# maximyudayev/Realtime-ST-GCN

Hardware: AMD Instinct MI355X
Metric: skeleton-frames/sec/GPU (fwd+bwd), 10-layer ST-GCN N=64 T=300 V=25 (higher is better)
Workload: dtype bf16; 1 GPU; config 2: as_is st-gcn (fcn_in + 9 StgcnLayer, BatchNorm, Kt=9), fwd + loss + bwd + Adam; global_batch=64, seq_len=300, joints=25, parallelism=single, bn_stats=per-replica, launch=eager

## Files before the change

### include/stgcn_amd.h

```cpp
#ifndef STGCN_AMD_H
#define STGCN_AMD_H

#ifdef __cplusplus
extern "C" {
#endif

#define STGCN_ABI_VERSION 7

typedef struct {
  const void* in;
  void* out;
  const void* w;
  const float* bias;
  const float* pro_a;
  const float* pro_b;
  const float* pro_stats;
  float* stats;
  int N, T_in, T_out, V, Cin, Cout, Cin_pad, Cout_pad;
  int Kt, stride, pad, trans, pro, bias_mode, accumulate;
  int in_ld, out_ld;
  const void* w_frag;
} stgcn_conv_desc;

int stgcn_conv_rows(const stgcn_conv_desc* d, int dtype, void* stream);
// ... 2 lines not shown
int stgcn_pack_weight(const float* src, long s0, long s1, long s2, int Kt, int Cout, int Cin, void* dst, int Cout_pad,
                      int Cin_pad, int dtype, void* stream);
int stgcn_pack_weight_frag(const float* src, long s0, long s1, long s2, int Kt, int Cout, int Cin, void* dst,
                           void* dst_frag, int Cout_pad, int Cin_pad, int dtype, void* stream);
int stgcn_pack_weight_s2frag(const float* src, long s0, long s1, long s2, int Cout, int Cin, void* dst_frag, int trans,
                             int dtype, void* stream);
int stgcn_conv_rows_col_tile(int cout);
long stgcn_conv_rows_row_blocks(long M, int cout);

typedef struct {
  const void* in;
  const void* dy;
  float* dw;
  const float* pro_a;
  const float* pro_b;
  const float* pro_stats;
  int N, T_in, T_out, V, Cin, Cout, Kt, stride, pad, pro;
  int in_ld, dy_ld;
  long rows_per_block;
  void* work;
  long work_bytes;
  int out_mode;
  int pad_;
} stgcn_wgrad_desc;

int stgcn_conv_wgrad(const stgcn_wgrad_desc* d, int dtype, void* stream);
long stgcn_conv_wgrad_workspace(const stgcn_wgrad_desc* d, int dtype);

typedef struct {
  const void* x;
  void* out;
  const float* A;
  int N, T, V, P, Cin, per_sample, accumulate;
  int x_ld, out_ld;
} stgcn_amix_desc;

int stgcn_amix_fwd(const stgcn_amix_desc* d, int dtype, void* stream);
int stgcn_amix_trans(const stgcn_amix_desc* d, int dtype, void* stream);
long stgcn_amix_dA_workspace(const stgcn_amix_desc* d);
int stgcn_amix_dA(const stgcn_amix_desc* d, const void* dw, float* dA, void* work, int dtype, void* stream);
int stgcn_gcn_bias_bwd(const float* A, const float* b, const float* S, int P, int V, int C, float* dA, float* db,
                       void* stream);
int stgcn_gcn_bias(const float* A, const float* b, float* out, int N, int P, int V, int C, int per_sample,
                   void* stream);

typedef struct {
  const void* in;
  void* out;
  const void* w;
  const int* nbr;
  const int* deg;
  const float* bias;
  float* stats;
  int NT, V, J, Cin, Cout, Cin_pad, Cout_pad, in_ld, out_ld, accumulate;
  const void* res;
  const void* res_bits;
  int res_ld;
} stgcn_gconv_desc;

int stgcn_gconv(const stgcn_gconv_desc* d, int dtype, void* stream);

long stgcn_gconv_row_blocks(int NT, int V);
int stgcn_gconv_weights(const float* A, const float* W, const int* nbr, const int* deg, int P, int V, int J, int Cout,
                        int Cin, int trans, void* out, int rows_pad, int cols_pad, int dtype, void* stream);
int stgcn_gconv_weights_bias(const float* A, const float* W, const float* b, const int* nbr, const int* deg, int P,
                             int V, int J, int Cout, int Cin, void* out, int rows_pad, int cols_pad, float* bias2d,
                             int dtype, void* stream);
typedef struct {
  const void* x;
  const void* dy;
  const int* nbr;
  const int* deg;
  float* dweff;
  int NT, V, J, Cin, Cout, x_ld, dy_ld;
  void* work;
  long work_bytes;
  float* rowsum;
  int phase;
  int pad_;
} stgcn_gconv_wgrad_desc;

int stgcn_gconv_wgrad(const stgcn_gconv_wgrad_desc* d, int dtype, void* stream);
long stgcn_gconv_wgrad_workspace(const stgcn_gconv_wgrad_desc* d, int dtype);
long stgcn_gconv_wgrad_finish_workspace(int P, int V, int J, int Cout, int Cin);
int stgcn_gconv_wgrad_finish_bias(const float* dweff, const float* A, const float* W, const int* nbr, const int* deg,
                                  int P, int V, int J, int Cout, int Cin, const float* bconv, const float* S, float* dW,
                                  float* dA, float* db, void* work, void* stream);
int stgcn_gconv_wgrad_finish(const float* dweff, const float* A, const float* W, const int* nbr, const int* deg, int P,
                             int V, int J, int Cout, int Cin, float* dW, float* dA, void* work, void* stream);

long stgcn_bn_stat_blocks(long M);
int stgcn_bn_stats_partial(const void* x, int ld, long M, int C, void* part_f4, int dtype, void* stream);
int stgcn_bn_finalize(const void* part_f4, int nblocks, int ld_part, int C, const float* gamma, const float* beta,
                      float eps, void* mean_rstd_f2, float* scale, float* shift, void* stream);
int stgcn_bn_merge(const void* part_f4, int nblocks, int ld_part, int C, void* merged_f4, void* stream);
typedef struct {
  const void* dy;
  const void* mref;
  const void* x1;
  const void* x2;
  const float* msc;
  const float* msh;
  const float* mean_rstd1;
  const float* mean_rstd2;
  const float* gamma1;
  const float* gamma2;
  float* sums;
  void* out1;
  void* out2;
  float* osum;
  float* work;
  long M;
  int C, mask, lddy, ldm, ldx1, ldx2, ldo1, ldo2, acc2;
} stgcn_bn_bwd_desc;

long stgcn_bn_bwd_fused_workspace(long M, int C, int dtype);
int stgcn_bn_bwd_fused_reduce(const stgcn_bn_bwd_desc* d, int dtype, void* stream);
int stgcn_bn_bwd_fused_apply(const stgcn_bn_bwd_desc* d, int dtype, void* stream);
int stgcn_bn_apply(const void* u, int ldu, const float* sc, const float* sh, int res_mode, const void* r, int ldr,
                   const float* rsc, const float* rsh, int relu, void* y, int ldy, long M, int C, int dtype,
                   void* stream);
int stgcn_bn_apply_bits(const void* u, int ldu, const float* sc, const float* sh, int res_mode, const void* r, int ldr,
                        const float* rsc, const float* rsh, int relu, void* y, int ldy, long M, int C, void* bits,
                        void* stream);
int stgcn_bn_bwd_reduce(const void* dy, int lddy, int mask, const void* mref, int ldm, const float* msc,
                        const float* msh, const void* x, int ldx, const void* mean_rstd_f2, long M, int C,
                        void* part_f2, void* sums_f2, int dtype, void* stream);
int stgcn_bn_bwd_apply(const void* dy, int lddy, int mask, const void* mref, int ldm, const float* msc,
                       const float* msh, const void* x, int ldx, const void* mean_rstd_f2, const float* gamma,
                       const void* sums_f2, long M, int C, void* dx, int lddx, int accumulate, int dtype,
                       void* stream);
int stgcn_rowgroup_sum(const void* x, int ld, long M, int C, int G, long period, float* S, float* work, int dtype,
                       void* stream);
long stgcn_rowgroup_sum_workspace(long M, int C, int G, long period);

int stgcn_ln_stats(const void* x, int ld, long frames, int V, int C, float eps, void* stats_f2, int dtype,
                   void* stream);
int stgcn_ln_apply(const void* u, int ldu, const void* st_f2, const float* g, const float* b, int res_mode,
                   const void* r, int ldr, const void* rst_f2, const float* rg, const float* rb, int relu, void* y,
                   int ldy, long M, int V, int C, int dtype, void* stream);
int stgcn_ln_bwd(const void* dy, int lddy, int mask, const void* mref, int ldm, const void* x, int ldx,
                 const void* st_f2, const float* g, const float* b, long frames, int V, int C, void* dx, int lddx,
                 int accumulate, float* dgb, void* work, long work_bytes, int dtype, void* stream);
long stgcn_ln_bwd_workspace(long frames, int V, int C, int dtype);

int stgcn_cast_colsum(const float* x, int ldx, long M, int C, void* out_bf16, int ldo, float* colsum, float* work,
                      void* stream);
long stgcn_cast_colsum_workspace(long M, int C);

int stgcn_pool_rows(const void* x, int ld, int N, int R, int C, void* out, int ldo, int dtype, void* stream);
int stgcn_unpool_rows(const void* dp, int ldp, int R, int C, long M, void* dx, int ldx, int dtype, void* stream);

int stgcn_box_sum(const void* x, int ldx, void* y, int ldy, int N, int T, int V, int C, int K, int S, int trans,
                  int accumulate, int dtype, void* stream);
int stgcn_rt_online_step(const void* z_f32, float* fifo, float* acc, int* idx, int C, int V, int fifo_size, int S,
                         float* out, void* stream);

int stgcn_attn_proj(const void* x, int ldx, long M, int Cin, const float* w, const float* bias, int Nout, float* out,
                    int ldo, void* stream);
long stgcn_attn_scores_workspace(int N, int T, int V, int P);
int stgcn_attn_scores(const void* theta, const void* phi, int ld, int N, int T, int V, int P, int ce, float* C,
                      void* work, int dtype, void* stream);
int stgcn_attn_bwd(const void* theta, const void* phi, int ld, int N, int T, int V, int P, int ce, const float* C,
                   const float* dC, float* dS, void* dtheta, void* dphi, int dtype, void* stream);

int stgcn_abi_version(void);
// ... 290 lines not shown
  const float* ln_b;
  const float* w_in;
  const float* b_in;
  const float* w_out;
  const float* b_out;
  float* xb;
  float* z;
  float* r;
  float* a;
  float* out;
  stgcn_rt_streams_layer layers[STGCN_RT_MAX_LAYERS];
} stgcn_rt_streams_clip_desc;
int stgcn_rt_streams_clip(const stgcn_rt_streams_clip_desc* d, void* stream);

typedef struct {
  int R, V, F, dil, dtype, pad_;
  const float* x;
  const void* wp;
  const float* b1;
  const float* b2;
  float* y;
  void* h;
  const float* dy;
  void* g;
  float* dx;
  float* part;
  float* grads;
} stgcn_ms_layer;
long stgcn_ms_pack_elems(int F);
int stgcn_ms_pack_layer(const float* w1, const float* w2, int F, int kernel, void* dst, int dtype, void* stream);
int stgcn_ms_wgrad_blocks(int R);
int stgcn_ms_layer_fwd(const stgcn_ms_layer* d, void* stream);
int stgcn_ms_layer_bwd(const stgcn_ms_layer* d, void* stream);

typedef struct {
  int rows, pool, I, O, mode, pad_;
  const float* in;
  const float* w;
  const float* b;
  float* out;
  float* p;
  const float* d;
  float* din;
  float* part;
  float* grads;
} stgcn_ms_lin;
int stgcn_ms_lin_blocks(int rows);
int stgcn_ms_in_fwd(const stgcn_ms_lin* d, void* stream);
int stgcn_ms_in_bwd(const stgcn_ms_lin* d, void* stream);
int stgcn_ms_out_fwd(const stgcn_ms_lin* d, void* stream);
int stgcn_ms_out_bwd(const stgcn_ms_lin* d, void* stream);
int stgcn_ms_prob_fwd(const float* x, int rows, int C, int mode, float* y, void* stream);
int stgcn_ms_prob_bwd(const float* y, const float* dy, int rows, int C, int mode, float* dx, void* stream);

int stgcn_window_stat_blocks(int nw, int W);
int stgcn_window_stats(const float* x, int Cin, int Lp, int V, int W, int n0, int nw, int mode, float eps, float* out,
                       void* stream);
int stgcn_window_expand(const float* x, int Cin, int Lp, int V, int W, int n0, int nw, int mode, const float* g,
                        const float* b, const float* fst, const float* w, const float* bias, int Cout, void* out,
                        int ldo, int dtype, void* stream);
long stgcn_window_grad_workspace(int nw, int W, int V, int Cin, int Cout);
int stgcn_window_grad(const void* dy, int ldd, int dtype, const float* x, int Cin, int Lp, int V, int W, int n0, int nw,
                      int mode, const float* st, const float* gamma, const float* beta, const float* w, int Cout,
                      void* work, float* dgamma, float* dbeta, float* dw, float* db, void* stream);

typedef struct {
  int kind, dtype, trans, Kt, Co, Ci, cp, kp;
  long s0, s1, s2, threads;
  const float* src;
  void* dst;
  void* dst_frag;
  const float* A;
  const float* M;
  const int* nbr;
  const int* deg;
  int P, V, J, R_pad, C_pad, pad_;
  const float* bconv;
  float* bias2d;
} stgcn_prep_job;
int stgcn_prep_check(stgcn_prep_job* jobs, int njobs);
int stgcn_prep_run(const stgcn_prep_job* jobs_dev, const long* block_start_dev, int njobs, long nblocks,
                   void* stream);

#define STGCN_ADAM_MAXT 256
typedef struct {
  float* p;
  float* m;
  float* v;
  long n, b0;
  int vec, pad_;
} stgcn_adam_entry;
long stgcn_adam_blocks(long n);
int stgcn_adam_step(const stgcn_adam_entry* table_dev, int ntensors, long nblocks, const float* const* grads,
                    float* steps, double lr, double beta1, double beta2, double eps, double weight_decay,
                    void* stream);

#ifdef __cplusplus
}
#endif
#endif
```

### realtime-st-gcn_amd/__init__.py

```python
from . import _lib, data, loss, metrics, native, optim, parallel, routing, segment, syncbn
from .syncbn import convert_sync_batchnorm, revert_sync_batchnorm
from .graph import Graph, PKU_MMD
from .modules import BatchNorm1d, ConvTemporalGraphical, LayerNorm, StgcnLayer, set_compute_dtype
from .stgcn import Model as Stgcn

MODELS = {
    "st-gcn": Stgcn,
}

try:
    from .rtstgcn import Model as RtStgcn
    MODELS["rt-st-gcn"] = RtStgcn
except ImportError:
    pass
try:
    from .aagcn import Model as AaGcn
    MODELS["aa-gcn"] = AaGcn
except ImportError:
    pass
try:
    from .costgcn import Model as CoStgcn
    MODELS["co-st-gcn"] = CoStgcn
except ImportError:
    pass
try:
    from .mstcn import Model as MsTcn
    from .msgcn import Model as MsGcn
    MODELS["ms-tcn"] = MsTcn
    MODELS["ms-gcn"] = MsGcn
except ImportError:
    pass
```

### realtime-st-gcn_amd/_lib.py

```python
from __future__ import annotations

import ctypes
import os

import torch

_HERE = os.path.dirname(os.path.abspath(__file__))
LIB_PATH = os.environ.get("STGCN_LIB") or os.path.join(_HERE, "lib", "libstgcn_amd.so")

ABI_VERSION = 7

_ERR = {1: "bad shape/arguments", 2: "unsupported dtype", 3: "HIP launch error"}

c_void_p = ctypes.c_void_p
c_int = ctypes.c_int
c_long = ctypes.c_long
c_float = ctypes.c_float


class AdamEntry(ctypes.Structure):
    _fields_ = [("p", c_void_p), ("m", c_void_p), ("v", c_void_p), ("n", c_long), ("b0", c_long), ("vec", c_int),
                ("pad_", c_int)]


class ConvDesc(ctypes.Structure):
    _fields_ = [("in_", c_void_p), ("out", c_void_p), ("w", c_void_p), ("bias", c_void_p), ("pro_a", c_void_p),
                ("pro_b", c_void_p), ("pro_stats", c_void_p), ("stats", c_void_p)] + \
               [(n, c_int) for n in ("N", "T_in", "T_out", "V", "Cin", "Cout", "Cin_pad", "Cout_pad", "Kt", "stride",
                                     "pad", "trans", "pro", "bias_mode", "accumulate", "in_ld", "out_ld")] + \
               [("w_frag", c_void_p)]


class WgradDesc(ctypes.Structure):
    _fields_ = [("in_", c_void_p), ("dy", c_void_p), ("dw", c_void_p), ("pro_a", c_void_p), ("pro_b", c_void_p),
                ("pro_stats", c_void_p)] + \
               [(n, c_int) for n in ("N", "T_in", "T_out", "V", "Cin", "Cout", "Kt", "stride", "pad", "pro",
                                     "in_ld", "dy_ld")] + [("rows_per_block", c_long), ("work", c_void_p),
                                                           ("work_bytes", c_long), ("out_mode", c_int), ("pad_", c_int)]


class AmixDesc(ctypes.Structure):
    _fields_ = [("x", c_void_p), ("out", c_void_p), ("A", c_void_p)] + \
               [(n, c_int) for n in ("N", "T", "V", "P", "Cin", "per_sample", "accumulate", "x_ld", "out_ld")]


class GconvDesc(ctypes.Structure):
    _fields_ = [("in_", c_void_p), ("out", c_void_p), ("w", c_void_p), ("nbr", c_void_p), ("deg", c_void_p),
                ("bias", c_void_p), ("stats", c_void_p)] + \
               [(n, c_int) for n in ("NT", "V", "J", "Cin", "Cout", "Cin_pad", "Cout_pad", "in_ld", "out_ld",
                                     "accumulate")] + [("res", c_void_p), ("res_bits", c_void_p), ("res_ld", c_int)]


class GconvWgradDesc(ctypes.Structure):
    _fields_ = [("x", c_void_p), ("dy", c_void_p), ("nbr", c_void_p), ("deg", c_void_p), ("dweff", c_void_p)] + \
               [(n, c_int) for n in ("NT", "V", "J", "Cin", "Cout", "x_ld", "dy_ld")] + \
               [("work", c_void_p), ("work_bytes", c_long), ("rowsum", c_void_p), ("phase", c_int), ("pad_", c_int)]


class LayerFusedDesc(ctypes.Structure):
    _fields_ = [(n, c_void_p) for n in ("x", "z", "wg_frag", "A", "gbias", "wt_frag", "tbias")] + \
               [(n, c_int) for n in ("N", "T", "V", "P", "x_ld", "z_ld")] + \
               [(n, c_void_p) for n in ("ln1_g", "ln1_b", "ln2_g", "ln2_b")] + [("residual", c_int), ("pad_", c_int)] + \
               [(n, c_void_p) for n in ("g_out", "u_out", "st1_out", "st2_out")] + [("g_ld", c_int), ("u_ld", c_int)] + \
               [("h_out", c_void_p), ("h_ld", c_int), ("pad2_", c_int)]


class BnBwdDesc(ctypes.Structure):
    _fields_ = [(n, c_void_p) for n in ("dy", "mref", "x1", "x2", "msc", "msh", "mean_rstd1", "mean_rstd2",
                                        "gamma1", "gamma2", "sums", "out1", "out2", "osum", "work")] + \
               [("M", c_long)] + [(n, c_int) for n in ("C", "mask", "lddy", "ldm", "ldx1", "ldx2", "ldo1", "ldo2",
                                                       "acc2")]


class PrepJob(ctypes.Structure):
    _fields_ = [(n, c_int) for n in ("kind", "dtype", "trans", "Kt", "Co", "Ci", "cp", "kp")] + \
               [(n, c_long) for n in ("s0", "s1", "s2", "threads")] + \
               [(n, c_void_p) for n in ("src", "dst", "dst_frag", "A", "M", "nbr", "deg")] + \
               [(n, c_int) for n in ("P", "V", "J", "R_pad", "C_pad", "pad_")] + \
               [(n, c_void_p) for n in ("bconv", "bias2d")]


RT_MAX_LAYERS = 12


class RtLayer(ctypes.Structure):
    _fields_ = [(n, c_int) for n in ("Cin", "Cout", "P", "fifo_size", "S", "res_mode")] + \
               [(n, c_void_p) for n in ("A", "w", "bias2d", "wr", "ln_w", "ln_b", "lnr_w", "lnr_b", "fifo", "acc",
                                        "idx", "a_buf", "r_buf")]


class RtFrameDesc(ctypes.Structure):
    _fields_ = [(n, c_int) for n in ("V", "L", "C0", "K", "blocks")] + \
               [(n, c_void_p) for n in ("x", "ln_w", "ln_b", "w_in", "b_in", "w_out", "b_out", "out", "sync",
                                        "status")] + \
               [("layers", RtLayer * RT_MAX_LAYERS)]


class RtStreamsLayer(ctypes.Structure):
    _fields_ = [(n, c_int) for n in ("Cin", "Cout", "P", "fifo_size", "S", "res_mode")] + \
               [(n, c_void_p) for n in ("A", "wp", "bias2d", "wrp", "ln_w", "ln_b", "lnr_w", "lnr_b", "fifo", "acc",
                                        "idx")]


class RtStreamsDesc(ctypes.Structure):
    _fields_ = [(n, c_int) for n in ("V", "L", "C0", "K", "B", "dtype")] + \
               [(n, c_void_p) for n in ("x", "active", "ln_w", "ln_b", "w_in", "b_in", "w_out", "b_out", "out")] + \
               [("layers", RtStreamsLayer * RT_MAX_LAYERS)]


class CoLayer(ctypes.Structure):
    _fields_ = [(n, c_int) for n in ("V", "Cin", "Cout", "P", "Kt", "S", "res_mode", "dtype", "splits", "pad_")] + \
               [(n, c_void_p) for n in ("x", "A", "w", "bias2d", "wr", "br", "ln1_w", "ln1_b", "ln2_w", "ln2_b",
                                        "lnr_w", "lnr_b", "wt", "bt", "ring", "res_ring", "idx", "z_buf", "r_buf",
                                        "partial", "y")]


class CoStreamsLayer(ctypes.Structure):
    _fields_ = [(n, c_int) for n in ("Cin", "Cout", "P", "Kt", "S", "res_mode", "splits", "pad_")] + \
               [(n, c_void_p) for n in ("A", "wp", "bias2d", "wrp", "br", "ln1_w", "ln1_b", "ln2_w", "ln2_b", "lnr_w",
                                        "lnr_b", "wt", "bt", "ring", "res_ring", "idx", "z_buf", "r_buf", "partial",
                                        "y")]


class CoStreamsDesc(ctypes.Structure):
    _fields_ = [(n, c_int) for n in ("B", "V", "L", "C0", "K", "dtype")] + \
               [(n, c_void_p) for n in ("x", "active", "ln_w", "ln_b", "w_in", "b_in", "w_out", "b_out", "h0", "order",
                                        "out")] + \
               [("layers", CoStreamsLayer * RT_MAX_LAYERS)]


CO_CLIP_MAX_T = 256


class CoClipLayer(ctypes.Structure):
    _fields_ = [(n, c_int) for n in ("Cin", "Cout", "P", "Kt", "S", "res_mode", "splits", "pad_")] + \
               [(n, c_void_p) for n in ("A", "wp", "bias2d", "wrp", "br", "ln1_w", "ln1_b", "ln2_w", "ln2_b", "lnr_w",
                                        "lnr_b", "wt", "bt", "ring", "res_ring", "idx", "z_buf", "r_buf", "hist",
                                        "resq", "partial", "y")]


class CoClipDesc(ctypes.Structure):
    _fields_ = [(n, c_int) for n in ("T", "V", "L", "C0", "K", "dtype")] + [("x_stride", c_long)] + \
               [(n, c_void_p) for n in ("x", "ln_w", "ln_b", "w_in", "b_in", "w_out", "b_out", "h0", "out")] + \
               [("layers", CoClipLayer * RT_MAX_LAYERS)]


class CoStreamsClipLayer(ctypes.Structure):
    _fields_ = list(CoClipLayer._fields_)


class CoStreamsClipDesc(ctypes.Structure):
    _fields_ = [(n, c_int) for n in ("B", "T", "t0", "V", "L", "C0", "K", "dtype")] + \
               [(n, c_long) for n in ("x_stride", "x_bstride", "out_bstride")] + \
               [(n, c_void_p) for n in ("x", "active", "lengths", "ln_w", "ln_b", "w_in", "b_in", "w_out", "b_out",
                                        "h0", "out")] + \
               [("layers", CoStreamsClipLayer * RT_MAX_LAYERS)]


RT_CLIP_MAX_T = 256


class RtStreamsClipDesc(ctypes.Structure):
    _fields_ = [(n, c_int) for n in ("B", "T", "t0", "V", "L", "C0", "K", "dtype")] + \
               [(n, c_long) for n in ("x_stride", "x_bstride", "out_bstride", "fstride")] + \
               [(n, c_void_p) for n in ("x", "active", "lengths", "ln_w", "ln_b", "w_in", "b_in", "w_out", "b_out",
                                        "xb", "z", "r", "a", "out")] + \
               [("layers", RtStreamsLayer * RT_MAX_LAYERS)]


class MsLayer(ctypes.Structure):
    _fields_ = [(n, c_int) for n in ("R", "V", "F", "dil", "dtype", "pad_")] + \
               [(n, c_void_p) for n in ("x", "wp", "b1", "b2", "y", "h", "dy", "g", "dx", "part", "grads")]


class MsLin(ctypes.Structure):
    _fields_ = [(n, c_int) for n in ("rows", "pool", "I", "O", "mode", "pad_")] + \
               [(n, c_void_p) for n in ("in_", "w", "b", "out", "p", "d", "din", "part", "grads")]


_SIGS = {
    "stgcn_abi_version": (c_int, []),
    "stgcn_conv_rows": (c_int, [ctypes.POINTER(ConvDesc), c_int, c_void_p]),
    "stgcn_conv_rows_col_tile": (c_int, [c_int]),
    "stgcn_conv_rows_row_blocks": (c_long, [c_long, c_int]),
    "stgcn_conv_wgrad": (c_int, [ctypes.POINTER(WgradDesc), c_int, c_void_p]),
    "stgcn_conv_wgrad_workspace": (c_long, [ctypes.POINTER(WgradDesc), c_int]),
    "stgcn_gconv": (c_int, [ctypes.POINTER(GconvDesc), c_int, c_void_p]),
    "stgcn_bn_bwd_fused_workspace": (c_long, [c_long, c_int, c_int]),
    "stgcn_bn_bwd_fused_reduce": (c_int, [ctypes.POINTER(BnBwdDesc), c_int, c_void_p]),
    "stgcn_bn_bwd_fused_apply": (c_int, [ctypes.POINTER(BnBwdDesc), c_int, c_void_p]),
    "stgcn_gconv_row_blocks": (c_long, [c_int, c_int]),
    "stgcn_gconv_weights_bias": (c_int, [c_void_p] * 5 + [c_int] * 5 + [c_void_p, c_int, c_int, c_void_p, c_int,
                                                                       c_void_p]),
    "stgcn_gconv_weights": (c_int, [c_void_p, c_void_p, c_void_p, c_void_p] + [c_int] * 6 + [c_void_p, c_int, c_int,
                                                                                           c_int, c_void_p]),
    "stgcn_gconv_wgrad": (c_int, [ctypes.POINTER(GconvWgradDesc), c_int, c_void_p]),
    "stgcn_gconv_wgrad_workspace": (c_long, [ctypes.POINTER(GconvWgradDesc), c_int]),
    "stgcn_gconv_wgrad_finish_workspace": (ctypes.c_long, [c_int] * 5),
    "stgcn_gconv_wgrad_finish": (c_int, [c_void_p] * 5 + [c_int] * 5 + [c_void_p, c_void_p, c_void_p, c_void_p]),
    "stgcn_gconv_wgrad_finish_bias": (c_int, [c_void_p] * 5 + [c_int] * 5 + [c_void_p] * 7),
    "stgcn_amix_fwd": (c_int, [ctypes.POINTER(AmixDesc), c_int, c_void_p]),
    "stgcn_amix_trans": (c_int, [ctypes.POINTER(AmixDesc), c_int, c_void_p]),
    "stgcn_gcn_bias_bwd": (c_int, [c_void_p, c_void_p, c_void_p, c_int, c_int, c_int, c_void_p, c_void_p, c_void_p]),
    "stgcn_pack_weight": (c_int, [c_void_p, ctypes.c_long, ctypes.c_long, ctypes.c_long, c_int, c_int, c_int,
                                  c_void_p, c_int, c_int, c_int, c_void_p]),
    "stgcn_tconv_frame": (c_int, [ctypes.POINTER(ConvDesc), c_void_p]),
    "stgcn_tconv_frame_row_blocks": (ctypes.c_long, [c_int, c_int]),
    "stgcn_pack_weight_s2frag": (c_int, [c_void_p, ctypes.c_long, ctypes.c_long, ctypes.c_long, c_int, c_int,
                                         c_void_p, c_int, c_int, c_void_p]),
    "stgcn_pack_weight_frag": (c_int, [c_void_p, ctypes.c_long, ctypes.c_long, ctypes.c_long, c_int, c_int, c_int,
                                       c_void_p, c_void_p, c_int, c_int, c_int, c_void_p]),
    "stgcn_amix_dA_workspace": (ctypes.c_long, [ctypes.POINTER(AmixDesc)]),
    "stgcn_amix_dA": (c_int, [ctypes.POINTER(AmixDesc), c_void_p, c_void_p, c_void_p, c_int, c_void_p]),
    "stgcn_gcn_bias": (c_int, [c_void_p, c_void_p, c_void_p, c_int, c_int, c_int, c_int, c_int, c_void_p]),
    "stgcn_bn_stat_blocks": (c_long, [c_long]),
    "stgcn_bn_stats_partial": (c_int, [c_void_p, c_int, c_long, c_int, c_void_p, c_int, c_void_p]),
    "stgcn_bn_finalize": (c_int, [c_void_p, c_int, c_int, c_int, c_void_p, c_void_p, c_float, c_void_p, c_void_p,
                                  c_void_p, c_void_p]),
    "stgcn_bn_merge": (c_int, [c_void_p, c_int, c_int, c_int, c_void_p, c_void_p]),
    "stgcn_bn_apply": (c_int, [c_void_p, c_int, c_void_p, c_void_p, c_int, c_void_p, c_int, c_void_p, c_void_p,
                               c_int, c_void_p, c_int, c_long, c_int, c_int, c_void_p]),
    "stgcn_bn_apply_bits": (c_int, [c_void_p, c_int, c_void_p, c_void_p, c_int, c_void_p, c_int, c_void_p, c_void_p,
                                    c_int, c_void_p, c_int, c_long, c_int, c_void_p, c_void_p]),
    "stgcn_bn_bwd_reduce": (c_int, [c_void_p, c_int, c_int, c_void_p, c_int, c_void_p, c_void_p, c_void_p, c_int,
                                    c_void_p, c_long, c_int, c_void_p, c_void_p, c_int, c_void_p]),
    "stgcn_bn_bwd_apply": (c_int, [c_void_p, c_int, c_int, c_void_p, c_int, c_void_p, c_void_p, c_void_p, c_int,
                                   c_void_p, c_void_p, c_void_p, c_long, c_int, c_void_p, c_int, c_int, c_int,
                                   c_void_p]),
    "stgcn_rowgroup_sum": (c_int, [c_void_p, c_int, c_long, c_int, c_int, c_long, c_void_p, c_void_p, c_int,
                                   c_void_p]),
    "stgcn_rowgroup_sum_workspace": (c_long, [c_long, c_int, c_int, c_long]),
    "stgcn_ln_stats": (c_int, [c_void_p, c_int, c_long, c_int, c_int, c_float, c_void_p, c_int, c_void_p]),
    "stgcn_ln_apply": (c_int, [c_void_p, c_int, c_void_p, c_void_p, c_void_p, c_int, c_void_p, c_int, c_void_p,
                               c_void_p, c_void_p, c_int, c_void_p, c_int, c_long, c_int, c_int, c_int, c_void_p]),
    "stgcn_ln_bwd": (c_int, [c_void_p, c_int, c_int, c_void_p, c_int, c_void_p, c_int, c_void_p, c_void_p, c_void_p,
                             c_long, c_int, c_int, c_void_p, c_int, c_int, c_void_p, c_void_p, c_long, c_int,
                             c_void_p]),
    "stgcn_ln_bwd_workspace": (c_long, [c_long, c_int, c_int, c_int]),
    "stgcn_cast_colsum": (c_int, [c_void_p, c_int, c_long, c_int, c_void_p, c_int, c_void_p, c_void_p, c_void_p]),
    "stgcn_cast_colsum_workspace": (c_long, [c_long, c_int]),
    "stgcn_pool_rows": (c_int, [c_void_p, c_int, c_int, c_int, c_int, c_void_p, c_int, c_int, c_void_p]),
    "stgcn_unpool_rows": (c_int, [c_void_p, c_int, c_int, c_int, c_long, c_void_p, c_int, c_int, c_void_p]),
    "stgcn_box_sum": (c_int, [c_void_p, c_int, c_void_p, c_int, c_int, c_int, c_int, c_int, c_int, c_int, c_int,
                              c_int, c_int, c_void_p]),
    "stgcn_rt_online_step": (c_int, [c_void_p, c_void_p, c_void_p, c_void_p, c_int, c_int, c_int, c_int, c_void_p,
                                     c_void_p]),
    "stgcn_attn_scores_workspace": (ctypes.c_long, [c_int, c_int, c_int, c_int]),
    "stgcn_attn_scores": (c_int, [c_void_p, c_void_p, c_int, c_int, c_int, c_int, c_int, c_int, c_void_p, c_void_p,
                                  c_int, c_void_p]),
    "stgcn_attn_bwd": (c_int, [c_void_p, c_void_p, c_int, c_int, c_int, c_int, c_int, c_int, c_void_p, c_void_p,
                               c_void_p, c_void_p, c_void_p, c_int, c_void_p]),
    "stgcn_layer_fused_fwd": (c_int, [ctypes.POINTER(LayerFusedDesc), c_void_p]),
    "stgcn_rt_frame_in": (c_int, [c_void_p, c_int, c_void_p, c_void_p, c_void_p, c_void_p, c_int, c_void_p, c_void_p]),
    "stgcn_rt_frame_gcn": (c_int, [c_void_p, c_int, c_int, c_int, c_int] + [c_void_p] * 10),
    "stgcn_rt_frame_norm": (c_int, [c_void_p, c_void_p, c_void_p, c_int, c_void_p, c_void_p, c_void_p, c_int, c_int,
                                    c_void_p, c_int, c_int, c_void_p, c_void_p]),
    "stgcn_rt_frame_out": (c_int, [c_void_p, c_int, c_int, c_void_p, c_void_p, c_int, c_void_p, c_void_p]),
    "stgcn_rt_frame": (c_int, [ctypes.POINTER(RtFrameDesc), c_void_p]),
    "stgcn_rt_streams_pack_elems": (c_long, [c_int, c_int]),
    "stgcn_rt_streams_pack_weight": (c_int, [c_void_p, c_int, c_int, c_int, c_void_p, c_void_p]),
    "stgcn_rt_streams_pack_weight_as": (c_int, [c_void_p, c_int, c_int, c_int, c_void_p, c_int, c_void_p]),
    "stgcn_rt_streams": (c_int, [ctypes.POINTER(RtStreamsDesc), c_void_p]),
    "stgcn_co_pack_elems": (c_long, [c_int, c_int, c_int]),
    "stgcn_co_pack_weight": (c_int, [c_void_p, c_int, c_int, c_int, c_void_p, c_int, c_void_p]),
    "stgcn_co_splits": (c_int, [ctypes.POINTER(CoLayer), c_void_p]),
    "stgcn_co_workspace": (c_long, [ctypes.POINTER(CoLayer), c_void_p]),
    "stgcn_co_gcn": (c_int, [ctypes.POINTER(CoLayer), c_void_p]),
    "stgcn_co_push": (c_int, [ctypes.POINTER(CoLayer), c_void_p]),
    "stgcn_co_taps": (c_int, [ctypes.POINTER(CoLayer), c_void_p]),
    "stgcn_co_finish": (c_int, [ctypes.POINTER(CoLayer), c_void_p]),
    "stgcn_co_streams_splits": (c_int, [ctypes.POINTER(CoStreamsDesc), c_int]),
    "stgcn_co_streams_workspace": (c_long, [ctypes.POINTER(CoStreamsDesc), c_int]),
    "stgcn_co_streams": (c_int, [ctypes.POINTER(CoStreamsDesc), c_void_p]),
    "stgcn_co_clip_splits": (c_int, [ctypes.POINTER(CoClipDesc), c_int]),
    "stgcn_co_clip_workspace": (c_long, [ctypes.POINTER(CoClipDesc), c_int]),
    "stgcn_co_clip": (c_int, [ctypes.POINTER(CoClipDesc), c_void_p]),
    "stgcn_co_streams_clip_splits": (c_int, [ctypes.POINTER(CoStreamsClipDesc), c_int]),
    "stgcn_co_streams_clip_workspace": (c_long, [ctypes.POINTER(CoStreamsClipDesc), c_int]),
    "stgcn_co_streams_clip": (c_int, [ctypes.POINTER(CoStreamsClipDesc), c_void_p]),
    "stgcn_rt_streams_clip": (c_int, [ctypes.POINTER(RtStreamsClipDesc), c_void_p]),
    "stgcn_ms_pack_elems": (c_long, [c_int]),
    "stgcn_ms_pack_layer": (c_int, [c_void_p, c_void_p, c_int, c_int, c_void_p, c_int, c_void_p]),
    "stgcn_ms_wgrad_blocks": (c_int, [c_int]),
    "stgcn_ms_layer_fwd": (c_int, [ctypes.POINTER(MsLayer), c_void_p]),
    "stgcn_ms_layer_bwd": (c_int, [ctypes.POINTER(MsLayer), c_void_p]),
    "stgcn_ms_lin_blocks": (c_int, [c_int]),
    "stgcn_ms_in_fwd": (c_int, [ctypes.POINTER(MsLin), c_void_p]),
    "stgcn_ms_in_bwd": (c_int, [ctypes.POINTER(MsLin), c_void_p]),
    "stgcn_ms_out_fwd": (c_int, [ctypes.POINTER(MsLin), c_void_p]),
    "stgcn_ms_out_bwd": (c_int, [ctypes.POINTER(MsLin), c_void_p]),
    "stgcn_ms_prob_fwd": (c_int, [c_void_p, c_int, c_int, c_int, c_void_p, c_void_p]),
    "stgcn_ms_prob_bwd": (c_int, [c_void_p, c_void_p, c_int, c_int, c_int, c_void_p, c_void_p]),
    "stgcn_window_stat_blocks": (c_int, [c_int, c_int]),
    "stgcn_window_stats": (c_int, [c_void_p] + [c_int] * 7 + [c_float, c_void_p, c_void_p]),
    "stgcn_window_expand": (c_int, [c_void_p] + [c_int] * 7 + [c_void_p] * 5 + [c_int, c_void_p, c_int, c_int,
                                                                                c_void_p]),
    "stgcn_window_grad_workspace": (ctypes.c_long, [c_int] * 5),
    "stgcn_window_grad": (c_int, [c_void_p, c_int, c_int, c_void_p] + [c_int] * 7 + [c_void_p] * 4 + [c_int] +
                          [c_void_p] * 6),
    "stgcn_attn_proj": (c_int, [c_void_p, c_int, c_long, c_int, c_void_p, c_void_p, c_int, c_void_p, c_int, c_void_p]),
    "stgcn_segment_metrics_workspace": (ctypes.c_long, [c_int]),
    "stgcn_segment_metrics": (c_int, [c_void_p, c_void_p, c_int, c_int, c_void_p, c_int, c_void_p, c_void_p,
                                      c_void_p, c_void_p, c_void_p]),
    "stgcn_seg_loss_workspace": (ctypes.c_long, [c_int]),
    "stgcn_seg_loss": (c_int, [c_void_p, c_int, c_void_p, c_void_p, c_void_p, c_int, c_int, c_int, c_int, c_void_p,
                               c_float, c_void_p, c_void_p, c_void_p, c_void_p, c_void_p, c_void_p]),
    "stgcn_seg_loss_bwd": (c_int, [c_void_p, c_void_p, c_void_p, c_void_p, c_long, c_void_p, c_void_p]),
    "stgcn_prep_check": (c_int, [ctypes.POINTER(PrepJob), c_int]),
    "stgcn_prep_run": (c_int, [c_void_p, c_void_p, c_int, c_long, c_void_p]),
    "stgcn_adam_blocks": (ctypes.c_long, [c_long]),
    "stgcn_adam_step": (c_int, [c_void_p, c_int, c_long, c_void_p, c_void_p] + [ctypes.c_double] * 5 + [c_void_p]),
}

EXPORTS = tuple(_SIGS)

_lib = None


def load_library(path: str = LIB_PATH):
    global _lib
    if _lib is not None:
        return _lib
    if not os.path.exists(path):
        raise RuntimeError(f"stgcn_amd: native library not built: {path} (run __graft_entry__.build())")
    lib = ctypes.CDLL(path)
    for name, (res, args) in _SIGS.items():
        fn = getattr(lib, name)
        fn.restype = res
        fn.argtypes = args
    got = lib.stgcn_abi_version()
    if got != ABI_VERSION:
        raise RuntimeError(f"stgcn_amd: {path} implements C-ABI version {got}, these bindings need {ABI_VERSION} "
                           "(stale build: run __graft_entry__.build())")
    _lib = lib
    return lib


def lib():
    if _lib is None:
        load_library()
    return _lib


def check(rc: int, name: str):
    if rc != 0:
        raise RuntimeError(f"stgcn_amd.{name} failed with code {rc} ({_ERR.get(rc, 'unknown')})")


def require_device(t: torch.Tensor):
    if not t.is_cuda:
        raise RuntimeError("stgcn_amd ops run on the HIP device only (no CPU fallback); got a CPU tensor")


def stream() -> int:
    return torch._C._cuda_getCurrentRawStream(torch._C._cuda_getDevice())


def dtype_code(dt: torch.dtype) -> int:
    if dt == torch.float32:
        return 0
    if dt == torch.bfloat16:
        return 1
    raise RuntimeError(f"stgcn_amd: unsupported dtype {dt} (fp32 or bf16)")


def ptr(t):
    return None if t is None else t.data_ptr()
```

### realtime-st-gcn_amd/csrc/capi.cpp

```cpp
#include <hip/hip_runtime.h>

#include "../../include/stgcn_amd.h"
#include "launchers.h"

#define STGCN_OK 0
#define STGCN_EBADSHAPE 1
#define STGCN_EDTYPE 2

#define CHECK_DTYPE(dt) \
  if ((dt) != 0 && (dt) != 1) return STGCN_EDTYPE
#define STREAM(s) reinterpret_cast<hipStream_t>(s)

extern "C" {

int stgcn_abi_version(void) { return STGCN_ABI_VERSION; }

int stgcn_conv_rows(const stgcn_conv_desc* d, int dtype, void* stream) {
  CHECK_DTYPE(dtype);
  if (!d || !d->in || !d->out || !d->w || d->N <= 0 || d->V <= 0 || d->T_in <= 0 || d->T_out <= 0 || d->Kt <= 0 ||
      d->stride <= 0 || d->Cin <= 0 || d->Cout <= 0 || d->in_ld < d->Cin || d->out_ld < d->Cout ||
      d->Cin_pad < d->Cin || d->Cout_pad < d->Cout)
    return STGCN_EBADSHAPE;
  if ((d->pro == 1 && (!d->pro_a || !d->pro_b)) || (d->pro == 2 && (!d->pro_a || !d->pro_b || !d->pro_stats)))
    return STGCN_EBADSHAPE;
// ... 20 lines not shown
  if (!src || !dst || !dst_frag || Kt <= 0 || Co <= 0 || Ci <= 0 || Cout_pad < Co || Cin_pad < Ci) return STGCN_EBADSHAPE;
  return pack_weight_launch(src, s0, s1, s2, Kt, Co, Ci, dst, Cout_pad, Cin_pad, dtype, STREAM(stream), dst_frag);
}
long stgcn_conv_rows_row_blocks(long M, int cout) { return conv_rows_num_row_blocks(M, cout); }

long stgcn_conv_wgrad_workspace(const stgcn_wgrad_desc* d, int dtype) {
  if (!d || (dtype != 0 && dtype != 1)) return 0;
  const long wr = wgrad_ring_workspace(*d, dtype);
  if (wr > 0) return wr;
  const long w = wgrad_wide_workspace(*d, dtype);
  if (w > 0) return w;
  const long w1 = wgrad1x1_workspace(*d, dtype);
  return w1 > 0 ? w1 : wgrad_tile_workspace(*d, dtype);
}

int stgcn_conv_wgrad(const stgcn_wgrad_desc* d, int dtype, void* stream) {
  CHECK_DTYPE(dtype);
  if (!d || !d->in || !d->dy || !d->dw || d->N <= 0 || d->Kt <= 0 || d->stride <= 0) return STGCN_EBADSHAPE;
  if (d->pro && (!d->pro_a || !d->pro_b || (d->pro == 2 && !d->pro_stats))) return STGCN_EBADSHAPE;
  if (d->out_mode != 0 && d->out_mode != 1) return STGCN_EBADSHAPE;
  const int rr = wgrad_ring_launch(*d, dtype, STREAM(stream));
  if (rr >= 0) return rr;
  const int rw = wgrad_wide_launch(*d, dtype, STREAM(stream));
  if (rw >= 0) return rw;
  const int r1 = wgrad1x1_launch(*d, dtype, STREAM(stream));
  if (r1 >= 0) return r1;
  const int r = wgrad_tile_launch(*d, dtype, STREAM(stream));
  if (r >= 0) return r;
  if (d->out_mode) return STGCN_EBADSHAPE;
  return conv_wgrad_launch(*d, dtype, STREAM(stream));
}

long stgcn_bn_bwd_fused_workspace(long M, int C, int dtype) {
  if (M <= 0 || C <= 0 || (dtype != 0 && dtype != 1)) return 0;
  return bn_bwd_fused_work_floats(M, C, dtype);
}
int stgcn_bn_bwd_fused_reduce(const stgcn_bn_bwd_desc* d, int dtype, void* stream) {
  CHECK_DTYPE(dtype);
  if (!d || !d->dy || d->M <= 0 || d->C <= 0 || (d->mask && !d->mref) || (d->mask == 2 && (!d->msc || !d->msh)) ||
      (d->x1 && !d->mean_rstd1) || (d->x2 && !d->mean_rstd2) || (d->mask == 3 && (dtype != 1 || d->C % 8 || d->ldm < d->C / 8)))
    return STGCN_EBADSHAPE;
  return bn_bwd_fused_reduce_launch(*d, dtype, STREAM(stream));
}
int stgcn_bn_bwd_fused_apply(const stgcn_bn_bwd_desc* d, int dtype, void* stream) {
  CHECK_DTYPE(dtype);
  if (!d || !d->dy || d->M <= 0 || d->C <= 0 || (d->mask && !d->mref) || (d->mask == 2 && (!d->msc || !d->msh)) ||
      (d->x1 && !d->mean_rstd1) || (d->x2 && !d->mean_rstd2) || (d->mask == 3 && (dtype != 1 || d->C % 8 || d->ldm < d->C / 8)))
    return STGCN_EBADSHAPE;
  return bn_bwd_fused_apply_launch(*d, dtype, STREAM(stream));
}

int stgcn_gconv(const stgcn_gconv_desc* d, int dtype, void* stream) {
  CHECK_DTYPE(dtype);
  if (!d || !d->in || !d->out || !d->w || !d->nbr || !d->deg || d->NT <= 0 || d->V <= 0 || d->J <= 0 ||
      d->Cin <= 0 || d->Cout <= 0 || d->Cin_pad < d->Cin || d->Cout_pad < d->Cout || d->in_ld < d->Cin ||
      d->out_ld < d->Cout)
    return STGCN_EBADSHAPE;
  return gconv_launch(*d, dtype, STREAM(stream));
}
long stgcn_gconv_row_blocks(int NT, int V) { return gconv_row_blocks(NT, V); }
int stgcn_gconv_weights(const float* A, const float* W, const int* nbr, const int* deg, int P, int V, int J, int Cout,
                        int Cin, int trans, void* out, int rows_pad, int cols_pad, int dtype, void* stream) {
  CHECK_DTYPE(dtype);
  if (!A || !W || !nbr || !deg || !out || P <= 0 || V <= 0 || J <= 0 || Cout <= 0 || Cin <= 0 ||
      rows_pad < (trans ? Cin : Cout) || cols_pad < (trans ? Cout : Cin))
    return STGCN_EBADSHAPE;
  return gconv_weights_launch(A, W, nbr, deg, P, V, J, Cout, Cin, trans, out, rows_pad, cols_pad, dtype,
                              STREAM(stream));
}
int stgcn_gconv_weights_bias(const float* A, const float* W, const float* b, const int* nbr, const int* deg, int P,
                             int V, int J, int Cout, int Cin, void* out, int rows_pad, int cols_pad, float* bias2d,
                             int dtype, void* stream) {
  CHECK_DTYPE(dtype);
  if (!A || !W || !b || !nbr || !deg || !out || !bias2d || P <= 0 || V <= 0 || J <= 0 || Cout <= 0 || Cin <= 0 ||
      rows_pad < Cout || cols_pad < Cin || (cols_pad % 8) != 0)
    return STGCN_EBADSHAPE;
  return gconv_weights_launch(A, W, nbr, deg, P, V, J, Cout, Cin, 0, out, rows_pad, cols_pad, dtype, STREAM(stream),
                              b, bias2d);
}
long stgcn_gconv_wgrad_workspace(const stgcn_gconv_wgrad_desc* d, int dtype) {
  if (!d || (dtype != 0 && dtype != 1)) return 0;
  return gconv_wgrad_workspace(*d, dtype);
}
int stgcn_gconv_wgrad(const stgcn_gconv_wgrad_desc* d, int dtype, void* stream) {
  CHECK_DTYPE(dtype);
  if (!d || !d->x || !d->dy || !d->nbr || !d->deg || !d->dweff || d->NT <= 0 || d->V <= 0 || d->J <= 0 ||
      d->Cin <= 0 || d->Cout <= 0)
    return STGCN_EBADSHAPE;
  return gconv_wgrad_launch(*d, dtype, STREAM(stream));
}
int stgcn_gconv_wgrad_finish_bias(const float* dweff, const float* A, const float* W, const int* nbr, const int* deg,
                                  int P, int V, int J, int Cout, int Cin, const float* bconv, const float* S, float* dW,
                                  float* dA, float* db, void* work, void* stream) {
  if (!dweff || !A || !W || !nbr || !deg || !bconv || !S || !dW || !dA || !db || !work || P <= 0 || V <= 0 || J <= 0 ||
      Cout <= 0 || Cin <= 0)
    return STGCN_EBADSHAPE;
  return gconv_wgrad_finish_bias_launch(dweff, A, W, nbr, deg, P, V, J, Cout, Cin, bconv, S, dW, dA, db, work,
                                        STREAM(stream));
}
long stgcn_gconv_wgrad_finish_workspace(int P, int V, int J, int Cout, int Cin) {
  return gconv_wgrad_finish_workspace(P, V, J, Cout, Cin);
}
int stgcn_gconv_wgrad_finish(const float* dweff, const float* A, const float* W, const int* nbr, const int* deg, int P,
                             int V, int J, int Cout, int Cin, float* dW, float* dA, void* work, void* stream) {
  if (!dweff || !A || !W || !nbr || !deg || P <= 0 || V <= 0 || J <= 0 || Cout <= 0 || Cin <= 0)
    return STGCN_EBADSHAPE;
  return gconv_wgrad_finish_launch(dweff, A, W, nbr, deg, P, V, J, Cout, Cin, dW, dA, work, STREAM(stream));
}
int stgcn_tconv_frame(const stgcn_conv_desc* d, void* stream) {
  if (!d) return STGCN_EBADSHAPE;
  return tconv_frame_launch(*d, STREAM(stream));
}
long stgcn_tconv_frame_row_blocks(int N, int T) { return tconv_frame_row_blocks(N, T); }

int stgcn_amix_fwd(const stgcn_amix_desc* d, int dtype, void* stream) {
  CHECK_DTYPE(dtype);
  if (!d || !d->x || !d->out || !d->A) return STGCN_EBADSHAPE;
  return amix_fwd_launch(*d, dtype, STREAM(stream));
}
int stgcn_amix_trans(const stgcn_amix_desc* d, int dtype, void* stream) {
  CHECK_DTYPE(dtype);
  if (!d || !d->x || !d->out || !d->A) return STGCN_EBADSHAPE;
  return amix_trans_launch(*d, dtype, STREAM(stream));
}
long stgcn_amix_dA_workspace(const stgcn_amix_desc* d) { return d ? amix_dA_workspace(*d) : 0; }
int stgcn_amix_dA(const stgcn_amix_desc* d, const void* dw, float* dA, void* work, int dtype, void* stream) {
  CHECK_DTYPE(dtype);
  if (!d || !d->x || !dw || !dA) return STGCN_EBADSHAPE;
  return amix_dA_launch(*d, dw, dA, work, dtype, STREAM(stream));
}
int stgcn_gcn_bias_bwd(const float* A, const float* b, const float* S, int P, int V, int C, float* dA, float* db,
                       void* stream) {
  if (!A || !b || !S || !dA || !db || P <= 0 || V <= 0 || C <= 0) return STGCN_EBADSHAPE;
  return gcn_bias_bwd_launch(A, b, S, P, V, C, dA, db, STREAM(stream));
}
int stgcn_gcn_bias(const float* A, const float* b, float* out, int N, int P, int V, int C, int per_sample,
                   void* stream) {
  if (!A || !b || !out) return STGCN_EBADSHAPE;
  return gcn_bias_launch(A, b, out, N, P, V, C, per_sample, STREAM(stream));
}

long stgcn_bn_stat_blocks(long M) { return norm_stats_num_blocks(M); }
int stgcn_bn_stats_partial(const void* x, int ld, long M, int C, void* part, int dtype, void* stream) {
  CHECK_DTYPE(dtype);
  return bn_stats_partial_launch(x, ld, M, C, (float4*)part, dtype, STREAM(stream));
}
int stgcn_bn_finalize(const void* part, int nb, int ldp, int C, const float* gamma, const float* beta, float eps,
                      void* mean_rstd, float* scale, float* shift, void* stream) {
  return bn_finalize_launch((const float4*)part, nb, ldp, C, gamma, beta, eps, (float2*)mean_rstd, scale, shift,
                            STREAM(stream));
}
int stgcn_bn_merge(const void* part, int nb, int ldp, int C, void* merged, void* stream) {
  return bn_merge_launch((const float4*)part, nb, ldp, C, (float4*)merged, STREAM(stream));
}
int stgcn_bn_apply(const void* u, int ldu, const float* sc, const float* sh, int res_mode, const void* r, int ldr,
                   const float* rsc, const float* rsh, int relu, void* y, int ldy, long M, int C, int dtype,
                   void* stream) {
  CHECK_DTYPE(dtype);
  if (res_mode && !r) return STGCN_EBADSHAPE;
  return bn_apply_launch(u, ldu, sc, sh, res_mode, r, ldr, rsc, rsh, relu, y, ldy, M, C, dtype, STREAM(stream));
}
int stgcn_bn_apply_bits(const void* u, int ldu, const float* sc, const float* sh, int res_mode, const void* r, int ldr,
                        const float* rsc, const float* rsh, int relu, void* y, int ldy, long M, int C, void* bits,
                        void* stream) {
  if ((res_mode && !r) || !bits || C % 8) return STGCN_EBADSHAPE;
  return bn_apply_launch(u, ldu, sc, sh, res_mode, r, ldr, rsc, rsh, relu, y, ldy, M, C, 1, STREAM(stream),
// ... 267 lines not shown
```

### realtime-st-gcn_amd/csrc/gconv_finish.hip

```cpp
#include "common.h"
#include "launchers.h"

namespace {

__global__ void gconv_dw_kernel(const float* __restrict__ dweff, const float* __restrict__ A, const int* nbr,
                                const int* deg, int P, int V, int J, int Cout, int Cin, float* dW) {
  const long idx = (long)blockIdx.x * blockDim.x + threadIdx.x;
  const long E = (long)Cout * Cin;
  if (idx >= (long)P * E) return;
  const int p = (int)(idx / E);
  const long e = idx % E;
  float s = 0.f;
  for (int w = 0; w < V; ++w)
    for (int j = 0; j < deg[w]; ++j) s += A[((long)p * V + nbr[w * J + j]) * V + w] * dweff[(long)(w * J + j) * E + e];
  dW[idx] += s;
}

__global__ void gconv_dA_kernel(const float* __restrict__ dweff, const float* __restrict__ W, const int* nbr,
                                const int* deg, int P, int V, int J, int Cout, int Cin, float* dA) {
  const int pair = blockIdx.x, p = blockIdx.y;
  const int w = pair / J, j = pair % J;
  if (j >= deg[w]) return;
  const long E = (long)Cout * Cin;
  const float* d = dweff + (long)pair * E;
  const float* wp = W + (long)p * E;
  float s = 0.f;
  for (long e = threadIdx.x; e < E; e += blockDim.x) s += wp[e] * d[e];
  s = wave_sum(s);
  __shared__ float part[4];
  if ((threadIdx.x & 63) == 0) part[threadIdx.x >> 6] = s;
  __syncthreads();
  if (threadIdx.x == 0) {
    const float t = part[0] + part[1] + part[2] + part[3];
    dA[((long)p * V + nbr[w * J + j]) * V + w] += t;
  }
}

constexpr int PMAX = 4;
constexpr int DW_PAIRS = 32 * 8;
DEV void gconv_dw_all_body(const float* __restrict__ dweff, const float* __restrict__ A, const int* nbr,
                           const int* deg, int P, int V, int J, long E, float* dW, long bb, bool acc_out) {
  __shared__ int spair[DW_PAIRS];
  __shared__ float scoef[DW_PAIRS][PMAX];
  __shared__ int snp;
  if (threadIdx.x == 0) {
    int n = 0;
    for (int w = 0; w < V; ++w)
      for (int j = 0; j < deg[w]; ++j) spair[n++] = w * J + j;
    snp = n;
  }
  __syncthreads();
  const int np = snp;
  for (int i = threadIdx.x; i < np * PMAX; i += 256) {
    const int k = i / PMAX, p = i % PMAX;
    const int pr = spair[k], w = pr / J;
    scoef[k][p] = p < P ? A[((long)p * V + nbr[pr]) * V + w] : 0.f;
  }
  __syncthreads();
  const int g = threadIdx.x >> 6;
  const long e = (bb * 64 + (threadIdx.x & 63)) * 4;
  float4 acc[PMAX];
#pragma unroll
  for (int p = 0; p < PMAX; ++p) acc[p] = make_float4(0.f, 0.f, 0.f, 0.f);
  if (e < E) {
#pragma unroll 4
    for (int k = g; k < np; k += 4) {
      const float4 d = *reinterpret_cast<const float4*>(dweff + (long)spair[k] * E + e);
#pragma unroll
      for (int p = 0; p < PMAX; ++p) {
        const float c = scoef[k][p];
        acc[p].x += c * d.x; acc[p].y += c * d.y; acc[p].z += c * d.z; acc[p].w += c * d.w;
      }
    }
  }
  __shared__ float4 part[4][PMAX][64];
#pragma unroll
  for (int p = 0; p < PMAX; ++p) part[g][p][threadIdx.x & 63] = acc[p];
  __syncthreads();
  if (threadIdx.x < 64 && e < E) {
    const int l = threadIdx.x;
#pragma unroll
    for (int p = 0; p < PMAX; ++p)
      if (p < P) {
        const float4 a0 = part[0][p][l], a1 = part[1][p][l], a2 = part[2][p][l], a3 = part[3][p][l];
        float4 t = make_float4(((a0.x + a1.x) + a2.x) + a3.x, ((a0.y + a1.y) + a2.y) + a3.y,
                               ((a0.z + a1.z) + a2.z) + a3.z, ((a0.w + a1.w) + a2.w) + a3.w);
        float4* o = reinterpret_cast<float4*>(dW + (long)p * E + e);
        if (acc_out) {
          const float4 q = *o;
          t.x += q.x; t.y += q.y; t.z += q.z; t.w += q.w;
        }
        *o = t;
      }
  }
}
__global__ __launch_bounds__(256) void gconv_dw_all_kernel(const float* __restrict__ dweff, const float* __restrict__ A,
                                                           const int* nbr, const int* deg, int P, int V, int J, long E,
                                                           float* dW) {
  gconv_dw_all_body(dweff, A, nbr, deg, P, V, J, E, dW, blockIdx.x, true);
}

constexpr int DA_CHUNK = 2048;
DEV void gconv_dA_part_body(const float* __restrict__ dweff, const float* __restrict__ W, const int* deg, int P, int J,
                           long E, float* part, int pair, int c, int nch) {
  if (pair % J >= deg[pair / J]) return;
  const float* d = dweff + (long)pair * E;
  float acc[PMAX] = {0.f, 0.f, 0.f, 0.f};
  const long e1 = min(E, (long)(c + 1) * DA_CHUNK);
  for (long e = (long)c * DA_CHUNK + threadIdx.x * 4; e < e1; e += 1024) {
    const float4 dv = *reinterpret_cast<const float4*>(d + e);
#pragma unroll
    for (int p = 0; p < PMAX; ++p)
      if (p < P) {
        const float4 w = *reinterpret_cast<const float4*>(W + (long)p * E + e);
        acc[p] += ((w.x * dv.x + w.y * dv.y) + w.z * dv.z) + w.w * dv.w;
      }
  }
  __shared__ float red[4][PMAX];
#pragma unroll
  for (int p = 0; p < PMAX; ++p) {
    const float t = wave_sum(acc[p]);
    if ((threadIdx.x & 63) == 0) red[threadIdx.x >> 6][p] = t;
  }
  __syncthreads();
  if (threadIdx.x < P)
    part[((long)pair * nch + c) * PMAX + threadIdx.x] =
        ((red[0][threadIdx.x] + red[1][threadIdx.x]) + red[2][threadIdx.x]) + red[3][threadIdx.x];
}
__global__ __launch_bounds__(256) void gconv_dA_part_kernel(const float* __restrict__ dweff, const float* __restrict__ W,
                                                            const int* deg, int P, int J, long E, float* part) {
  gconv_dA_part_body(dweff, W, deg, P, J, E, part, blockIdx.x, blockIdx.y, gridDim.y);
}

__global__ __launch_bounds__(256) void gconv_finish1_kernel(const float* __restrict__ dweff, const float* __restrict__ A,
                                                            const float* __restrict__ W, const int* nbr, const int* deg,
                                                            int P, int V, int J, long E, float* dW, int nb_dw, int nch,
                                                            float* part) {
  const int b = blockIdx.x;
  if (b < nb_dw) {
    gconv_dw_all_body(dweff, A, nbr, deg, P, V, J, E, dW, b, false);
  } else {
    const int b2 = b - nb_dw;
    gconv_dA_part_body(dweff, W, deg, P, J, E, part, b2 / nch, b2 % nch, nch);
  }
}

constexpr int FV_MAX = 32;
__global__ __launch_bounds__(256) void gconv_finish2_kernel(const float* __restrict__ part, const float* __restrict__ A,
                                                            const float* __restrict__ b, const float* __restrict__ S,
                                                            const int* nbr, const int* deg, int P, int V, int J, int C,
                                                            int nch, float* dA, float* db) {
  const int bx = blockIdx.x;
  if (bx < P * V) {
    const int p = bx / V, w = bx % V;
    float t = 0.f;
    for (int c = threadIdx.x; c < C; c += 256) t += b[p * C + c] * S[w * C + c];
    t = wave_sum(t);
    __shared__ float red[4];
    __shared__ float sup[FV_MAX];
    if ((threadIdx.x & 63) == 0) red[threadIdx.x >> 6] = t;
    if (threadIdx.x < V) sup[threadIdx.x] = 0.f;
    __syncthreads();
    const float tot = ((red[0] + red[1]) + red[2]) + red[3];
    if (threadIdx.x < deg[w]) {
      const int j = threadIdx.x, pair = w * J + j;
      float s = 0.f;
      for (int c = 0; c < nch; ++c) s += part[((long)pair * nch + c) * PMAX + p];
      sup[nbr[pair]] = s;
    }
    __syncthreads();
    for (int v = threadIdx.x; v < V; v += 256) dA[(p * V + v) * V + w] = sup[v] + tot;
    return;
  }
  __shared__ float cs[PMAX * FV_MAX];
  for (int i = threadIdx.x; i < P * V; i += 256) {
    const int p = i / V, w = i % V;
    float t = 0.f;
    for (int v = 0; v < V; ++v) t += A[(p * V + v) * V + w];
    cs[i] = t;
  }
  __syncthreads();
  const int i = (bx - P * V) * 256 + threadIdx.x;
  if (i >= P * C) return;
  const int p = i / C, c = i % C;
  float t = 0.f;
  for (int w = 0; w < V; ++w) t += cs[p * V + w] * S[w * C + c];
  db[i] = t;
}

__global__ void gconv_dA_reduce_kernel(const float* __restrict__ part, const int* nbr, const int* deg, int P, int V,
                                       int J, int nch, float* dA) {
  const int i = blockIdx.x * blockDim.x + threadIdx.x;
  if (i >= V * J * P) return;
  const int pair = i / P, p = i % P, w = pair / J, j = pair % J;
  if (j >= deg[w]) return;
  float s = 0.f;
  for (int c = 0; c < nch; ++c) s += part[((long)pair * nch + c) * PMAX + p];
  dA[((long)p * V + nbr[w * J + j]) * V + w] += s;
}

}

long gconv_wgrad_finish_workspace(int P, int V, int J, int Cout, int Cin) {
  const long E = (long)Cout * Cin;
  return P > PMAX ? 0 : (long)V * J * ((E + DA_CHUNK - 1) / DA_CHUNK) * PMAX * (long)sizeof(float);
}

bool gconv_finish_bias_ok(int P, int V, int J) { return P <= PMAX && V <= FV_MAX && V * J <= DW_PAIRS; }

int gconv_wgrad_finish_bias_launch(const float* dweff, const float* A, const float* W, const int* nbr, const int* deg,
                                   int P, int V, int J, int Cout, int Cin, const float* bconv, const float* S, float* dW,
                                   float* dA, float* db, void* work, hipStream_t s) {
  if (!gconv_finish_bias_ok(P, V, J) || !work || ((long)Cout * Cin) % 4) return STGCN_EBADSHAPE;
  const long E = (long)Cout * Cin;
  const int nch = (int)((E + DA_CHUNK - 1) / DA_CHUNK);
  const int nb_dw = (int)((E + 255) / 256);
  float* part = reinterpret_cast<float*>(work);
  hipLaunchKernelGGL(gconv_finish1_kernel, dim3((unsigned)(nb_dw + V * J * nch)), dim3(256), 0, s, dweff, A, W, nbr,
                     deg, P, V, J, E, dW, nb_dw, nch, part);
  hipLaunchKernelGGL(gconv_finish2_kernel, dim3((unsigned)(P * V + (P * Cout + 255) / 256)), dim3(256), 0, s,
                     (const float*)part, A, bconv, S, nbr, deg, P, V, J, Cout, nch, dA, db);
  return hipGetLastError() == hipSuccess ? STGCN_OK : STGCN_EHIP;
}

int gconv_wgrad_finish_launch(const float* dweff, const float* A, const float* W, const int* nbr, const int* deg,
                              int P, int V, int J, int Cout, int Cin, float* dW, float* dA, void* work, hipStream_t s) {
  const long E = (long)Cout * Cin;
  if (P > PMAX || (dA && !work) || V * J > DW_PAIRS || E % 4) {
    const long n = (long)P * E;
    if (dW)
      hipLaunchKernelGGL(gconv_dw_kernel, dim3((unsigned)((n + 255) / 256)), dim3(256), 0, s, dweff, A, nbr, deg, P,
                         V, J, Cout, Cin, dW);
    if (dA)
      hipLaunchKernelGGL(gconv_dA_kernel, dim3((unsigned)(V * J), (unsigned)P), dim3(256), 0, s, dweff, W, nbr, deg,
                         P, V, J, Cout, Cin, dA);
  } else {
    if (dW)
      hipLaunchKernelGGL(gconv_dw_all_kernel, dim3((unsigned)((E + 255) / 256)), dim3(256), 0, s, dweff, A, nbr, deg,
                         P, V, J, E, dW);
    if (dA) {
      const int nch = (int)((E + DA_CHUNK - 1) / DA_CHUNK);
      float* part = reinterpret_cast<float*>(work);
      hipLaunchKernelGGL(gconv_dA_part_kernel, dim3((unsigned)(V * J), (unsigned)nch), dim3(256), 0, s, dweff, W,
                         deg, P, J, E, part);
      hipLaunchKernelGGL(gconv_dA_reduce_kernel, dim3((unsigned)((V * J * P + 255) / 256)), dim3(256), 0, s, part,
                         nbr, deg, P, V, J, nch, dA);
    }
  }
  return hipGetLastError() == hipSuccess ? STGCN_OK : STGCN_EHIP;
}
```

### realtime-st-gcn_amd/csrc/gconv_wgrad.hip

```cpp
#include "common.h"
#include "launchers.h"
#include "lds_ops.h"
#include "../../include/stgcn_amd.h"

namespace {

constexpr int WKM = 128;
constexpr int WPR = 64;

struct WGG {
  int ntile, tpb, R, nco, nci;
  float* slab;
  float* rowpart;
  int zero_unused;
  float* part;
  unsigned* cnt;
};
constexpr int W3_SPLIT_DEG = 4;

__global__ __launch_bounds__(256, 2) void gconv_wgrad_kernel(const stgcn_gconv_wgrad_desc a, const WGG g) {
  constexpr int PANEL = WKM * WPR;
  constexpr int STAGE = 4 * PANEL;
  extern __shared__ __attribute__((aligned(16))) char smem[];
  const int tid = threadIdx.x, lane = tid & 63, wave = tid >> 6;
  const int V = a.V;
  const int ngrp = g.nco * g.nci;
  const int pair = blockIdx.x / (ngrp * g.R);
  const int rem = blockIdx.x % (ngrp * g.R);
  const int rr = rem / ngrp, grp = rem % ngrp;
  const int w = pair / a.J, j = pair % a.J;
  if (j >= a.deg[w]) return;
  const int src = a.nbr[pair];
  const int co0 = (grp % g.nco) * 64, ci0 = (grp / g.nco) * 64;
  const int t0 = rr * g.tpb, t1 = min(g.ntile, t0 + g.tpb);

  const bf16* __restrict__ dy = reinterpret_cast<const bf16*>(a.dy);
  const bf16* __restrict__ x = reinterpret_cast<const bf16*>(a.x);
  const int uc = tid & 7;
  const int co = co0 + uc * 8, ci = ci0 + uc * 8;
  uint4 ry[4], rx[4];
  auto load = [&](int t) {
#pragma unroll
    for (int u = 0; u < 4; ++u) {
      const int row = (tid >> 3) + u * 32;
      const int i = t * WKM + row;
      ry[u] = make_uint4(0, 0, 0, 0);
      rx[u] = make_uint4(0, 0, 0, 0);
      if (i < a.NT) {
        if (co < a.Cout) ry[u] = *reinterpret_cast<const uint4*>(dy + ((long)i * V + w) * a.dy_ld + co);
        if (ci < a.Cin) rx[u] = *reinterpret_cast<const uint4*>(x + ((long)i * V + src) * a.x_ld + ci);
      }
    }
  };
  auto store = [&](int buf) {
    char* base = smem + buf * STAGE;
#pragma unroll
    for (int u = 0; u < 4; ++u) {
      const int row = (tid >> 3) + u * 32;
      const int off = (uc >> 2) * PANEL + row * WPR + (uc & 3) * 16;
      *reinterpret_cast<uint4*>(base + off) = ry[u];
      *reinterpret_cast<uint4*>(base + 2 * PANEL + off) = rx[u];
    }
  };

  f32x16 acc[2][2];
#pragma unroll
  for (int a2 = 0; a2 < 2; ++a2)
#pragma unroll
    for (int b2 = 0; b2 < 2; ++b2)
#pragma unroll
      for (int r = 0; r < 16; ++r) acc[a2][b2][r] = 0.f;

  int cur = 0;
  if (t0 < t1) {
    load(t0);
    store(0);
  }
  __syncthreads();
  for (int t = t0; t < t1; ++t) {
    const bool more = t + 1 < t1;
    if (more) load(t + 1);
    const char* base = smem + cur * STAGE;
#pragma unroll
    for (int kk = 0; kk < WKM / 16 / 4; ++kk) {
      const int ks = wave + 4 * kk;
// ... 569 lines not shown

__global__ __launch_bounds__(256, 1) void gconv_wgrad3w_kernel(const stgcn_gconv_wgrad_desc a, const WGG g) {
  extern __shared__ __attribute__((aligned(16))) char smem[];
  const int ngrp = g.nco * g.nci;
  const int bid = blockIdx.x;
  const int e = bid / (ngrp * g.R), rem = bid % (ngrp * g.R);
  const int rr = rem / ngrp, grp = rem % ngrp;
  int* sdeg = reinterpret_cast<int*>(smem);
  int* order = sdeg + 64;
  int* ent = order + 64;
  const int tid = threadIdx.x;
  if (tid < a.V) sdeg[tid] = a.deg[tid];
  __syncthreads();
  if (tid < a.V) {
    const int d = sdeg[tid];
    int r = 0;
    for (int u = 0; u < a.V; ++u) r += (sdeg[u] > d) | ((sdeg[u] == d) & (u < tid));
    order[r] = tid;
  }
  __syncthreads();
  if (tid == 0) {
    int E = 0;
    for (int r = 0; r < a.V; ++r) {
      const int w = order[r], d = sdeg[w];
      if (d > W3W_JE) {
        const int h = (d + 1) / 2;
        ent[1 + 3 * E] = w, ent[2 + 3 * E] = 0, ent[3 + 3 * E] = h, ++E;
        ent[1 + 3 * E] = w, ent[2 + 3 * E] = h, ent[3 + 3 * E] = d - h, ++E;
      } else {
        ent[1 + 3 * E] = w, ent[2 + 3 * E] = 0, ent[3 + 3 * E] = d, ++E;
      }
    }
    ent[0] = E;
  }
  __syncthreads();
  const int E = ent[0];
  const int wj = e < E ? ent[1 + 3 * e] : 0, j0 = e < E ? ent[2 + 3 * e] : 0, n = e < E ? ent[3 + 3 * e] : 0;
  const int dtot = e < E ? sdeg[wj] : 0;
  __syncthreads();
  if (e >= E) return;
  const int t0 = rr * g.tpb, t1 = min(g.ntile, t0 + g.tpb);
  switch (n) {
    case 1: wgrad3w_body<1>(a, g, smem, wj, e, j0, dtot, rr, grp, t0, t1); break;
    case 2: wgrad3w_body<2>(a, g, smem, wj, e, j0, dtot, rr, grp, t0, t1); break;
    case 3: wgrad3w_body<3>(a, g, smem, wj, e, j0, dtot, rr, grp, t0, t1); break;
    default:
      if (rr != 0) break;
      const int co0 = (grp % g.nco) * 128, ci0 = (grp / g.nco) * 128;
      if (g.rowpart != nullptr && grp / g.nco == 0 && tid < 128) {
        const bf16* dy = reinterpret_cast<const bf16*>(a.dy);
        float s = 0.f;
        for (int i = 0; i < a.NT; ++i) s += (float)dy[((long)i * a.V + wj) * a.dy_ld + co0 + tid];
        g.rowpart[(long)wj * a.Cout + co0 + tid] = s;
      }
      for (int i = tid; i < a.J * 128 * 128; i += blockDim.x) {
        const int j = i >> 14, co = (i >> 7) & 127, ci = i & 127;
        g.slab[(((long)wj * a.J + j) * a.Cout + co0 + co) * a.Cin + ci0 + ci] = 0.f;
      }
      break;
  }
}

__global__ void gconv_wgrad_f32_kernel(const stgcn_gconv_wgrad_desc a) {
  const long idx = (long)blockIdx.x * blockDim.x + threadIdx.x;
  const long total = (long)a.V * a.J * a.Cout * a.Cin;
  if (idx >= total) return;
  const int ci = (int)(idx % a.Cin);
  const int co = (int)((idx / a.Cin) % a.Cout);
  const int pair = (int)(idx / ((long)a.Cin * a.Cout));
  const int w = pair / a.J, j = pair % a.J;
  if (j >= a.deg[w]) {
    a.dweff[idx] = 0.f;
    return;
  }
  const int src = a.nbr[pair];
  const float* dy = reinterpret_cast<const float*>(a.dy);
  const float* x = reinterpret_cast<const float*>(a.x);
  float s = 0.f;
  for (int i = 0; i < a.NT; ++i)
    s += dy[((long)i * a.V + w) * a.dy_ld + co] * x[((long)i * a.V + src) * a.x_ld + ci];
  a.dweff[idx] = s;
}

__global__ void rowpart_sum_kernel(const float* __restrict__ part, int R, long E, float* __restrict__ out) {
  const long e = (long)blockIdx.x * blockDim.x + threadIdx.x;
  if (e >= E) return;
  float s = 0.f;
  for (int r = 0; r < R; ++r) s += part[(long)r * E + e];
  out[e] = s;
}

__global__ void gslab_rowpart_kernel(const float* __restrict__ slab, int R, long E, long EC, const int* deg, int J,
                                     float* __restrict__ dweff, int nb1, const float* __restrict__ rpart, long ER,
                                     float* __restrict__ rowsum) {
  if ((int)blockIdx.x < nb1) {
    const long e = (long)blockIdx.x * blockDim.x + threadIdx.x;
    if (e >= E) return;
    const int pair = (int)(e / EC);
    float s = 0.f;
    if (pair % J < deg[pair / J])
      for (int r = 0; r < R; ++r) s += slab[(long)r * E + e];
    dweff[e] = s;
    return;
  }
  const long e = (long)(blockIdx.x - nb1) * blockDim.x + threadIdx.x;
  if (e >= ER) return;
  float s = 0.f;
  for (int r = 0; r < R; ++r) s += rpart[(long)r * ER + e];
  rowsum[e] = s;
}

__global__ void gslab_reduce_kernel(const float* __restrict__ slab, int R, long E, long EC, const int* deg, int J,
                                    float* __restrict__ out) {
  const long e = (long)blockIdx.x * blockDim.x + threadIdx.x;
  if (e >= E) return;
  const int pair = (int)(e / EC);
  float s = 0.f;
  if (pair % J < deg[pair / J])
    for (int r = 0; r < R; ++r) s += slab[(long)r * E + e];
  out[e] = s;
}

enum WgradKernel {
  WG_F32,
  WG_PAIR,
  WG_REG,
  WG_RING,
  WG_WIDE,
};
struct WgradPlan {
  WgradKernel kernel;
  WGG g;
  bool direct;
  bool split;
  long slab_floats;
  long rowpart_floats;
  long part_floats;
  long cnt_bytes;
  long slab_off, rowpart_off, part_off, cnt_off, total;
  long grid;
  int block;
  size_t lds;
};

void set_row_parts(WGG& g, long want) {
  long R = want;
  if (R > g.ntile) R = g.ntile;
  if (R < 1) R = 1;
  g.tpb = (int)((g.ntile + R - 1) / R);
  g.R = (g.ntile + g.tpb - 1) / g.tpb;
}

constexpr long W3_WIDE_TARGET = 256;
constexpr long W3_NARROW_TARGET = 1024;
constexpr long W2_TARGET = 512;
constexpr long W3W_TARGET = 256;

WgradPlan plan_wgrad(const stgcn_gconv_wgrad_desc& a, int dtype) {
  WgradPlan p{};
  WGG& g = p.g;
  const long E = (long)a.V * a.J * a.Cout * a.Cin;
  p.block = 256;
  if (dtype != 1) {
    p.kernel = WG_F32;
    p.direct = true;
    p.grid = (E + 255) / 256;
    return p;
  }
  const bool grouped = a.J <= J2 && a.Cin % 64 == 0 && a.Cout % 64 == 0;
  const bool wide = grouped && a.Cin % 128 == 0 && a.Cout % 128 == 0 && a.V <= 64 && a.J <= 2 * W3W_JE &&
                    W3W_TARGET / ((long)a.V * (a.Cout / 128) * (a.Cin / 128)) <= 2;
  if (wide) {
    p.kernel = WG_WIDE;
    g.ntile = (a.NT + 31) / 32;
    g.nco = a.Cout / 128;
    g.nci = a.Cin / 128;
    const long groups = (long)a.V * g.nco * g.nci;
    set_row_parts(g, W3W_TARGET / groups);
    p.direct = true;
    if (g.R > 1) {
      p.part_floats = 2 * groups * g.R * ((long)W3W_JE * W3W_PSZ_J + 128);
      p.cnt_bytes = (2 * groups * 4 + 15) / 16 * 16;
    }
    p.grid = 2 * groups * g.R;
    p.lds = W3W_LDS;
  } else if (grouped) {
    const bool ring = !(a.Cin == 64 && a.Cout == 128);
    p.kernel = ring ? WG_RING : WG_REG;
    g.ntile = (a.NT + W2M - 1) / W2M;
    g.nco = a.Cout / W2_COB;
    g.nci = a.Cin / 64;
    const long groups = (long)a.V * g.nco * g.nci;
    const long target = !ring ? W2_TARGET : groups <= 32 ? W3_NARROW_TARGET : groups < 200 ? 512 : W3_WIDE_TARGET;
    set_row_parts(g, (target + groups - 1) / groups);
    p.direct = p.split = ring && g.R == 1;
    if (p.split) {
      p.part_floats = groups * 2 * ((long)a.J * 4096 + 64);
      p.cnt_bytes = (groups * 4 + 15) / 16 * 16;
    } else {
      p.slab_floats = (long)g.R * E;
      p.rowpart_floats = a.rowsum ? (long)g.R * a.V * a.Cout : 0;
    }
    p.grid = groups * g.R * (p.split ? 2 : 1);
    p.lds = ring ? W3_LDS : W2_LDS;
  } else {
    p.kernel = WG_PAIR;
    g.ntile = (a.NT + WKM - 1) / WKM;
    g.nco = (a.Cout + 63) / 64;
    g.nci = (a.Cin + 63) / 64;
    const long groups = (long)a.V * a.J * g.nco * g.nci;
    set_row_parts(g, (1024 + groups - 1) / groups);
    p.slab_floats = (long)g.R * E;
    p.grid = groups * g.R;
    p.lds = 2 * 4 * WKM * WPR;
  }
  p.rowpart_off = p.slab_off + p.slab_floats * (long)sizeof(float);
  p.part_off = p.rowpart_off + p.rowpart_floats * (long)sizeof(float);
  p.cnt_off = p.part_off + p.part_floats * (long)sizeof(float);
  p.total = p.cnt_off + p.cnt_bytes;
  return p;
}

}

long gconv_wgrad_workspace(const stgcn_gconv_wgrad_desc& a, int dtype) { return plan_wgrad(a, dtype).total; }

int gconv_wgrad_launch(const stgcn_gconv_wgrad_desc& a, int dtype, hipStream_t s) {
  const long E = (long)a.V * a.J * a.Cout * a.Cin;
  if (a.phase < 0 || a.phase > 2) return STGCN_EBADSHAPE;
  if (dtype == 1 && (a.Cin % 8 || a.Cout % 8 || a.x_ld % 8 || a.dy_ld % 8)) return STGCN_EBADSHAPE;
  const WgradPlan p = plan_wgrad(a, dtype);
  if (p.kernel == WG_F32) {
    if (a.phase == 2) return STGCN_OK;
    hipLaunchKernelGGL(gconv_wgrad_f32_kernel, dim3((unsigned)p.grid), dim3(p.block), 0, s, a);
    return hipGetLastError() == hipSuccess ? STGCN_OK : STGCN_EHIP;
  }
  if (p.kernel == WG_WIDE && a.phase == 2) return STGCN_OK;
  if (p.kernel == WG_PAIR && a.rowsum) return STGCN_EBADSHAPE;
  if (p.total && (!a.work || a.work_bytes < p.total)) return STGCN_EBADSHAPE;
  char* const work = reinterpret_cast<char*>(a.work);
  WGG g = p.g;
  if (p.direct) {
    g.slab = a.dweff;
    g.rowpart = a.rowsum;
    g.zero_unused = 1;
  } else {
    g.slab = reinterpret_cast<float*>(work + p.slab_off);
    g.rowpart = p.rowpart_floats ? reinterpret_cast<float*>(work + p.rowpart_off) : nullptr;
  }
  if (p.part_floats) {
    g.part = reinterpret_cast<float*>(work + p.part_off);
    g.cnt = reinterpret_cast<unsigned*>(work + p.cnt_off);
    if (a.phase != 2 && hipMemsetAsync(g.cnt, 0, (size_t)p.cnt_bytes, s) != hipSuccess) return STGCN_EHIP;
  }
  void (*const k)(const stgcn_gconv_wgrad_desc, const WGG) = p.kernel == WG_WIDE   ? gconv_wgrad3w_kernel
                                                             : p.kernel == WG_RING ? gconv_wgrad3_kernel
                                                             : p.kernel == WG_REG  ? gconv_wgrad2_kernel
                                                                                   : gconv_wgrad_kernel;
  if (stgcn_lds_attr((const void*)k, 160 * 1024, s)) return STGCN_EHIP;
  if (a.phase != 2) hipLaunchKernelGGL(k, dim3((unsigned)p.grid), dim3(p.block), p.lds, s, a, g);
  if (p.direct || a.phase == 1) return hipGetLastError() == hipSuccess ? STGCN_OK : STGCN_EHIP;
  if (p.rowpart_floats) {
    const long ER = (long)a.V * a.Cout;
    const int nb1 = (int)((E + 255) / 256);
    hipLaunchKernelGGL(gslab_rowpart_kernel, dim3((unsigned)(nb1 + (ER + 255) / 256)), dim3(256), 0, s,
                       (const float*)g.slab, g.R, E, (long)a.Cout * a.Cin, a.deg, a.J, a.dweff, nb1,
                       (const float*)g.rowpart, ER, a.rowsum);
  } else {
    hipLaunchKernelGGL(gslab_reduce_kernel, dim3((unsigned)((E + 255) / 256)), dim3(256), 0, s, (const float*)g.slab,
                       g.R, E, (long)a.Cout * a.Cin, a.deg, a.J, a.dweff);
  }
  return hipGetLastError() == hipSuccess ? STGCN_OK : STGCN_EHIP;
}
```

### realtime-st-gcn_amd/csrc/launchers.h

```cpp
#pragma once
#include <hip/hip_runtime.h>

#include "../../include/stgcn_amd.h"

int conv_rows_launch(const stgcn_conv_desc& a, int dtype, hipStream_t s);
int conv_rows_bn_tile(int cout);
int pack_weight_launch(const float* src, long s0, long s1, long s2, int Kt, int Co, int Ci, void* dst, int cp, int kp,
                       int dtype, hipStream_t s, void* dst_frag);
long conv_rows_num_row_blocks(long M, int cout);
int pack_s2frag_launch(const float* src, long s0, long s1, long s2, int Co, int Ci, void* dst, int trans,
                       hipStream_t s);
int tconv_frame_launch(const stgcn_conv_desc& a, hipStream_t s);
long tconv_frame_row_blocks(int N, int T);
int conv_wgrad_launch(stgcn_wgrad_desc a, int dtype, hipStream_t s);
long wgrad_tile_workspace(const stgcn_wgrad_desc& a, int dtype);
int wgrad_tile_launch(const stgcn_wgrad_desc& a, int dtype, hipStream_t s);
long wgrad_wide_workspace(const stgcn_wgrad_desc& a, int dtype);
int wgrad_wide_launch(const stgcn_wgrad_desc& a, int dtype, hipStream_t s);
long wgrad_ring_workspace(const stgcn_wgrad_desc& a, int dtype);
int wgrad_ring_launch(const stgcn_wgrad_desc& a, int dtype, hipStream_t s);
long wgrad1x1_workspace(const stgcn_wgrad_desc& a, int dtype);
int wgrad1x1_launch(const stgcn_wgrad_desc& a, int dtype, hipStream_t s);
long gconv_row_blocks(int NT, int V);
int gconv_launch(const stgcn_gconv_desc& a, int dtype, hipStream_t s);
int gconv_weights_launch(const float* A, const float* W, const int* nbr, const int* deg, int P, int V, int J, int Cout,
                         int Cin, int trans, void* out, int R_pad, int C_pad, int dtype, hipStream_t s,
                         const float* bconv = nullptr, float* bias2d = nullptr);
long gconv_wgrad_workspace(const stgcn_gconv_wgrad_desc& a, int dtype);
int gconv_wgrad_launch(const stgcn_gconv_wgrad_desc& a, int dtype, hipStream_t s);
int gconv_wgrad_finish_launch(const float* dweff, const float* A, const float* W, const int* nbr, const int* deg,
                              int P, int V, int J, int Cout, int Cin, float* dW, float* dA, void* work, hipStream_t s);
long gconv_wgrad_finish_workspace(int P, int V, int J, int Cout, int Cin);
int gconv_wgrad_finish_bias_launch(const float* dweff, const float* A, const float* W, const int* nbr, const int* deg,
                                   int P, int V, int J, int Cout, int Cin, const float* bconv, const float* S, float* dW,
                                   float* dA, float* db, void* work, hipStream_t s);
int amix_fwd_launch(const stgcn_amix_desc& a, int dtype, hipStream_t s);
int amix_trans_launch(const stgcn_amix_desc& a, int dtype, hipStream_t s);
int amix_dA_launch(const stgcn_amix_desc& a, const void* dw, float* dA, void* work, int dtype, hipStream_t s);
long amix_dA_workspace(const stgcn_amix_desc& a);
int gcn_bias_bwd_launch(const float* A, const float* b, const float* S, int P, int V, int C, float* dA, float* db,
                        hipStream_t s);
int gcn_bias_launch(const float* A, const float* b, float* out, int N, int P, int V, int C, int per_sample,
                    hipStream_t s);
long bn_bwd_fused_work_floats(long M, int C, int dtype);
int bn_bwd_fused_reduce_launch(const stgcn_bn_bwd_desc& a, int dtype, hipStream_t s);
int bn_bwd_fused_apply_launch(const stgcn_bn_bwd_desc& a, int dtype, hipStream_t s);
long norm_stats_num_blocks(long M);
int bn_stats_partial_launch(const void* x, int ld, long M, int C, float4* part, int dtype, hipStream_t s);
int bn_finalize_launch(const float4* part, int nb, int ldp, int C, const float* gamma, const float* beta, float eps,
                       float2* mean_rstd, float* scale, float* shift, hipStream_t s);
int bn_merge_launch(const float4* part, int nb, int ldp, int C, float4* merged, hipStream_t s);
int bn_apply_launch(const void* u, int ldu, const float* sc, const float* sh, int res_mode, const void* r, int ldr,
                    const float* rsc, const float* rsh, int relu, void* y, int ldy, long M, int C, int dtype,
                    hipStream_t s, unsigned char* bits = nullptr);
int bn_bwd_reduce_launch(const void* dy, int lddy, int mask, const void* mref, int ldm, const float* msc,
                         const float* msh, const void* x, int ldx, const float2* mean_rstd, long M, int C,
                         float2* part, float2* out, int dtype, hipStream_t s);
int bn_bwd_apply_launch(const void* dy, int lddy, int mask, const void* mref, int ldm, const float* msc,
                        const float* msh, const void* x, int ldx, const float2* mean_rstd, const float* gamma,
                        const float2* sums, long M, int C, void* dx, int lddx, int accumulate, int dtype,
                        hipStream_t s);
int rowgroup_sum_launch(const void* x, int ld, long M, int C, int G, long period, float* S, float* work, int dtype,
                        hipStream_t s);
long rowgroup_sum_workspace(long M, int C, int G, long period);
long cast_colsum_workspace(long M, int C);
int cast_colsum_launch(const float* x, int ldx, long M, int C, void* out16, int ldo, float* colsum, float* work,
                       hipStream_t s);
int pool_rows_launch(const void* x, int ld, int N, int R, int C, void* out, int ldo, int dtype, hipStream_t s);
int unpool_rows_launch(const void* dp, int ldp, int R, int C, long M, void* dx, int ldx, int dtype, hipStream_t s);
int ln_stats_launch(const void* x, int ld, long F, int V, int C, float eps, float2* stats, int dtype, hipStream_t s);
int ln_apply_launch(const void* u, int ldu, const float2* st, const float* g, const float* b, int res_mode,
                    const void* r, int ldr, const float2* rst, const float* rg, const float* rb, int relu, void* y,
                    int ldy, long M, int V, int C, int dtype, hipStream_t s);
long ln_bwd_workspace(long F, int V, int C, int dtype);
int ln_bwd_launch(const void* dy, int lddy, int mask, const void* mref, int ldm, const void* x, int ldx,
                  const float2* st, const float* g, const float* b, long F, int V, int C, void* dx, int lddx,
                  int accumulate, float* dgb, void* work, long work_bytes, int dtype, hipStream_t s);
int box_sum_launch(const void* x, int ldx, void* y, int ldy, int N, int T_, int V, int C, int K, int S, int trans,
                   int accumulate, int dtype, hipStream_t s);
int rt_online_launch(const float* z, float* fifo, float* acc, int* idx, int C, int V, int fifo_size, int S,
                     float* out, hipStream_t s);
int attn_scores_launch(const void* th, const void* ph, int ld, int N, int T_, int V, int P, int ce, float* S,
                       void* work, int dtype, hipStream_t s);
long attn_scores_workspace(int N, int T_, int V, int P);
int attn_proj_launch(const void* x, int ldx, long M, int Cin, const float* W, const float* bias, int Nout, float* out,
                     int ldo, hipStream_t s);
int attn_bwd_launch(const void* th, const void* ph, int ld, int N, int T_, int V, int P, int ce, const float* C,
                    const float* dC, float* dS, void* dth, void* dph, int dtype, hipStream_t s);
int layer_fused_launch(const stgcn_layer_fused_desc& a, hipStream_t s);
int rt_in_launch(const float* x, int V, const float* g, const float* b, const float* W, const float* bias, int C0,
                 float* out, hipStream_t s);
int rt_gcn_launch(const float* x, int V, int Cin, int Cout, int P, const float* A, const float* W, const float* bias2d,
                  float* fifo, float* acc, const int* idx, const float* Wr, float* a_out, float* r_out,
                  hipStream_t s);
int rt_norm_launch(const float* a, const float* g, const float* b, int res_mode, const float* res, const float* gr,
                   const float* br, int V, int C, int* idx, int fifo_size, int S, float* y, hipStream_t s);
int rt_out_launch(const float* x, int V, int C, const float* W, const float* bias, int K, float* out, hipStream_t s);
int rt_frame_launch(const stgcn_rt_frame_desc& d, hipStream_t s);
int rt_streams_launch(const stgcn_rt_streams_desc& d, hipStream_t s);
int co_check(const stgcn_co_layer& d, bool shapes_only);
int co_num_splits(const stgcn_co_layer& d, hipStream_t s);
long co_pack_elems(int Cout, int C, int Kt);
int co_pack_launch(const float* w, int Cout, int C, int Kt, void* dst, int dtype, hipStream_t s);
long co_pack_rows_elems(int rows, int C);
int co_pack_rows_launch(const float* w, int groups, int rows, int C, void* dst, int dtype, hipStream_t s);
int co_gcn_launch(const stgcn_co_layer& d, hipStream_t s);
int co_push_launch(const stgcn_co_layer& d, hipStream_t s);
int co_taps_launch(const stgcn_co_layer& d, hipStream_t s);
int co_finish_launch(const stgcn_co_layer& d, hipStream_t s);
int co_streams_check(const stgcn_co_streams_desc& d, bool shapes_only);
int co_streams_num_splits(const stgcn_co_streams_desc& d, int layer);
int co_streams_launch(const stgcn_co_streams_desc& d, hipStream_t s);
// ... 36 lines not shown
```

### realtime-st-gcn_amd/layer_fn.py

```python
from __future__ import annotations

from types import SimpleNamespace
from typing import NamedTuple

import torch

from . import native as K
from .routing import ROUTING
from .syncbn import active_sync

BN, LN = "BatchNorm", "LayerNorm"


class LayerCfg(NamedTuple):
    kt: int
    stride: int
    residual: bool
    norm: str
    dtype: torch.dtype
    sup: object = None
    dense_dA: bool = False
    infer: bool = False
    cache: dict = None
    packs: object = None
    sync: object = None


class RtLayerCfg(NamedTuple):
    Kt: int
    S: int
    residual: bool
    norm: str
    dtype: torch.dtype
    sync: object = None


def _save_named(ctx, **tensors):
    ctx.saved_names = tuple(tensors)
    ctx.save_for_backward(*tensors.values())


def _saved(ctx):
    return SimpleNamespace(**dict(zip(ctx.saved_names, ctx.saved_tensors)))


def _f32(p):
    return p.detach().float().contiguous()


def _flat_ln(p):
    return p.detach().reshape(-1).float().contiguous()


def _wg_rows(wg, P, Cout, Cin):
    return wg.detach().float().view(P, Cout, Cin).permute(1, 0, 2).reshape(1, Cout, P * Cin)


def _wg_rows_T(wg, P, Cout, Cin):
    return wg.detach().float().view(P, Cout, Cin).permute(0, 2, 1).reshape(1, P * Cin, Cout)


def gcn_forward(x, A32, wg, bg, dtype, stats=None):
    N, Cin, T, V = x.shape
    P = A32.shape[-3]
    Cout = wg.shape[0] // P
    XA = K.amix_fwd(x, A32)
    wgp, cp, kp = K.pack_weight(_wg_rows(wg, P, Cout, Cin), dtype)
    bias2d = K.gcn_bias(A32, _f32(bg), N, Cout)
    g = K.conv_rows(XA, wgp, P * Cin, Cout, cp, kp, T, T, bias=bias2d, bias_mode=3 if A32.dim() == 4 else 2,
                    stats=stats)
    return XA, g, cp


def gcn_stats_buffer(M, Cout, dev):
    cp = -(-Cout // K.col_tile(Cout)) * K.col_tile(Cout)
    return torch.zeros((K.row_blocks(M, Cout), cp, 4), dtype=torch.float32, device=dev), cp


def _gcn_dgrad_rows(dg, wg, P, Cin, Cout, T, dtype):
    wgTp, cq, kq = K.pack_weight(_wg_rows_T(wg, P, Cout, Cin), dtype)
    return K.conv_rows(dg, wgTp, Cout, P * Cin, cq, kq, T, T)


def gcn_backward(x, A32, XA, wg, bg, dg, dx, accumulate, dtype, z_S=None):
    N, Cin, T, V = x.shape
    P = A32.shape[-3]
    Cout = wg.shape[0] // P
    DW = _gcn_dgrad_rows(dg, wg, P, Cin, Cout, T, dtype)
    K.amix_trans(DW, A32, Cin, dx, accumulate=accumulate)
    dA = K.amix_dA(x, DW, A32)
    dwg = K.conv_wgrad(XA, dg, P * Cin, Cout, T, T, Kt=1)
    dwg = dwg.view(Cout, P, Cin).permute(1, 0, 2).reshape(P * Cout, Cin, 1, 1)
    dA, dbg = _bias_through_A(dA, A32, bg, dg, z_S=z_S)
    return dA, dwg, dbg


def _bias_through_A(dA, A32, bg, dg, S=None, z_S=None):
    N, Cout, T, V = dg.shape
    M = N * T * V
    if A32.dim() == 4:
        Sn = K.rowgroup_sum(dg, M, Cout, V, per_sample=True, out=z_S)
        dA = dA + torch.einsum("pc,nwc->npw", bg.detach().float().view(-1, Cout), Sn).unsqueeze(2)
        colsum = A32.sum(dim=2)
        return dA, torch.einsum("npw,nwc->pc", colsum, Sn).reshape(-1)
    if S is None:
        S = K.rowgroup_sum(dg, M, Cout, V, out=z_S)
    if not dA.is_contiguous():
        dA = dA.contiguous()
# ... 1 lines not shown


def _packs(cache, wg, wt, P, Cin, Cout, dtype):
    key = (wg.data_ptr(), wg._version, wt.data_ptr(), wt._version, dtype)
    if cache is not None and cache.get("key") == key:
        return cache["val"]
    wimg, cpg, kwg = K.pack_gcn_weight(_wg_rows(wg, P, Cout, Cin)[0], dtype)
    wt3 = wt.detach().float().squeeze(-1).permute(2, 0, 1)
    wtp, _, _ = K.pack_weight(wt3, dtype, stride=1)
    val = (wimg, cpg, kwg, wtp)
    if cache is not None:
        cache["key"], cache["val"] = key, val
    return val


class LayerPacks:
    __slots__ = ("gw", "gwT", "wt", "wtT", "wr", "wrT")

    def __init__(self):
        self.gw = self.gwT = self.wt = self.wtT = self.wr = self.wrT = None


def plan_layer_packs(plan, layer, A, M, dtype):
    sup = layer._gsup
    P, V = A.shape[0], A.shape[-1]
    conv = layer.tcn[2]
    Cout, Cin = conv.out_channels, layer.gcn.conv.in_channels
    kt, stride = layer.kernel_size[0], layer.stride
    if sup is None or A.dim() != 3 or sup.dense(P):
        return None
    pk = LayerPacks()
    wg2 = layer.gcn.conv.weight.detach().reshape(P * Cout, Cin)
    pk.gw = K.gconv_weights(A, wg2, sup, Cout, Cin, False, dtype, bias=layer.gcn.conv.bias.detach(), plan=plan, M=M)
    pk.gwT = K.gconv_weights(A, wg2, sup, Cout, Cin, True, dtype, plan=plan, M=M)
    wt = conv.weight.detach().squeeze(-1)
    pk.wt = K.pack_weight(wt.permute(2, 0, 1), dtype, stride=stride, plan=plan)
    pk.wtT = K.pack_weight(wt.permute(2, 1, 0), dtype, stride=stride, trans=True, plan=plan)
    if layer.is_residual_conv:
        wr = layer.residual[0].weight.detach().view(Cout, Cin)
        pk.wr = K.pack_weight(wr.unsqueeze(0), dtype, plan=plan)
        pk.wrT = K.pack_weight(wr.t().unsqueeze(0), dtype, plan=plan)
    return pk


def fused_layer_forward(x, A32, wg, bg, n1w, n1b, wt, bt, n2w, n2b, residual, dtype, tag=None, cache=None,
                        train=False, packs=None):
    N, Cin, T, V = x.shape
    P = A32.shape[0]
    Cout = wt.shape[0]
    if packs is not None and packs.wt is not None and packs.gw is not None:
        bias2d = packs.gw[1]
        wimg, cpg, kwg = K.pack_gcn_weight(_wg_rows(wg, P, Cout, Cin)[0], dtype)
        wtp = packs.wt[0]
    else:
        bias2d = K.gcn_bias(A32, _f32(bg), N, Cout)
        wimg, cpg, kwg, wtp = _packs(cache, wg, wt, P, Cin, Cout, dtype)
    lkey = tuple((t.data_ptr(), t._version) for t in (n1w, n1b, n2w, n2b))
    if cache is not None and cache.get("ln_key") == lkey:
        ln = cache["ln_val"]
    else:
        ln = tuple(torch.stack([p.detach().float().reshape(Cout, V).t() for p in (n1w, n1b, n2w, n2b)]).unbind(0))
        if cache is not None:
            cache["ln_key"], cache["ln_val"] = lkey, ln
    return K.layer_fused(x, A32, wimg, bias2d, wtp, _f32(bt), ln, tag=tag, residual=residual, train=train)


def _stats_arena(cache, dev, dtype, shapes, route):
    if cache is None:
        return K.zeros_arena(dev, *shapes)
    key = ("bn_stats", str(dev), dtype, tuple(map(tuple, shapes)), route)
    st = cache.get(key)
    if st is None:
        old = [k for k in list(cache) if isinstance(k, tuple) and k[:1] == ("bn_stats",)]
        for k in old[:-6]:
            del cache[k]
        st = cache[key] = K.zeros_arena(dev, *shapes)
    return st


@K.on_tensor_device
class StgcnLayerFunction(torch.autograd.Function):

    @staticmethod
    def forward(ctx, x, A, wg, bg, n1w, n1b, wt, bt, n2w, n2b, wr, br, nrw, nrb, cfg):
        kt, stride, residual, norm, dtype, sup, packs = (cfg.kt, cfg.stride, cfg.residual, cfg.norm, cfg.dtype,
                                                         cfg.sup, cfg.packs)
        dev = x.device
        x = K.to_rows(x, dtype)
        N, Cin, T, V = x.shape
        P = A.shape[-3]
        Cout = wt.shape[0]
        pad = (kt - 1) // 2
        T_out = (T + 2 * pad - kt) // stride + 1
        M1, M2 = N * T * V, N * T_out * V
        A32 = _f32(A)
        res_conv = residual and not (Cin == Cout and stride == 1)
        cache = cfg.cache.setdefault(("dev", str(dev)), {}) if cfg.cache is not None else None
        bn_finalize = cfg.sync.finalize if cfg.sync is not None else K.bn_finalize

        gather = sup is not None and A32.dim() == 3 and not sup.dense(P)
        if (gather and cfg.infer and ROUTING.fused_inference and norm == LN
                and K.layer_fused_ok(sup, P, Cin, Cout, V, kt, stride, dtype)):
            return fused_layer_forward(x, A32, wg, bg, n1w, n1b, wt, bt, n2w, n2b, residual, dtype, cache=cache)
        if (gather and norm == LN and ROUTING.fused_ln_train and not cfg.infer
                and K.layer_fused_ok(sup, P, Cin, Cout, V, kt, stride, dtype)):
            y, g, u, ls1, ls2, h = fused_layer_forward(x, A32, wg, bg, n1w, n1b, wt, bt, n2w, n2b, residual, dtype,
                                                       cache=cache, train=True, packs=packs)
            ctx.cfg = cfg
            ctx.sup = sup
            ctx.dims = (N, Cin, Cout, T, T_out, V, P, pad, False)
            _save_named(ctx, x=x, A32=A32, XA=None, g=g, u=u, y=y, wg=wg, bg=bg, wt=wt, n1w=n1w, n1b=n1b, n2w=n2w,
                        n2b=n2b, ls1=ls1, ls2=ls2, h=h)
            ctx.in_dtype = A.dtype
            return y
        st1 = st2 = str_ = None
        if norm == BN:
            cpo = -(-Cout // K.col_tile(Cout)) * K.col_tile(Cout)
            rb1 = K.gconv_row_blocks(N * T, V) if gather else K.row_blocks(M1, Cout)
            rb2 = K.row_blocks(M2, Cout)
            st_shapes = [(rb1, cpo, 4), (rb2, cpo, 4)] + ([(K.row_blocks(M2, Cout), cpo, 4)] if res_conv else [])
            st_all = _stats_arena(cache, dev, x.dtype, st_shapes, gather)
            st1, st2 = st_all[0], st_all[1]
            str_ = st_all[2] if res_conv else None
        r = None
        if res_conv:
            wrp, cpr, kpr = packs.wr if packs is not None else K.pack_weight(_f32(wr).view(1, Cout, Cin), dtype)
            r = K.conv_rows(x, wrp, Cin, Cout, cpr, kpr, T, T_out, Kt=1, stride=stride, pad=0, bias=_f32(br),
                            stats=str_)
            if norm == BN:
                strr, scr, shr = bn_finalize(str_, str_.shape[0], cpr, Cout, _f32(nrw), _f32(nrb))
            else:
                strr = K.ln_stats(r, N * T_out, V, Cout)

        if gather:
            if packs is not None and packs.gw is not None:
                wgp, bias2d = packs.gw
            else:
                wgp, bias2d = K.gconv_weights(A32, _f32(wg).reshape(P * Cout, Cin), sup, Cout, Cin, False, dtype,
                                              bias=_f32(bg))
            cpg = wgp.shape[2]
            if norm == BN:
                assert cpg == cpo
            g = K.gconv(x, wgp, sup, Cin, Cout, bias=bias2d, stats=st1)
            XA = None
        else:
            XA, g, cpg = gcn_forward(x, A32, wg, bg, dtype, stats=st1)
        if norm == BN:
            mr1, sc1, sh1 = bn_finalize(st1, st1.shape[0], cpg, Cout, _f32(n1w), _f32(n1b))
            pro1 = dict(pro=1, pro_a=sc1, pro_b=sh1)
        else:
            ls1 = K.ln_stats(g, N * T, V, Cout)
            h = K.ln_apply(g, ls1, _flat_ln(n1w), _flat_ln(n1b), M1, V, Cout, relu=True)
            pro1 = {}

        wtp, cpt, kpt = packs.wt if packs is not None else \
            K.pack_weight(wt.detach().float().squeeze(-1).permute(2, 0, 1), dtype, stride=stride)
        u = K.conv_rows(g if norm == BN else h, wtp, Cout, Cout, cpt, kpt, T, T_out, Kt=kt, stride=stride,
                        pad=pad, bias=_f32(bt), stats=st2, tag=f"tcn_fwd_c{Cout}" if stride == 1 else None, **pro1)

        if norm == BN:
            mr2, sc2, sh2 = bn_finalize(st2, st2.shape[0], cpt, Cout, _f32(n2w), _f32(n2b))
            ybits = torch.empty((M2, Cout // 8), dtype=torch.uint8, device=dev) \
                if (ROUTING.bn_mask_bits and dtype == torch.bfloat16 and K.bn_fused_ok(Cout, dtype) and Cout % 8 == 0) \
                else None
            if res_conv:
                y = K.bn_apply(u, sc2, sh2, M2, Cout, res_mode=2, r=r, rsc=scr, rsh=shr, bits=ybits)
            else:
                y = K.bn_apply(u, sc2, sh2, M2, Cout, res_mode=1 if residual else 0, r=x if residual else None,
                               bits=ybits)
        else:
            ls2 = K.ln_stats(u, N * T_out, V, Cout)
            g2, b2 = _flat_ln(n2w), _flat_ln(n2b)
            if res_conv:
                y = K.ln_apply(u, ls2, g2, b2, M2, V, Cout, res_mode=2, r=r, rst=strr, rg=_flat_ln(nrw),
                               rb=_flat_ln(nrb))
            else:
                y = K.ln_apply(u, ls2, g2, b2, M2, V, Cout, res_mode=1 if residual else 0,
                               r=x if residual else None)

        ctx.cfg = cfg
        ctx.sup = sup if gather else None
        ctx.dims = (N, Cin, Cout, T, T_out, V, P, pad, res_conv)
        saved = dict(x=x, A32=A32, XA=XA, g=g, u=u, y=y, wg=wg, bg=bg, wt=wt, n1w=n1w, n1b=n1b, n2w=n2w, n2b=n2b)
        if norm == BN:
            saved.update(mr1=mr1, sc1=sc1, sh1=sh1, mr2=mr2, ybits=ybits)
        else:
            saved.update(ls1=ls1, ls2=ls2, h=h)
        if res_conv:
            saved.update(r=r, wr=wr, nrw=nrw, nrb=nrb, strr=strr)
        _save_named(ctx, **saved)
        ctx.in_dtype = A.dtype
        return y

    @staticmethod
    def backward(ctx, dy):
        cfg, s = ctx.cfg, _saved(ctx)
        kt, stride, residual, norm, dtype, packs, sync = (cfg.kt, cfg.stride, cfg.residual, cfg.norm, cfg.dtype,
                                                          cfg.packs, cfg.sync)
        N, Cin, Cout, T, T_out, V, P, pad, res_conv = ctx.dims
        x, A32, g, u, y, wg, bg, wt = s.x, s.A32, s.g, s.u, s.y, s.wg, s.bg, s.wt
        st1, st2 = (s.mr1, s.mr2) if norm == BN else (s.ls1, s.ls2)
        ybits = s.ybits if norm == BN else None
        dev = x.device
        dy = K.to_rows(dy, dtype)
        M1, M2 = N * T * V, N * T_out * V
        grads = {}
        zl = {}

        def zero_targets():
            if not zl:
                zl["t"] = K.zeros_arena(dev, (P * Cout, Cin), (P, V, V),
                                        (N, V, Cout) if A32.dim() == 4 else (V, Cout))
            return zl["t"]

        du = K.cl_empty(N, Cout, T_out, V, dtype, dev)
        dx = K.cl_empty(N, Cin, T, V, dtype, dev)
        dx_written = False
        fused = norm == BN and K.bn_fused_ok(Cout, dtype)
        res_in_gconv = fused and residual and not res_conv and ybits is not None and ctx.sup is not None
        if fused:
            kw = dict(mask=1, mref=y, x1=u, mr1=st2, g1=_f32(s.n2w), out1=du, bias_sums=True)
            if ybits is not None:
                kw.update(mask=3, mref=ybits)
            if res_conv:
                dr = K.cl_empty(N, Cout, T_out, V, dtype, dev)
                kw.update(x2=s.r, mr2=s.strr, g2=_f32(s.nrw), out2=dr)
            elif residual and not res_in_gconv:
                kw.update(out2=dx)
                dx_written = True
            sums2, osum2 = K.bn_bwd_fused(dy, M2, Cout, sync=sync, **kw)
            grads["n2w"], grads["n2b"] = sums2[1], sums2[0]
            grads["bt"] = osum2[0]
            if res_conv:
                grads["nrw"], grads["nrb"] = sums2[2], sums2[0].clone()
                grads["br"] = osum2[1]
        else:
            grads["n2w"], grads["n2b"] = _norm_backward(norm, dy, u, st2, s.n2w, s.n2b, du, sync, mask=1, mref=y)

        if res_conv:
            if not fused:
                dr = K.cl_empty(N, Cout, T_out, V, dtype, dev)
                grads["nrw"], grads["nrb"] = _norm_backward(norm, dy, s.r, s.strr, s.nrw, s.nrb, dr, sync,
                                                            mask=1, mref=y)
                grads["br"] = K.bn_bwd_reduce(dr, M2, Cout)[:, 0].clone()
            wrTp, cq, kq = packs.wrT if packs is not None else \
                K.pack_weight(_f32(s.wr).view(Cout, Cin).t().unsqueeze(0), dtype)
            grads["wr"] = K.conv_wgrad_w(x, dr, Cin, Cout, T, T_out, Kt=1, stride=stride, pad=0).view(Cout, Cin, 1, 1)
            K.conv_rows(dr, wrTp, Cout, Cin, cq, kq, T_out, T, Kt=1, stride=stride, pad=0, trans=True, out=dx)
            dx_written = True
        elif residual and not fused:
            K.bn_bwd_apply(dy, M2, Cin, dx, mask=1, mref=y)
            dx_written = True

        wtTp, cq, kq = packs.wtT if packs is not None else \
            K.pack_weight(wt.detach().float().squeeze(-1).permute(2, 1, 0), dtype, stride=stride, trans=True)
        if norm == BN:
            pro1, hin = dict(pro=1, pro_a=s.sc1, pro_b=s.sh1), g
        else:
            pro1 = {}
            hin = s.h if s.h is not None else \
                K.ln_apply(g, st1, _flat_ln(s.n1w), _flat_ln(s.n1b), M1, V, Cout, relu=True)
        grads["wt"] = K.conv_wgrad_w(hin, du, Cout, Cout, T, T_out, Kt=kt, stride=stride, pad=pad,
                                     **pro1).unsqueeze(-1)
        if K.tconv_frame_ok(Cout, kt, stride, V, dtype) and getattr(wtTp, "frag_stride", None) == 1:
            dh = K.tconv_frame(du, wtTp, cq, kq, trans=True)
        else:
            dh = K.conv_rows(du, wtTp, Cout, Cout, cq, kq, T_out, T, Kt=kt, stride=stride, pad=pad, trans=True)
        if not fused:
            grads["bt"] = K.bn_bwd_reduce(du, M2, Cout)[:, 0].clone()

        dg = K.cl_empty(N, Cout, T, V, dtype, dev)
        if fused:
            s1, _ = K.bn_bwd_fused(dh, M1, Cout, mask=2, mref=g, msc=s.sc1, msh=s.sh1, x1=g, mr1=st1,
                                   g1=_f32(s.n1w), out1=dg, sync=sync)
            grads["n1w"], grads["n1b"] = s1[1], s1[0]
        else:
            m1 = dict(mask=2, mref=g, msc=s.sc1, msh=s.sh1) if norm == BN else dict(mask=2)
            grads["n1w"], grads["n1b"] = _norm_backward(norm, dh, g, st1, s.n1w, s.n1b, dg, sync, **m1)

        if ctx.sup is not None:
            sup = ctx.sup
            wg2 = _f32(wg).reshape(P * Cout, Cin)
            dA, grads["wg"], grads["bg"] = _gconv_wgrad_dweff(x, dg, A32, wg2, bg, sup,
                                                              cfg.dense_dA and ctx.needs_input_grad[1], zero_targets,
                                                              dtype)
            wgT = packs.gwT if packs is not None and packs.gwT is not None else \
                K.gconv_weights(A32, wg2, sup, Cout, Cin, True, dtype)
            K.gconv(dg, wgT, sup, Cout, Cin, trans=True, out=dx, accumulate=dx_written,
                    res=(dy, ybits) if res_in_gconv else None)
        else:
            dA, grads["wg"], grads["bg"] = gcn_backward(x, A32, s.XA, wg, bg, dg, dx, dx_written, dtype,
                                                        z_S=zero_targets()[2])

        def gr(name, like):
            v = grads.get(name)
            if v is None or like is None or not like.requires_grad:
                return None
            return v.to(like.dtype).view(like.shape)

        wr_, nrw_, nrb_ = (s.wr, s.nrw, s.nrb) if res_conv else (None, None, None)
        return (dx, dA.to(ctx.in_dtype), gr("wg", wg), gr("bg", bg), gr("n1w", s.n1w), gr("n1b", s.n1b), gr("wt", wt),
                grads["bt"], gr("n2w", s.n2w), gr("n2b", s.n2b), gr("wr", wr_),
                grads.get("br"), gr("nrw", nrw_), gr("nrb", nrb_), None)


def _norm_backward(norm, dy, x, st, gamma, beta, out, sync=None, **mask):
    N, C, T, V = x.shape
    M = N * T * V
    if norm == BN:
        sums = K.bn_bwd_reduce(dy, M, C, x=x, mean_rstd=st, **mask)
        dgamma, dbeta = sums[:, 1].clone(), sums[:, 0].clone()
        if sync is not None:
            sync.all_reduce_sums(sums, M)
        K.bn_bwd_apply(dy, M, C, out, x=x, mean_rstd=st, gamma=_f32(gamma), sums=sums, **mask)
        return dgamma, dbeta
    dgb = torch.zeros((2, C * V), dtype=torch.float32, device=x.device)
    K.ln_bwd(dy, x, st, _flat_ln(gamma), _flat_ln(beta), N * T, V, C, out, dgb=dgb, **mask)
    return dgb[0].view(gamma.shape), dgb[1].view(beta.shape)


def _gconv_wgrad_dweff(x, dg, A32, wg2, bg, sup, dense_dA, zero_targets, dtype):
    N, Cin, T, V = x.shape
    P, Cout = A32.shape[-3], dg.shape[1]
    fuse_s = A32.dim() == 3 and K.gconv_wgrad_rowsum_ok(sup, Cin, Cout, dtype)
    S_rows = torch.empty((V, Cout), dtype=torch.float32, device=x.device) if fuse_s else None
    dweff = K.gconv_wgrad(x, dg, sup, Cin, Cout, rowsum=S_rows)
    if fuse_s and not dense_dA and K.gconv_finish_bias_ok(A32, sup):
        dwg2, dA, dbg = K.gconv_finish_bias(dweff, A32, wg2, sup, Cout, Cin, _f32(bg), S_rows)
        return dA, dwg2, dbg
    z_dwg, z_dA, z_S = zero_targets()
    dwg2, dA = K.gconv_finish(dweff, A32, wg2, sup, Cout, Cin, dW=z_dwg, dA=z_dA)
    if dense_dA:
        dA = K.amix_dA(x, _gcn_dgrad_rows(dg, wg2, P, Cin, Cout, T, dtype), A32)
    dA, dbg = _bias_through_A(dA, A32, bg, dg, S=S_rows, z_S=z_S)
    return dA, dwg2, dbg


@K.on_tensor_device
class GcnFunction(torch.autograd.Function):

    @staticmethod
    def forward(ctx, x, A, wg, bg, dtype):
        x = K.to_rows(x, dtype)
        A32 = _f32(A)
        XA, g, _ = gcn_forward(x, A32, wg, bg, dtype)
        ctx.save_for_backward(x, A32, XA, wg, bg)
        ctx.meta = (dtype, A.dtype)
        return g

    @staticmethod
    def backward(ctx, dg):
        x, A32, XA, wg, bg = ctx.saved_tensors
        dtype, adt = ctx.meta
        dx = K.cl_empty(*x.shape, dtype, x.device)
        dA, dwg, dbg = gcn_backward(x, A32, XA, wg, bg, K.to_rows(dg, dtype), dx, False, dtype)
        return dx, dA.to(adt), dwg.to(wg.dtype), dbg.to(bg.dtype), None


def plan_conv1x1_packs(plan, w, dtype):
    Cout, Ci = w.shape[0], w.shape[1]
    w2 = w.detach().view(Cout, Ci)
    return K.pack_weight(w2.unsqueeze(0), dtype, plan=plan), K.pack_weight(w2.t().unsqueeze(0), dtype, plan=plan)


@K.on_tensor_device
class Conv1x1Function(torch.autograd.Function):

    @staticmethod
    def forward(ctx, x, w, b, dtype, packs=None):
        x = K.to_rows(x, dtype)
        N, Cin, T, V = x.shape
        Cout, Ci = w.shape[0], w.shape[1]
        wp, cp, kp = packs[0] if packs is not None else \
            K.pack_weight(w.detach().float().view(Cout, Ci).unsqueeze(0), dtype)
        y = K.conv_rows(x, wp, Cin, Cout, cp, kp, T, T, bias=_f32(b))
        ctx.save_for_backward(x, w)
        ctx.dtype = dtype
        ctx.packT = packs[1] if packs is not None else None
        return y

    @staticmethod
    def backward(ctx, dy):
        x, w = ctx.saved_tensors
        dtype = ctx.dtype
        N, Cin, T, V = x.shape
        Cout, Ci = w.shape[0], w.shape[1]
        dy = K.to_rows(dy, dtype)
        wT, cq, kq = ctx.packT if ctx.packT is not None else \
            K.pack_weight(w.detach().float().view(Cout, Ci).t().unsqueeze(0), dtype)
        dx = K.conv_rows(dy, wT, Cout, Cin, cq, kq, T, T, trans=True)
        dw = K.conv_wgrad_w(x, dy, Cin, Cout, T, T).view(Cout, Cin, 1, 1)
        if Ci < Cin:
            dw = dw[:, :Ci]
        db = K.bn_bwd_reduce(dy, N * T * V, Cout)[:, 0]
        return dx, dw.to(w.dtype), db.to(w.dtype), None, None


@K.on_tensor_device
class InputBatchNormFunction(torch.autograd.Function):

    @staticmethod
    def forward(ctx, x, w, b, dtype, sync=None):
        x = K.to_rows(x, dtype)
        N, C, T, V = x.shape
        if K.rows_ld(x) != C:
            x = x.contiguous(memory_format=torch.channels_last)
        F_, CV = N * T, V * C
        part, nb, _ = K.bn_stats_partial(x, F_, CV, ld=CV)
        mr, sc, sh = (sync.finalize if sync is not None else K.bn_finalize)(part, nb, CV, CV, w.detach().float(),
                                                                            b.detach().float())
        y = K.cl_empty(N, C, T, V, dtype, x.device)
        K.bn_apply(x, sc, sh, F_, CV, relu=False, out=y, ldu=CV, ldy=CV)
        ctx.save_for_backward(x, w, mr)
        ctx.dtype = dtype
        ctx.sync = sync
        return y

    @staticmethod
# ... 289 lines not shown
```

### realtime-st-gcn_amd/modules.py

```python
from __future__ import annotations

import torch
import torch.nn as nn

from . import layer_fn as F_
from . import native as K
from .syncbn import active_sync

_DTYPES = {"fp32": torch.float32, "bf16": torch.bfloat16, torch.float32: torch.float32,
           torch.bfloat16: torch.bfloat16}


def resolve_dtype(d):
    return _DTYPES[d]


class LayerNorm(nn.Module):

    def __init__(self, normalized_shape, eps=1e-05, elementwise_affine=True, bias=True, device=None, dtype=None):
        super().__init__()
        self.weight = nn.Parameter(torch.ones(normalized_shape, device=device, dtype=dtype))
        self.bias = nn.Parameter(torch.zeros(normalized_shape, device=device, dtype=dtype))
        self.eps = eps
        self.compute_dtype = torch.float32
# ... 13 lines not shown
        return F_.InputBatchNormFunction.apply(x, self.norm.weight, self.norm.bias, self.compute_dtype,
                                               active_sync(self))


def make_norm(normalization, channels, num_joints):
    if normalization == "LayerNorm":
        return LayerNorm([channels, 1, num_joints])
    return nn.BatchNorm2d(channels, track_running_stats=False)


class ConvTemporalGraphical(nn.Module):

    def __init__(self, in_channels, out_channels, kernel_size, partitions, t_kernel_size=1, t_stride=1,
                 t_padding=0, t_dilation=1, bias=True):
        super().__init__()
        if (t_kernel_size, t_stride, t_padding, t_dilation) != (1, 1, 0, 1) or not bias:
            raise NotImplementedError("stgcn_amd: ConvTemporalGraphical supports the reference's only use "
                                      "(t_kernel_size=1, stride 1, no padding/dilation, bias=True)")
        self.out_channels = out_channels
        self.partitions = partitions
        self.kernel_size = kernel_size
        self.conv = nn.Conv2d(in_channels, out_channels * partitions, kernel_size=(t_kernel_size, 1))
        self.compute_dtype = torch.float32

    def forward(self, x, A):
        return F_.GcnFunction.apply(x, A, self.conv.weight, self.conv.bias, self.compute_dtype)


class StgcnLayer(nn.Module):

    def __init__(self, in_channels, out_channels, kernel_size, partitions, num_joints, stride=1, dropout=0,
                 residual=True, normalization="LayerNorm"):
        super().__init__()
        assert len(kernel_size) == 2
        assert kernel_size[0] % 2 == 1
        padding = ((kernel_size[0] - 1) // 2, 0)
        self.kernel_size = kernel_size
        self.stride = stride
        self.dropout = dropout
        self.normalization = normalization
        self.is_residual = residual
        self.is_residual_conv = residual and not ((in_channels == out_channels) and (stride == 1))
        self.gcn = ConvTemporalGraphical(in_channels, out_channels, kernel_size[1], partitions)
        self.tcn = nn.Sequential(
            make_norm(normalization, out_channels, num_joints),
            nn.ReLU(inplace=True),
            nn.Conv2d(out_channels, out_channels, (kernel_size[0], 1), stride=(stride, 1), padding=padding),
            make_norm(normalization, out_channels, num_joints),
            nn.Dropout(dropout, inplace=True))
        if self.is_residual_conv:
            self.residual = nn.Sequential(
                nn.Conv2d(in_channels, out_channels, kernel_size=1, stride=(stride, 1)),
                make_norm(normalization, out_channels, num_joints))
        else:
            self.residual = nn.Identity()
        self.compute_dtype = torch.float32
        self._gsup = None
        self._graph_bound = False
        self._fused_cache = {}

    def _drop_packs(self):
        self._fused_cache.clear()

    def train(self, mode: bool = True):
        self._drop_packs()
        return super().train(mode)

    def _load_from_state_dict(self, *args, **kwargs):
        self._drop_packs()
        return super()._load_from_state_dict(*args, **kwargs)

    def bind_graph(self, A, masked=True):
        s = self._gsup
        if A.dim() == 3 and (s is None or s.V != A.shape[-1] or s.mask.device != A.device):
            self._gsup = K.GraphSupport(A)
        self._graph_bound = self._graph_bound or masked

    def graph_support(self, A):
        if A.dim() != 3:
            return None
        self.bind_graph(A, masked=False)
        return self._gsup

    def forward(self, x, A, packs=None):
        if self.dropout and self.training:
            raise NotImplementedError("stgcn_amd: dropout > 0 in training is not implemented (every reference "
                                      "config uses dropout 0)")
        if not self.is_residual and x.shape[1] != self.tcn[2].out_channels:
            raise RuntimeError("StgcnLayer(residual=False) requires in_channels == out_channels")
        n1, conv, n2 = self.tcn[0], self.tcn[2], self.tcn[3]
        if self.is_residual_conv:
            rc, rn = self.residual[0], self.residual[1]
            wr, br, nrw, nrb = rc.weight, rc.bias, rn.weight, rn.bias
        else:
            wr = br = nrw = nrb = None
        infer = not torch.is_grad_enabled() or not (
            x.requires_grad or A.requires_grad or any(p.requires_grad for p in self.parameters()))
        cfg = F_.LayerCfg(kt=self.kernel_size[0], stride=self.stride, residual=self.is_residual,
                          norm=self.normalization, dtype=self.compute_dtype, sup=self.graph_support(A),
                          dense_dA=not self._graph_bound, infer=infer, cache=self._fused_cache,
                          packs=None if infer else packs, sync=active_sync(self))
        return F_.StgcnLayerFunction.apply(x, A, self.gcn.conv.weight, self.gcn.conv.bias, n1.weight, n1.bias,
                                           conv.weight, conv.bias, n2.weight, n2.bias, wr, br, nrw, nrb, cfg)


def set_compute_dtype(module: nn.Module, dtype):
    dt = resolve_dtype(dtype)
    for m in module.modules():
        if hasattr(m, "compute_dtype"):
            m.compute_dtype = dt
    return module
```

### realtime-st-gcn_amd/native.py

```python
from __future__ import annotations

import ctypes

import torch

from . import _lib as L


class device_of:
    __slots__ = ("idx", "prev")

    def __init__(self, t):
        self.idx = t.device.index if getattr(t, "is_cuda", False) else None
        self.prev = None

    def __enter__(self):
        if self.idx is not None:
            cur = torch._C._cuda_getDevice()
            if cur != self.idx:
                torch._C._cuda_setDevice(self.idx)
                self.prev = cur
        return self

    def __exit__(self, *exc):
# ... 424 lines not shown
    key = (K, w2.device)
    perm = _PERM16.get(key)
    if perm is None:
        h = torch.arange(16) // 8
        j = torch.arange(16) % 8
        within = 8 * (j // 4) + 4 * h + j % 4
        perm = (torch.arange(K) // 16 * 16 + within.repeat(K // 16)).to(w2.device)
        _PERM16[key] = perm
    return pack_frag1(w2.float().index_select(1, perm), dtype)


def gcn_bias_plan(A, b, Cout, plan, M=None):
    A = _dense(A)
    P, V = A.shape[0], A.shape[-1]
    b2 = torch.empty((V, Cout), dtype=torch.float32, device=A.device)
    bc = b.detach()
    plan.add(kind=3, dtype=1, src=bc.view(1, -1), dst=b2, Co=Cout, Ci=1, A=A, M=None if M is None else _dense(M), P=P, V=V,
             bconv=bc, bias2d=b2)
    return b2


def layer_fused_ok(sup, P, Cin, Cout, V, kt, stride, dtype) -> bool:
    return (dtype == torch.bfloat16 and sup is not None and P <= 3 and 16 < V <= 25
            and Cin == 64 and Cout == 64 and kt == 9 and stride == 1)


def layer_fused(x, A, wimg, gbias, wt_packed, tbias, ln, tag=None, residual=False, train=False):
    N, C, T, V = x.shape
    if getattr(wt_packed, "frag_stride", None) != 1:
        raise RuntimeError("stgcn_amd: layer_fused needs the stride-1 fragment image of the temporal weight")
    z = cl_empty(N, C, T, V, x.dtype, x.device)
    A = _dense(A)
    d = L.LayerFusedDesc()
    d.x, d.z, d.wg_frag, d.A = x.data_ptr(), z.data_ptr(), wimg.data_ptr(), A.data_ptr()
    d.gbias, d.wt_frag, d.tbias = L.ptr(gbias), wt_packed.frag_ptr, L.ptr(tbias)
    d.N, d.T, d.V, d.P, d.x_ld, d.z_ld = N, T, V, A.shape[0], rows_ld(x), rows_ld(z)
    ln = [_f32c(t) for t in ln]
    if any(t.numel() != V * C for t in ln):
        raise RuntimeError("stgcn_amd: layer_fused LayerNorm parameters must be [V][64]")
    d.ln1_g, d.ln1_b, d.ln2_g, d.ln2_b = (t.data_ptr() for t in ln)
    d.residual = int(bool(residual))
    d._keep = ln
    if train:
        g = cl_empty(N, C, T, V, x.dtype, x.device)
        u = cl_empty(N, C, T, V, x.dtype, x.device)
        st = torch.empty((2, N * T, 2), dtype=torch.float32, device=x.device)
        d.g_out, d.u_out, d.st1_out, d.st2_out = g.data_ptr(), u.data_ptr(), st[0].data_ptr(), st[1].data_ptr()
        d.g_ld, d.u_ld = rows_ld(g), rows_ld(u)
        hh = cl_empty(N, C, T, V, x.dtype, x.device)
        d.h_out, d.h_ld = hh.data_ptr(), rows_ld(hh)
    _launch("layer_fused", L.lib().stgcn_layer_fused_fwd, d, L.stream(), tag=tag)
    if train:
        return z, g, u, st[0], st[1], hh
    return z


def gconv(x, wpk, sup, Cin, Cout, trans=False, bias=None, stats=None, out=None, accumulate=False, tag=None,
          res=None):
    N, _, T, V = x.shape
    if out is None:
        out = cl_empty(N, Cout, T, V, x.dtype, x.device)
    nbr, deg = (sup.rnbr, sup.rdeg) if trans else (sup.nbr, sup.deg)
    d = L.GconvDesc()
    d.in_, d.out, d.w = x.data_ptr(), out.data_ptr(), wpk.data_ptr()
    d.nbr, d.deg, d.bias, d.stats = nbr.data_ptr(), deg.data_ptr(), L.ptr(bias), L.ptr(stats)
    d.NT, d.V, d.J, d.Cin, d.Cout = N * T, V, sup.J, Cin, Cout
    d.Cin_pad, d.Cout_pad = wpk.shape[3], wpk.shape[2]
    d.in_ld, d.out_ld, d.accumulate = rows_ld(x), rows_ld(out), int(accumulate)
    if res is not None:
        rr, rbits = res
        if accumulate or rbits.dtype != torch.uint8:
            raise RuntimeError("stgcn_amd: gconv's masked residual needs accumulate=False and uint8 sign bits")
        d.res, d.res_bits, d.res_ld = rr.data_ptr(), rbits.data_ptr(), rows_ld(rr)
    _launch("gconv", L.lib().stgcn_gconv, d, L.dtype_code(x.dtype), L.stream(), kinfo=lambda: (
        "gconv_dgrad" if trans else "gconv_fwd", f"{Cin}->{Cout}" if not trans else f"{Cout}->{Cin}",
        2.0 * N * T * sup.nnz * Cin * Cout, x.element_size() * N * T * V * (Cin + Cout * (2 if accumulate else 1))))
    return out


def gconv_wgrad_rowsum_ok(sup, Cin, Cout, dtype) -> bool:
    return dtype == torch.bfloat16 and Cin % 64 == 0 and Cout % 64 == 0 and sup.J <= 5


def gconv_wgrad(x, dy, sup, Cin, Cout, rowsum=None):
    N, _, T, V = x.shape
    dweff = torch.empty((V, sup.J, Cout, Cin), dtype=torch.float32, device=x.device)
    d = L.GconvWgradDesc()
    d.rowsum = L.ptr(rowsum)
    d.x, d.dy, d.nbr, d.deg, d.dweff = x.data_ptr(), dy.data_ptr(), sup.nbr.data_ptr(), sup.deg.data_ptr(), \
        dweff.data_ptr()
    d.NT, d.V, d.J, d.Cin, d.Cout, d.x_ld, d.dy_ld = N * T, V, sup.J, Cin, Cout, rows_ld(x), rows_ld(dy)
    code = L.dtype_code(x.dtype)
    nbytes = L.lib().stgcn_gconv_wgrad_workspace(d, code)
    if nbytes > 0:
        work = torch.empty(nbytes // 4, dtype=torch.float32, device=x.device)
        d.work, d.work_bytes = work.data_ptr(), nbytes
    fn = L.lib().stgcn_gconv_wgrad

    def launches():
        hook = EVENT_HOOK
        if hook and gconv_wgrad3_shape(sup, Cin, Cout, x.dtype):
            d.phase = 1
            hook("gconv_wgrad3", "start", {"flop": 2.0 * N * T * sup.nnz * Cin * Cout,
                                           "bytes": x.element_size() * N * T * V * (Cin + Cout),
                                           "shape": f"{Cin}->{Cout}"})
            L.check(fn(d, code, L.stream()), "gconv_wgrad")
            hook("gconv_wgrad3", "end", None)
            d.phase = 2
        return fn(d, code, L.stream())

    _launch("gconv_wgrad", launches, kinfo=lambda: (
        "gconv_wgrad", f"{Cin}->{Cout}", 2.0 * N * T * sup.nnz * Cin * Cout,
        x.element_size() * N * T * V * (Cin + Cout)))
    return dweff


def gconv_wgrad3_shape(sup, Cin, Cout, dtype) -> bool:
    return dtype == torch.bfloat16 and Cin % 64 == 0 and Cout % 64 == 0 and sup.J <= 5 and not (Cin == 64 and Cout == 128)


def gconv_finish(dweff, A, W, sup, Cout, Cin, dW=None, dA=None):
    A = _dense(A)
    P, V = A.shape[0], A.shape[-1]
    if dW is None:
        dW = torch.zeros((P * Cout, Cin), dtype=torch.float32, device=A.device)
    if dA is None:
        dA = torch.zeros((P, V, V), dtype=torch.float32, device=A.device)
    work = _workspace(L.lib().stgcn_gconv_wgrad_finish_workspace(P, V, sup.J, Cout, Cin), A.device)
    L.check(L.lib().stgcn_gconv_wgrad_finish(dweff.data_ptr(), A.data_ptr(), W.data_ptr(), sup.nbr.data_ptr(),
                                             sup.deg.data_ptr(), P, V, sup.J, Cout, Cin, dW.data_ptr(), dA.data_ptr(),
                                             work.data_ptr(), L.stream()), "gconv_finish")
    return dW, dA


def gconv_finish_bias(dweff, A, W, sup, Cout, Cin, bconv, S):
    A = _dense(A)
    P, V = A.shape[0], A.shape[-1]
    dev = A.device
    out = torch.empty(P * Cout * Cin + P * V * V + P * Cout, dtype=torch.float32, device=dev)
    dW = out[:P * Cout * Cin].view(P * Cout, Cin)
    dA = out[P * Cout * Cin:P * Cout * Cin + P * V * V].view(P, V, V)
    db = out[P * Cout * Cin + P * V * V:]
    work = _workspace(L.lib().stgcn_gconv_wgrad_finish_workspace(P, V, sup.J, Cout, Cin), dev)
    _launch("gconv_finish_bias", L.lib().stgcn_gconv_wgrad_finish_bias, dweff.data_ptr(), A.data_ptr(), W.data_ptr(),
            sup.nbr.data_ptr(), sup.deg.data_ptr(), P, V, sup.J, Cout, Cin, bconv.data_ptr(), S.data_ptr(),
            dW.data_ptr(), dA.data_ptr(), db.data_ptr(), work.data_ptr(), L.stream(),
            kinfo=lambda: ("gconv_wgrad_finish", f"{Cin}->{Cout}", None, 4 * dweff.numel()))
    return dW, dA, db


def gconv_finish_bias_ok(A, sup) -> bool:
    return A.dim() == 3 and A.shape[0] <= 4 and A.shape[-1] <= 32 and A.shape[-1] * sup.J <= 256


def bn_stat_blocks(M: int) -> int:
    return L.lib().stgcn_bn_stat_blocks(M)


def bn_stats_partial(x, M, C, ld=None):
    nb = bn_stat_blocks(M)
    part = torch.empty((nb, C, 4), dtype=torch.float32, device=x.device)
    L.check(L.lib().stgcn_bn_stats_partial(x.data_ptr(), ld or rows_ld(x), M, C, part.data_ptr(),
                                           L.dtype_code(x.dtype), L.stream()), "bn_stats_partial")
    return part, nb, C


def bn_finalize(part, nb, ld_part, C, gamma, beta, eps=1e-5):
    buf = torch.empty(4 * C, dtype=torch.float32, device=part.device)
    mr, sc, sh = buf[:2 * C].view(C, 2), buf[2 * C:3 * C], buf[3 * C:]
    L.check(L.lib().stgcn_bn_finalize(part.data_ptr(), nb, ld_part, C, L.ptr(gamma), L.ptr(beta), eps, mr.data_ptr(),
                                      sc.data_ptr(), sh.data_ptr(), L.stream()), "bn_finalize")
    return mr, sc, sh


def bn_merge(part, nb, ld_part, C):
    out = torch.empty((C, 4), dtype=torch.float32, device=part.device)
    L.check(L.lib().stgcn_bn_merge(part.data_ptr(), nb, ld_part, C, out.data_ptr(), L.stream()), "bn_merge")
    return out


def bn_apply(u, sc, sh, M, C, res_mode=0, r=None, rsc=None, rsh=None, relu=True, out=None, ldu=None, ldy=None,
             bits=None):
    if out is None:
        out = torch.empty_like(u)
    args = (u.data_ptr(), ldu or rows_ld(u), sc.data_ptr(), sh.data_ptr(), res_mode, L.ptr(r),
            rows_ld(r) if r is not None else 0, L.ptr(rsc), L.ptr(rsh), int(relu), out.data_ptr(),
            ldy or rows_ld(out), M, C)

    def kinfo():
        return "bn_apply", f"C{C}", None, u.element_size() * M * C * (3 if r is not None else 2)

    if bits is not None:
        if u.dtype != torch.bfloat16 or C % 8 or bits.dtype != torch.uint8 or bits.numel() < M * (C // 8):
            raise RuntimeError("stgcn_amd: bn_apply bits need bf16 rows, C % 8 == 0 and a uint8 [M][C/8] buffer")
        _launch("bn_apply_bits", L.lib().stgcn_bn_apply_bits, *args, bits.data_ptr(), L.stream(), kinfo=kinfo)
    else:
        _launch("bn_apply", L.lib().stgcn_bn_apply, *args, L.dtype_code(u.dtype), L.stream(), kinfo=kinfo)
    return out


def bn_bwd_reduce(dy, M, C, mask=0, mref=None, msc=None, msh=None, x=None, mean_rstd=None, lddy=None):
    nb = bn_stat_blocks(M)
    part = torch.empty((nb, C, 2), dtype=torch.float32, device=dy.device)
    sums = torch.empty((C, 2), dtype=torch.float32, device=dy.device)
    L.check(L.lib().stgcn_bn_bwd_reduce(dy.data_ptr(), lddy or rows_ld(dy), mask, L.ptr(mref),
                                        rows_ld(mref) if mref is not None else 0, L.ptr(msc), L.ptr(msh), L.ptr(x),
                                        rows_ld(x) if x is not None else 0, L.ptr(mean_rstd), M, C, part.data_ptr(),
                                        sums.data_ptr(), L.dtype_code(dy.dtype), L.stream()), "bn_bwd_reduce")
    return sums


def bn_bwd_apply(dy, M, C, out, mask=0, mref=None, msc=None, msh=None, x=None, mean_rstd=None, gamma=None,
                 sums=None, accumulate=False, lddy=None):
    L.check(L.lib().stgcn_bn_bwd_apply(dy.data_ptr(), lddy or rows_ld(dy), mask, L.ptr(mref),
                                       rows_ld(mref) if mref is not None else 0, L.ptr(msc), L.ptr(msh), L.ptr(x),
                                       rows_ld(x) if x is not None else 0, L.ptr(mean_rstd), L.ptr(gamma),
                                       L.ptr(sums), M, C, out.data_ptr(), rows_ld(out), int(accumulate),
                                       L.dtype_code(dy.dtype), L.stream()), "bn_bwd_apply")
    return out


def bn_fused_ok(C: int, dtype) -> bool:
    vec = 8 if dtype == torch.bfloat16 else 4
    return C % vec == 0 and C // vec <= 256


# ... 456 lines not shown
```

### realtime-st-gcn_amd/parallel.py

```python
from __future__ import annotations

import contextlib
from dataclasses import dataclass
from typing import Optional

import torch


def rank_slice(n_units: int, world: int, rank: int):
    base, extra = divmod(n_units, world)
    start = rank * base + min(rank, extra)
    return start, start + base + (1 if rank < extra else 0)


def windows_for_rank(trial: torch.Tensor, W: int, world: int, rank: int) -> torch.Tensor:
    _, C, L, V = trial.shape
    s, e = rank_slice(L, world, rank)
    padded = torch.nn.functional.pad(trial, (0, 0, W - 1, 0))
    win = padded[:, :, s:e + W - 1].unfold(2, W, 1)
    return win.permute(0, 2, 1, 4, 3).reshape(e - s, C, W, V)


def chunk_bounds(L: int, chunk: int, overlap: int):
    if chunk <= overlap:
        raise ValueError("chunk must exceed the overlap")
    out, s = [], 0
    while True:
        e = min(L, s + chunk)
        out.append((s, e))
        if e == L:
            return out
        s = e - overlap


def chunks_for_rank(L: int, chunk: int, overlap: int, world: int, rank: int):
    b = chunk_bounds(L, chunk, overlap)
    s, e = rank_slice(len(b), world, rank)
    return b[s:e]


@dataclass
class SegmentShard:
    prev: Optional[torch.Tensor]
    den: torch.Tensor
    pairs: int
    rank_first: bool

    @staticmethod
    def local(pred_full, labels_full, weight, start, end, L, rank):
        prev = pred_full[0, :, start - 1].detach() if start > 0 else None
        den = weight[labels_full.reshape(-1).to(weight.device)].sum()
        return SegmentShard(prev, den, L - 1, start == 0)


def exchange_shard(pred_local, labels_full, weight, start, L, group=None):
    import torch.distributed as dist

    world = dist.get_world_size(group)
    rank = dist.get_rank(group)
    C = pred_local.shape[1]
    last = pred_local[0, :, -1].detach().float() if pred_local.shape[2] > 0 else \
        torch.zeros((C,), device=pred_local.device)
    rows = [torch.empty_like(last) for _ in range(world)]
    dist.all_gather(rows, last.contiguous(), group=group)
    prev = rows[rank - 1] if start > 0 else None
    den = weight[labels_full.reshape(-1).to(weight.device)].sum()
    return SegmentShard(prev, den, L - 1, start == 0)


def sharded_loss(crit, i, pred_local, labels_local, shard: SegmentShard, world: int):
    if pred_local.shape[2] == 0:
        z = pred_local.sum() * 0.0
        return z, z
    ce, mse = crit(i, pred_local, labels_local, shard=shard)
    return ce * world, mse * world


def ddp(model: torch.nn.Module, device: torch.device, bucket_cap_mb: int = 4):
    from torch.nn.parallel import DistributedDataParallel as DDP
    ids = [device.index] if device.type == "cuda" else None
    return DDP(model, device_ids=ids, bucket_cap_mb=bucket_cap_mb, gradient_as_bucket_view=True)


@contextlib.contextmanager
def accumulate(model, last: bool):
    if not last and hasattr(model, "no_sync"):
        with model.no_sync():
            yield
    else:
        yield


@dataclass
class SegmentUnit:
    trial: int
    i: int
    count: int
    n0: int
    nw: int
    y0: int
    y1: int


def segment_units(lengths, W: int, segment: int):
    from .segment import window_segments
    out = []
    for k, L in enumerate(lengths):
        segs = window_segments(L, L + W - 1, L, W, segment)
        for i, (sx, ex, sy, ey) in enumerate(segs):
            out.append(SegmentUnit(k, i, len(segs), sx, ex - sx - (W - 1), sy, ey))
    return out


def units_for_rank(units, world: int, rank: int):
    return units[rank::world]


class GraphedStep:

    def __init__(self, fwd_loss, params, opt, world: int = 1, group=None, bucket_mb=None, capture: bool = True):
        self.fwd_loss, self.params, self.opt = fwd_loss, list(params), opt
        self.world, self.group = world, group
        self.capture = capture
        if not capture and bucket_mb is None:
            raise ValueError("GraphedStep(capture=False) needs bucket_mb (the flat mode is graph-only)")
        self.flat = None
        self.buckets = None
        dev = self.params[0].device
        s = torch.cuda.Stream(device=dev)
        s.wait_stream(torch.cuda.current_stream(dev))
        with torch.cuda.stream(s):
            self.opt.zero_grad(set_to_none=False)
            self.fwd_loss().backward()
            self.used = [p for p in self.params if p.grad is not None]
            self.numels = [p.numel() for p in self.used]
            if bucket_mb is not None:
                self._make_buckets(bucket_mb)
                for flat, _ in self.buckets:
                    self._allreduce(flat)
                self._apply()
                self.g1, self.g2 = None, None
                if capture:
                    self.g1 = torch.cuda.CUDAGraph()
                    with torch.cuda.graph(self.g1, stream=s, capture_error_mode="thread_local"):
                        self.loss = self._bucketed_step()
            else:
                if world > 1:
                    self.flat = torch.zeros(sum(self.numels), device=dev)
                    torch.cat([p.grad.reshape(-1) for p in self.used], out=self.flat)
                    self._allreduce(self.flat)
                self._apply()
                self.g1, self.g2 = torch.cuda.CUDAGraph(), torch.cuda.CUDAGraph()
                for p in self.used:
                    p.grad = None
                with torch.cuda.graph(self.g1, stream=s):
                    self.loss = self._fwd_bwd()
                if any(p.grad is None for p in self.used):
                    raise RuntimeError("GraphedStep: a parameter lost its gradient in the captured step")
                with torch.cuda.graph(self.g2, stream=s):
                    self._apply()
        torch.cuda.current_stream(dev).wait_stream(s)

# ... 95 lines not shown
```

### realtime-st-gcn_amd/routing.py

```python
import os


class _Routing:
    def __init__(self):
        e = os.environ.get
        self.fused_inference = e("STGCN_FUSED", "1") != "0"
        self.fused_ln_train = e("STGCN_FUSED_LN_TRAIN", "1") != "0"
        self.bn_mask_bits = e("STGCN_BN_BITS", "1") != "0"
        self.prep_plan = e("STGCN_PREP_PLAN", "1") != "0"
        self.rt_one_launch = e("STGCN_RT_ONE_LAUNCH", "1") != "0"


ROUTING = _Routing()
```

### realtime-st-gcn_amd/stgcn.py

```python
from __future__ import annotations

import torch
import torch.nn as nn
import torch.nn.functional as F

from . import layer_fn as LF
from . import native as K
from .graph import Graph
from .modules import BatchNorm1d, LayerNorm, StgcnLayer, resolve_dtype
from .routing import ROUTING
from .segment import WindowBatch

IN_PAD = 8


class Model(nn.Module):
    def __init__(self, rank=None, **kwargs):
        super().__init__()
        conf = kwargs["st-gcn"]
        self.graph = Graph(strategy=kwargs["strategy"], **kwargs["graph"])
        A = torch.tensor(self.graph.A, dtype=torch.float32, requires_grad=False).contiguous()
        self.register_buffer("A", A)
        kernel_size = (conf["kernel"], kwargs["graph"]["num_node"])
        self.normalization = kwargs["normalization"]
        self.norm_in = (LayerNorm([kwargs["in_feat"], 1, A.size(1)]) if kwargs["normalization"] == "LayerNorm"
                        else BatchNorm1d(kwargs["in_feat"] * A.size(1), track_running_stats=False))
        self.fcn_in = nn.Conv2d(in_channels=conf["in_feat"], out_channels=conf["in_ch"][0], kernel_size=1)
        self.gcn_networks = nn.ModuleList([
            StgcnLayer(in_channels=conf["in_ch"][i], out_channels=conf["out_ch"][i], kernel_size=kernel_size,
                       partitions=A.size(0), num_joints=A.size(1), stride=conf["stride"][i],
                       residual=not not conf["residual"][i], dropout=conf["dropout"][i],
                       normalization=kwargs["normalization"])
            for i in range(conf["layers"])])
        if conf["importance"]:
            self.edge_importance = nn.ParameterList([nn.Parameter(torch.ones(self.A.size()))
                                                     for _ in self.gcn_networks])
        else:
            self.edge_importance = [1] * len(self.gcn_networks)
        self.fcn_out = nn.Conv2d(conf["out_ch"][-1], out_channels=kwargs["num_classes"], kernel_size=1)
        self.compute_dtype = torch.float32
        self._plan = None

    def set_compute_dtype(self, dtype):
        dt = resolve_dtype(dtype)
        self.compute_dtype = dt
        for layer in self.gcn_networks:
            for m in layer.modules():
                if hasattr(m, "compute_dtype"):
                    m.compute_dtype = dt
        return self

    def _prepared(self):
        if not (ROUTING.prep_plan and torch.is_grad_enabled() and self.A.is_cuda) or getattr(self, "_is_replica",
                                                                                              False):
            return None
        dt = self.compute_dtype
        imp = isinstance(self.edge_importance, nn.ParameterList) and len(self.edge_importance)
        key = (dt, self.A.data_ptr(), tuple(p.data_ptr() for p in self.parameters()))
        plan = self._plan
        if plan is None or plan.key != key:
            with K.device_of(self.A):
                plan = K.PrepPlan(self.A.device, key)
                plan.layers = []
                for i, gcn in enumerate(self.gcn_networks):
                    gcn.bind_graph(self.A)
                    plan.layers.append(LF.plan_layer_packs(plan, gcn, self.A, self.edge_importance[i] if imp else None,
                                                           dt))
                plan.head = (LF.plan_conv1x1_packs(plan, self.fcn_in.weight, dt),
                             LF.plan_conv1x1_packs(plan, self.fcn_out.weight, dt))
                plan.finalize()
            self._plan = plan
        with K.device_of(self.A):
            plan.run()
        return plan

    def stage_windows(self, xb: WindowBatch):
        return LF.stage_window_batch(xb, self.norm_in, self.fcn_in, self.compute_dtype)

    def forward(self, x):
        plan = self._prepared()
        if isinstance(x, WindowBatch):
            x = self.stage_windows(x)
        else:
            x = self.norm_in(x)
            C = x.shape[1]
            if C % IN_PAD:
                x = F.pad(x.permute(0, 2, 3, 1), (0, IN_PAD - C % IN_PAD)).permute(0, 3, 1, 2)
            x = LF.Conv1x1Function.apply(x, self.fcn_in.weight, self.fcn_in.bias, self.compute_dtype,
                                         plan.head[0] if plan is not None else None)
        if isinstance(self.edge_importance, nn.ParameterList) and len(self.edge_importance):
            A_eff = (self.A * torch.stack(list(self.edge_importance))).unbind(0)
        else:
            A_eff = [self.A * m for m in self.edge_importance]
        for i, (gcn, A_i) in enumerate(zip(self.gcn_networks, A_eff)):
            gcn.bind_graph(self.A)
            x = gcn(x, A_i, packs=plan.layers[i] if plan is not None else None)
        x = LF.PoolFunction.apply(x, self.compute_dtype)
        x = LF.Conv1x1Function.apply(x, self.fcn_out.weight, self.fcn_out.bias, self.compute_dtype,
                                     plan.head[1] if plan is not None else None)
        return x.squeeze(-1).float()

    def prepare_benchmark(self, arch_conf):
        return arch_conf
```

Baseline: 2.574 million skeleton-frames/s.

## Defer graph-conv weight-gradient tail kernels into one batched end-of-backward launch

Adds a tail-job queue that collects the per-layer reduction and finish kernels of the graph-conv weight gradient (slab reduce, rowpart sum, dW/dA/db finish). These are flushed once per backward through an autograd engine callback as a single level-ordered job-table launch. It also computes the edge-importance gradient directly when edge importance is owned, avoiding autograd ops. The aim is to cut many small kernel launches and Python dispatch per layer in eager mode. In exchange it adds a host-to-device table upload, pinned buffers, and complex conditions around autograd task ids and graph capture.

Result: no change. 2.599 million skeleton-frames/s, median of 6 (+1.0%).

```diff
diff --git a/include/stgcn_amd.h b/include/stgcn_amd.h
--- a/include/stgcn_amd.h
+++ b/include/stgcn_amd.h
@@ -108,6 +108,7 @@
 
 int stgcn_gconv_wgrad(const stgcn_gconv_wgrad_desc* d, int dtype, void* stream);
 long stgcn_gconv_wgrad_workspace(const stgcn_gconv_wgrad_desc* d, int dtype);
+int stgcn_gconv_wgrad_tail(const stgcn_gconv_wgrad_desc* d, int dtype, int* R, long* slab_off, long* rowpart_off);
 long stgcn_gconv_wgrad_finish_workspace(int P, int V, int J, int Cout, int Cin);
 int stgcn_gconv_wgrad_finish_bias(const float* dweff, const float* A, const float* W, const int* nbr, const int* deg,
                                   int P, int V, int J, int Cout, int Cin, const float* bconv, const float* S, float* dW,
@@ -564,6 +565,25 @@
 int stgcn_prep_run(const stgcn_prep_job* jobs_dev, const long* block_start_dev, int njobs, long nblocks,
                    void* stream);
 
+typedef struct {
+  int kind, R, P, V, J, C, nch, pad_;
+  long E, EC, blocks;
+  const float* src;
+  const float* A;
+  const float* W;
+  const float* b;
+  const float* S;
+  const float* A0;
+  const int* nbr;
+  const int* deg;
+  float* dst;
+  float* dst2;
+  float* dst3;
+} stgcn_tail_job;
+int stgcn_tails_check(stgcn_tail_job* jobs, int njobs);
+int stgcn_tails_run(const stgcn_tail_job* jobs_dev, const long* block_start_dev, int njobs, long nblocks,
+                    void* stream);
+
 #define STGCN_ADAM_MAXT 256
 typedef struct {
   float* p;
diff --git a/realtime-st-gcn_amd/__init__.py b/realtime-st-gcn_amd/__init__.py
--- a/realtime-st-gcn_amd/__init__.py
+++ b/realtime-st-gcn_amd/__init__.py
@@ -1,4 +1,4 @@
-from . import _lib, data, loss, metrics, native, optim, parallel, routing, segment, syncbn
+from . import _lib, data, loss, metrics, native, optim, parallel, routing, segment, syncbn, tails
 from .syncbn import convert_sync_batchnorm, revert_sync_batchnorm
 from .graph import Graph, PKU_MMD
 from .modules import BatchNorm1d, ConvTemporalGraphical, LayerNorm, StgcnLayer, set_compute_dtype
diff --git a/realtime-st-gcn_amd/_lib.py b/realtime-st-gcn_amd/_lib.py
--- a/realtime-st-gcn_amd/_lib.py
+++ b/realtime-st-gcn_amd/_lib.py
@@ -78,6 +78,12 @@
                [(n, c_void_p) for n in ("src", "dst", "dst_frag", "A", "M", "nbr", "deg")] + \
                [(n, c_int) for n in ("P", "V", "J", "R_pad", "C_pad", "pad_")] + \
                [(n, c_void_p) for n in ("bconv", "bias2d")]
+
+
+class TailJob(ctypes.Structure):
+    _fields_ = [(n, c_int) for n in ("kind", "R", "P", "V", "J", "C", "nch", "pad_")] + \
+               [(n, c_long) for n in ("E", "EC", "blocks")] + \
+               [(n, c_void_p) for n in ("src", "A", "W", "b", "S", "A0", "nbr", "deg", "dst", "dst2", "dst3")]
 
 
 RT_MAX_LAYERS = 12
@@ -196,6 +202,8 @@
                                                                                            c_int, c_void_p]),
     "stgcn_gconv_wgrad": (c_int, [ctypes.POINTER(GconvWgradDesc), c_int, c_void_p]),
     "stgcn_gconv_wgrad_workspace": (c_long, [ctypes.POINTER(GconvWgradDesc), c_int]),
+    "stgcn_gconv_wgrad_tail": (c_int, [ctypes.POINTER(GconvWgradDesc), c_int, ctypes.POINTER(c_int),
+                                       ctypes.POINTER(c_long), ctypes.POINTER(c_long)]),
     "stgcn_gconv_wgrad_finish_workspace": (ctypes.c_long, [c_int] * 5),
     "stgcn_gconv_wgrad_finish": (c_int, [c_void_p] * 5 + [c_int] * 5 + [c_void_p, c_void_p, c_void_p, c_void_p]),
     "stgcn_gconv_wgrad_finish_bias": (c_int, [c_void_p] * 5 + [c_int] * 5 + [c_void_p] * 7),
@@ -308,6 +316,8 @@
     "stgcn_seg_loss_bwd": (c_int, [c_void_p, c_void_p, c_void_p, c_void_p, c_long, c_void_p, c_void_p]),
     "stgcn_prep_check": (c_int, [ctypes.POINTER(PrepJob), c_int]),
     "stgcn_prep_run": (c_int, [c_void_p, c_void_p, c_int, c_long, c_void_p]),
+    "stgcn_tails_check": (c_int, [ctypes.POINTER(TailJob), c_int]),
+    "stgcn_tails_run": (c_int, [c_void_p, c_void_p, c_int, c_long, c_void_p]),
     "stgcn_adam_blocks": (ctypes.c_long, [c_long]),
     "stgcn_adam_step": (c_int, [c_void_p, c_int, c_long, c_void_p, c_void_p] + [ctypes.c_double] * 5 + [c_void_p]),
 }
diff --git a/realtime-st-gcn_amd/csrc/capi.cpp b/realtime-st-gcn_amd/csrc/capi.cpp
--- a/realtime-st-gcn_amd/csrc/capi.cpp
+++ b/realtime-st-gcn_amd/csrc/capi.cpp
@@ -126,6 +126,12 @@
   if (!d || (dtype != 0 && dtype != 1)) return 0;
   return gconv_wgrad_workspace(*d, dtype);
 }
+int stgcn_gconv_wgrad_tail(const stgcn_gconv_wgrad_desc* d, int dtype, int* R, long* slab_off, long* rowpart_off) {
+  if (!d || !R || !slab_off || !rowpart_off || (dtype != 0 && dtype != 1) || d->V <= 0 || d->J <= 0 || d->Cin <= 0 ||
+      d->Cout <= 0 || d->NT <= 0)
+    return 0;
+  return gconv_wgrad_tail(*d, dtype, R, slab_off, rowpart_off);
+}
 int stgcn_gconv_wgrad(const stgcn_gconv_wgrad_desc* d, int dtype, void* stream) {
   CHECK_DTYPE(dtype);
   if (!d || !d->x || !d->dy || !d->nbr || !d->deg || !d->dweff || d->NT <= 0 || d->V <= 0 || d->J <= 0 ||
diff --git a/realtime-st-gcn_amd/csrc/gconv_finish.hip b/realtime-st-gcn_amd/csrc/gconv_finish.hip
--- a/realtime-st-gcn_amd/csrc/gconv_finish.hip
+++ b/realtime-st-gcn_amd/csrc/gconv_finish.hip
@@ -1,5 +1,6 @@
 #include "common.h"
 #include "launchers.h"
+#include "tail_ops.h"
 
 namespace {
 
@@ -36,97 +37,13 @@
   }
 }
 
-constexpr int PMAX = 4;
-constexpr int DW_PAIRS = 32 * 8;
-DEV void gconv_dw_all_body(const float* __restrict__ dweff, const float* __restrict__ A, const int* nbr,
-                           const int* deg, int P, int V, int J, long E, float* dW, long bb, bool acc_out) {
-  __shared__ int spair[DW_PAIRS];
-  __shared__ float scoef[DW_PAIRS][PMAX];
-  __shared__ int snp;
-  if (threadIdx.x == 0) {
-    int n = 0;
-    for (int w = 0; w < V; ++w)
-      for (int j = 0; j < deg[w]; ++j) spair[n++] = w * J + j;
-    snp = n;
-  }
-  __syncthreads();
-  const int np = snp;
-  for (int i = threadIdx.x; i < np * PMAX; i += 256) {
-    const int k = i / PMAX, p = i % PMAX;
-    const int pr = spair[k], w = pr / J;
-    scoef[k][p] = p < P ? A[((long)p * V + nbr[pr]) * V + w] : 0.f;
-  }
-  __syncthreads();
-  const int g = threadIdx.x >> 6;
-  const long e = (bb * 64 + (threadIdx.x & 63)) * 4;
-  float4 acc[PMAX];
-#pragma unroll
-  for (int p = 0; p < PMAX; ++p) acc[p] = make_float4(0.f, 0.f, 0.f, 0.f);
-  if (e < E) {
-#pragma unroll 4
-    for (int k = g; k < np; k += 4) {
-      const float4 d = *reinterpret_cast<const float4*>(dweff + (long)spair[k] * E + e);
-#pragma unroll
-      for (int p = 0; p < PMAX; ++p) {
-        const float c = scoef[k][p];
-        acc[p].x += c * d.x; acc[p].y += c * d.y; acc[p].z += c * d.z; acc[p].w += c * d.w;
-      }
-    }
-  }
-  __shared__ float4 part[4][PMAX][64];
-#pragma unroll
-  for (int p = 0; p < PMAX; ++p) part[g][p][threadIdx.x & 63] = acc[p];
-  __syncthreads();
-  if (threadIdx.x < 64 && e < E) {
-    const int l = threadIdx.x;
-#pragma unroll
-    for (int p = 0; p < PMAX; ++p)
-      if (p < P) {
-        const float4 a0 = part[0][p][l], a1 = part[1][p][l], a2 = part[2][p][l], a3 = part[3][p][l];
-        float4 t = make_float4(((a0.x + a1.x) + a2.x) + a3.x, ((a0.y + a1.y) + a2.y) + a3.y,
-                               ((a0.z + a1.z) + a2.z) + a3.z, ((a0.w + a1.w) + a2.w) + a3.w);
-        float4* o = reinterpret_cast<float4*>(dW + (long)p * E + e);
-        if (acc_out) {
-          const float4 q = *o;
-          t.x += q.x; t.y += q.y; t.z += q.z; t.w += q.w;
-        }
-        *o = t;
-      }
-  }
-}
+constexpr int PMAX = TAIL_PMAX, DW_PAIRS = TAIL_DW_PAIRS, DA_CHUNK = TAIL_DA_CHUNK, FV_MAX = TAIL_FV_MAX;
 __global__ __launch_bounds__(256) void gconv_dw_all_kernel(const float* __restrict__ dweff, const float* __restrict__ A,
                                                            const int* nbr, const int* deg, int P, int V, int J, long E,
                                                            float* dW) {
   gconv_dw_all_body(dweff, A, nbr, deg, P, V, J, E, dW, blockIdx.x, true);
 }
 
-constexpr int DA_CHUNK = 2048;
-DEV void gconv_dA_part_body(const float* __restrict__ dweff, const float* __restrict__ W, const int* deg, int P, int J,
-                           long E, float* part, int pair, int c, int nch) {
-  if (pair % J >= deg[pair / J]) return;
-  const float* d = dweff + (long)pair * E;
-  float acc[PMAX] = {0.f, 0.f, 0.f, 0.f};
-  const long e1 = min(E, (long)(c + 1) * DA_CHUNK);
-  for (long e = (long)c * DA_CHUNK + threadIdx.x * 4; e < e1; e += 1024) {
-    const float4 dv = *reinterpret_cast<const float4*>(d + e);
-#pragma unroll
-    for (int p = 0; p < PMAX; ++p)
-      if (p < P) {
-        const float4 w = *reinterpret_cast<const float4*>(W + (long)p * E + e);
-        acc[p] += ((w.x * dv.x + w.y * dv.y) + w.z * dv.z) + w.w * dv.w;
-      }
-  }
-  __shared__ float red[4][PMAX];
-#pragma unroll
-  for (int p = 0; p < PMAX; ++p) {
-    const float t = wave_sum(acc[p]);
-    if ((threadIdx.x & 63) == 0) red[threadIdx.x >> 6][p] = t;
-  }
-  __syncthreads();
-  if (threadIdx.x < P)
-    part[((long)pair * nch + c) * PMAX + threadIdx.x] =
-        ((red[0][threadIdx.x] + red[1][threadIdx.x]) + red[2][threadIdx.x]) + red[3][threadIdx.x];
-}
 __global__ __launch_bounds__(256) void gconv_dA_part_kernel(const float* __restrict__ dweff, const float* __restrict__ W,
                                                             const int* deg, int P, int J, long E, float* part) {
   gconv_dA_part_body(dweff, W, deg, P, J, E, part, blockIdx.x, blockIdx.y, gridDim.y);
@@ -145,47 +62,11 @@
   }
 }
 
-constexpr int FV_MAX = 32;
 __global__ __launch_bounds__(256) void gconv_finish2_kernel(const float* __restrict__ part, const float* __restrict__ A,
                                                             const float* __restrict__ b, const float* __restrict__ S,
                                                             const int* nbr, const int* deg, int P, int V, int J, int C,
                                                             int nch, float* dA, float* db) {
-  const int bx = blockIdx.x;
-  if (bx < P * V) {
-    const int p = bx / V, w = bx % V;
-    float t = 0.f;
-    for (int c = threadIdx.x; c < C; c += 256) t += b[p * C + c] * S[w * C + c];
-    t = wave_sum(t);
-    __shared__ float red[4];
-    __shared__ float sup[FV_MAX];
-    if ((threadIdx.x & 63) == 0) red[threadIdx.x >> 6] = t;
-    if (threadIdx.x < V) sup[threadIdx.x] = 0.f;
-    __syncthreads();
-    const float tot = ((red[0] + red[1]) + red[2]) + red[3];
-    if (threadIdx.x < deg[w]) {
-      const int j = threadIdx.x, pair = w * J + j;
-      float s = 0.f;
-      for (int c = 0; c < nch; ++c) s += part[((long)pair * nch + c) * PMAX + p];
-      sup[nbr[pair]] = s;
-    }
-    __syncthreads();
-    for (int v = threadIdx.x; v < V; v += 256) dA[(p * V + v) * V + w] = sup[v] + tot;
-    return;
-  }
-  __shared__ float cs[PMAX * FV_MAX];
-  for (int i = threadIdx.x; i < P * V; i += 256) {
-    const int p = i / V, w = i % V;
-    float t = 0.f;
-    for (int v = 0; v < V; ++v) t += A[(p * V + v) * V + w];
-    cs[i] = t;
-  }
-  __syncthreads();
-  const int i = (bx - P * V) * 256 + threadIdx.x;
-  if (i >= P * C) return;
-  const int p = i / C, c = i % C;
-  float t = 0.f;
-  for (int w = 0; w < V; ++w) t += cs[p * V + w] * S[w * C + c];
-  db[i] = t;
+  gconv_finish2_body(part, A, b, S, nbr, deg, P, V, J, C, nch, dA, db, nullptr, nullptr, blockIdx.x);
 }
 
 __global__ void gconv_dA_reduce_kernel(const float* __restrict__ part, const int* nbr, const int* deg, int P, int V,
diff --git a/realtime-st-gcn_amd/csrc/gconv_wgrad.hip b/realtime-st-gcn_amd/csrc/gconv_wgrad.hip
--- a/realtime-st-gcn_amd/csrc/gconv_wgrad.hip
+++ b/realtime-st-gcn_amd/csrc/gconv_wgrad.hip
@@ -1,6 +1,7 @@
 #include "common.h"
 #include "launchers.h"
 #include "lds_ops.h"
+#include "tail_ops.h"
 #include "../../include/stgcn_amd.h"
 
 namespace {
@@ -736,43 +737,18 @@
   a.dweff[idx] = s;
 }
 
-__global__ void rowpart_sum_kernel(const float* __restrict__ part, int R, long E, float* __restrict__ out) {
-  const long e = (long)blockIdx.x * blockDim.x + threadIdx.x;
-  if (e >= E) return;
-  float s = 0.f;
-  for (int r = 0; r < R; ++r) s += part[(long)r * E + e];
-  out[e] = s;
-}
-
 __global__ void gslab_rowpart_kernel(const float* __restrict__ slab, int R, long E, long EC, const int* deg, int J,
                                      float* __restrict__ dweff, int nb1, const float* __restrict__ rpart, long ER,
                                      float* __restrict__ rowsum) {
-  if ((int)blockIdx.x < nb1) {
-    const long e = (long)blockIdx.x * blockDim.x + threadIdx.x;
-    if (e >= E) return;
-    const int pair = (int)(e / EC);
-    float s = 0.f;
-    if (pair % J < deg[pair / J])
-      for (int r = 0; r < R; ++r) s += slab[(long)r * E + e];
-    dweff[e] = s;
-    return;
-  }
-  const long e = (long)(blockIdx.x - nb1) * blockDim.x + threadIdx.x;
-  if (e >= ER) return;
-  float s = 0.f;
-  for (int r = 0; r < R; ++r) s += rpart[(long)r * ER + e];
-  rowsum[e] = s;
+  if ((int)blockIdx.x < nb1)
+    gslab_reduce_body(slab, R, E, EC, deg, J, dweff, (long)blockIdx.x * blockDim.x + threadIdx.x);
+  else
+    rowpart_sum_body(rpart, R, ER, rowsum, (long)(blockIdx.x - nb1) * blockDim.x + threadIdx.x);
 }
 
 __global__ void gslab_reduce_kernel(const float* __restrict__ slab, int R, long E, long EC, const int* deg, int J,
                                     float* __restrict__ out) {
-  const long e = (long)blockIdx.x * blockDim.x + threadIdx.x;
-  if (e >= E) return;
-  const int pair = (int)(e / EC);
-  float s = 0.f;
-  if (pair % J < deg[pair / J])
-    for (int r = 0; r < R; ++r) s += slab[(long)r * E + e];
-  out[e] = s;
+  gslab_reduce_body(slab, R, E, EC, deg, J, out, (long)blockIdx.x * blockDim.x + threadIdx.x);
 }
 
 enum WgradKernel {
@@ -879,6 +855,15 @@
 
 long gconv_wgrad_workspace(const stgcn_gconv_wgrad_desc& a, int dtype) { return plan_wgrad(a, dtype).total; }
 
+int gconv_wgrad_tail(const stgcn_gconv_wgrad_desc& a, int dtype, int* R, long* slab_off, long* rowpart_off) {
+  const WgradPlan p = plan_wgrad(a, dtype);
+  if (p.direct || !p.slab_floats) return 0;
+  *R = (int)p.g.R;
+  *slab_off = p.slab_off;
+  *rowpart_off = p.rowpart_floats ? p.rowpart_off : -1;
+  return 1;
+}
+
 int gconv_wgrad_launch(const stgcn_gconv_wgrad_desc& a, int dtype, hipStream_t s) {
   const long E = (long)a.V * a.J * a.Cout * a.Cin;
   if (a.phase < 0 || a.phase > 2) return STGCN_EBADSHAPE;
diff --git a/realtime-st-gcn_amd/csrc/launchers.h b/realtime-st-gcn_amd/csrc/launchers.h
--- a/realtime-st-gcn_amd/csrc/launchers.h
+++ b/realtime-st-gcn_amd/csrc/launchers.h
@@ -28,6 +28,7 @@
                          const float* bconv = nullptr, float* bias2d = nullptr);
 long gconv_wgrad_workspace(const stgcn_gconv_wgrad_desc& a, int dtype);
 int gconv_wgrad_launch(const stgcn_gconv_wgrad_desc& a, int dtype, hipStream_t s);
+int gconv_wgrad_tail(const stgcn_gconv_wgrad_desc& a, int dtype, int* R, long* slab_off, long* rowpart_off);
 int gconv_wgrad_finish_launch(const float* dweff, const float* A, const float* W, const int* nbr, const int* deg,
                               int P, int V, int J, int Cout, int Cin, float* dW, float* dA, void* work, hipStream_t s);
 long gconv_wgrad_finish_workspace(int P, int V, int J, int Cout, int Cin);
diff --git a/realtime-st-gcn_amd/csrc/tail_ops.h b/realtime-st-gcn_amd/csrc/tail_ops.h
--- /dev/null
+++ b/realtime-st-gcn_amd/csrc/tail_ops.h
@@ -0,0 +1,156 @@
+#pragma once
+#include "common.h"
+
+constexpr int TAIL_PMAX = 4;
+constexpr int TAIL_DW_PAIRS = 32 * 8;
+constexpr int TAIL_DA_CHUNK = 2048;
+constexpr int TAIL_FV_MAX = 32;
+
+DEV void gslab_reduce_body(const float* __restrict__ slab, int R, long E, long EC, const int* deg, int J,
+                           float* __restrict__ out, long e) {
+  if (e >= E) return;
+  const int pair = (int)(e / EC);
+  float s = 0.f;
+  if (pair % J < deg[pair / J])
+    for (int r = 0; r < R; ++r) s += slab[(long)r * E + e];
+  out[e] = s;
+}
+
+DEV void rowpart_sum_body(const float* __restrict__ part, int R, long E, float* __restrict__ out, long e) {
+  if (e >= E) return;
+  float s = 0.f;
+  for (int r = 0; r < R; ++r) s += part[(long)r * E + e];
+  out[e] = s;
+}
+
+DEV void gconv_dw_all_body(const float* __restrict__ dweff, const float* __restrict__ A, const int* nbr,
+                           const int* deg, int P, int V, int J, long E, float* dW, long bb, bool acc_out) {
+  constexpr int PMAX = TAIL_PMAX;
+  __shared__ int spair[TAIL_DW_PAIRS];
+  __shared__ float scoef[TAIL_DW_PAIRS][PMAX];
+  __shared__ int snp;
+  if (threadIdx.x == 0) {
+    int n = 0;
+    for (int w = 0; w < V; ++w)
+      for (int j = 0; j < deg[w]; ++j) spair[n++] = w * J + j;
+    snp = n;
+  }
+  __syncthreads();
+  const int np = snp;
+  for (int i = threadIdx.x; i < np * PMAX; i += 256) {
+    const int k = i / PMAX, p = i % PMAX;
+    const int pr = spair[k], w = pr / J;
+    scoef[k][p] = p < P ? A[((long)p * V + nbr[pr]) * V + w] : 0.f;
+  }
+  __syncthreads();
+  const int g = threadIdx.x >> 6;
+  const long e = (bb * 64 + (threadIdx.x & 63)) * 4;
+  float4 acc[PMAX];
+#pragma unroll
+  for (int p = 0; p < PMAX; ++p) acc[p] = make_float4(0.f, 0.f, 0.f, 0.f);
+  if (e < E) {
+#pragma unroll 4
+    for (int k = g; k < np; k += 4) {
+      const float4 d = *reinterpret_cast<const float4*>(dweff + (long)spair[k] * E + e);
+#pragma unroll
+      for (int p = 0; p < PMAX; ++p) {
+        const float c = scoef[k][p];
+        acc[p].x += c * d.x; acc[p].y += c * d.y; acc[p].z += c * d.z; acc[p].w += c * d.w;
+      }
+    }
+  }
+  __shared__ float4 part[4][PMAX][64];
+#pragma unroll
+  for (int p = 0; p < PMAX; ++p) part[g][p][threadIdx.x & 63] = acc[p];
+  __syncthreads();
+  if (threadIdx.x < 64 && e < E) {
+    const int l = threadIdx.x;
+#pragma unroll
+    for (int p = 0; p < PMAX; ++p)
+      if (p < P) {
+        const float4 a0 = part[0][p][l], a1 = part[1][p][l], a2 = part[2][p][l], a3 = part[3][p][l];
+        float4 t = make_float4(((a0.x + a1.x) + a2.x) + a3.x, ((a0.y + a1.y) + a2.y) + a3.y,
+                               ((a0.z + a1.z) + a2.z) + a3.z, ((a0.w + a1.w) + a2.w) + a3.w);
+        float4* o = reinterpret_cast<float4*>(dW + (long)p * E + e);
+        if (acc_out) {
+          const float4 q = *o;
+          t.x += q.x; t.y += q.y; t.z += q.z; t.w += q.w;
+        }
+        *o = t;
+      }
+  }
+}
+
+DEV void gconv_dA_part_body(const float* __restrict__ dweff, const float* __restrict__ W, const int* deg, int P, int J,
+                            long E, float* part, int pair, int c, int nch) {
+  constexpr int PMAX = TAIL_PMAX;
+  if (pair % J >= deg[pair / J]) return;
+  const float* d = dweff + (long)pair * E;
+  float acc[PMAX] = {0.f, 0.f, 0.f, 0.f};
+  const long e1 = min(E, (long)(c + 1) * TAIL_DA_CHUNK);
+  for (long e = (long)c * TAIL_DA_CHUNK + threadIdx.x * 4; e < e1; e += 1024) {
+    const float4 dv = *reinterpret_cast<const float4*>(d + e);
+#pragma unroll
+    for (int p = 0; p < PMAX; ++p)
+      if (p < P) {
+        const float4 w = *reinterpret_cast<const float4*>(W + (long)p * E + e);
+        acc[p] += ((w.x * dv.x + w.y * dv.y) + w.z * dv.z) + w.w * dv.w;
+      }
+  }
+  __shared__ float red[4][PMAX];
+#pragma unroll
+  for (int p = 0; p < PMAX; ++p) {
+    const float t = wave_sum(acc[p]);
+    if ((threadIdx.x & 63) == 0) red[threadIdx.x >> 6][p] = t;
+  }
+  __syncthreads();
+  if (threadIdx.x < P)
+    part[((long)pair * nch + c) * PMAX + threadIdx.x] =
+        ((red[0][threadIdx.x] + red[1][threadIdx.x]) + red[2][threadIdx.x]) + red[3][threadIdx.x];
+}
+
+DEV void gconv_finish2_body(const float* __restrict__ part, const float* __restrict__ A, const float* __restrict__ b,
+                            const float* __restrict__ S, const int* nbr, const int* deg, int P, int V, int J, int C,
+                            int nch, float* dA, float* db, const float* __restrict__ A0, float* dM, int bx) {
+  constexpr int PMAX = TAIL_PMAX;
+  if (bx < P * V) {
+    const int p = bx / V, w = bx % V;
+    float t = 0.f;
+    for (int c = threadIdx.x; c < C; c += 256) t += b[p * C + c] * S[w * C + c];
+    t = wave_sum(t);
+    __shared__ float red[4];
+    __shared__ float sup[TAIL_FV_MAX];
+    if ((threadIdx.x & 63) == 0) red[threadIdx.x >> 6] = t;
+    if (threadIdx.x < V) sup[threadIdx.x] = 0.f;
+    __syncthreads();
+    const float tot = ((red[0] + red[1]) + red[2]) + red[3];
+    if (threadIdx.x < deg[w]) {
+      const int j = threadIdx.x, pair = w * J + j;
+      float s = 0.f;
+      for (int c = 0; c < nch; ++c) s += part[((long)pair * nch + c) * PMAX + p];
+      sup[nbr[pair]] = s;
+    }
+    __syncthreads();
+    for (int v = threadIdx.x; v < V; v += 256) {
+      const int i = (p * V + v) * V + w;
+      const float g = sup[v] + tot;
+      dA[i] = g;
+      if (dM) dM[i] = g * A0[i];
+    }
+    return;
+  }
+  __shared__ float cs[PMAX * TAIL_FV_MAX];
+  for (int i = threadIdx.x; i < P * V; i += 256) {
+    const int p = i / V, w = i % V;
+    float t = 0.f;
+    for (int v = 0; v < V; ++v) t += A[(p * V + v) * V + w];
+    cs[i] = t;
+  }
+  __syncthreads();
+  const int i = (bx - P * V) * 256 + threadIdx.x;
+  if (i >= P * C) return;
+  const int p = i / C, c = i % C;
+  float t = 0.f;
+  for (int w = 0; w < V; ++w) t += cs[p * V + w] * S[w * C + c];
+  db[i] = t;
+}
diff --git a/realtime-st-gcn_amd/csrc/tails.hip b/realtime-st-gcn_amd/csrc/tails.hip
--- /dev/null
+++ b/realtime-st-gcn_amd/csrc/tails.hip
@@ -0,0 +1,84 @@
+#include "common.h"
+#include "tail_ops.h"
+#include "../../include/stgcn_amd.h"
+
+namespace {
+
+constexpr int TAILS_LDS_STARTS = 512;
+
+__global__ __launch_bounds__(256) void tails_kernel(const stgcn_tail_job* __restrict__ jobs,
+                                                    const long* __restrict__ start, int njobs) {
+  const long b = blockIdx.x;
+  __shared__ long sst[TAILS_LDS_STARTS];
+  const bool lds = njobs <= TAILS_LDS_STARTS;
+  if (lds) {
+    for (int t = threadIdx.x; t < njobs; t += blockDim.x) sst[t] = start[t];
+    __syncthreads();
+  }
+  int lo = 0, hi = njobs - 1;
+  while (lo < hi) {
+    const int mid = (lo + hi + 1) >> 1;
+    if ((lds ? sst[mid] : start[mid]) <= b) lo = mid;
+    else hi = mid - 1;
+  }
+  lo = __builtin_amdgcn_readfirstlane(lo);
+  const stgcn_tail_job& j = jobs[lo];
+  const long bb = b - (lds ? sst[lo] : start[lo]);
+  if (bb >= j.blocks) return;
+  if (j.kind == 0) {
+    gslab_reduce_body(j.src, j.R, j.E, j.EC, j.deg, j.J, j.dst, bb * 256 + threadIdx.x);
+  } else if (j.kind == 1) {
+    rowpart_sum_body(j.src, j.R, j.E, j.dst, bb * 256 + threadIdx.x);
+  } else if (j.kind == 2) {
+    gconv_dw_all_body(j.src, j.A, j.nbr, j.deg, j.P, j.V, j.J, j.E, j.dst, bb, false);
+  } else if (j.kind == 3) {
+    gconv_dA_part_body(j.src, j.W, j.deg, j.P, j.J, j.E, j.dst, (int)(bb / j.nch), (int)(bb % j.nch), j.nch);
+  } else {
+    gconv_finish2_body(j.src, j.A, j.b, j.S, j.nbr, j.deg, j.P, j.V, j.J, j.C, j.nch, j.dst, j.dst2, j.A0, j.dst3,
+                       (int)bb);
+  }
+}
+
+}
+
+extern "C" int stgcn_tails_check(stgcn_tail_job* jobs, int njobs) {
+  if (!jobs || njobs <= 0) return STGCN_EBADSHAPE;
+  for (int k = 0; k < njobs; ++k) {
+    stgcn_tail_job& j = jobs[k];
+    if (!j.src || !j.dst || j.E <= 0) return STGCN_EBADSHAPE;
+    if (j.kind == 0) {
+      if (j.R <= 0 || j.EC <= 0 || j.E % j.EC || !j.deg || j.J <= 0 || (j.E / j.EC) % j.J) return STGCN_EBADSHAPE;
+      j.blocks = (j.E + 255) / 256;
+    } else if (j.kind == 1) {
+      if (j.R <= 0) return STGCN_EBADSHAPE;
+      j.blocks = (j.E + 255) / 256;
+    } else if (j.kind >= 2 && j.kind <= 4) {
+      if (j.P <= 0 || j.P > TAIL_PMAX || j.V <= 0 || j.V > TAIL_FV_MAX || j.J <= 0 || j.V * j.J > TAIL_DW_PAIRS ||
+          j.E % 4 || !j.deg)
+        return STGCN_EBADSHAPE;
+      const long nch = (j.E + TAIL_DA_CHUNK - 1) / TAIL_DA_CHUNK;
+      if (j.kind == 2) {
+        if (!j.A || !j.nbr) return STGCN_EBADSHAPE;
+        j.blocks = (j.E + 255) / 256;
+      } else if (j.kind == 3) {
+        if (!j.W || j.nch != nch) return STGCN_EBADSHAPE;
+        j.blocks = (long)j.V * j.J * nch;
+      } else {
+        if (!j.A || !j.b || !j.S || !j.nbr || !j.dst2 || j.C <= 0 || j.nch != nch || (j.dst3 && !j.A0))
+          return STGCN_EBADSHAPE;
+        j.blocks = (long)j.P * j.V + ((long)j.P * j.C + 255) / 256;
+      }
+    } else {
+      return STGCN_EBADSHAPE;
+    }
+  }
+  return STGCN_OK;
+}
+
+extern "C" int stgcn_tails_run(const stgcn_tail_job* jobs_dev, const long* block_start_dev, int njobs, long nblocks,
+                               void* stream) {
+  if (!jobs_dev || !block_start_dev || njobs <= 0 || nblocks <= 0 || nblocks > 0x7fffffffL) return STGCN_EBADSHAPE;
+  hipLaunchKernelGGL(tails_kernel, dim3((unsigned)nblocks), dim3(256), 0, (hipStream_t)stream, jobs_dev,
+                     block_start_dev, njobs);
+  return hipGetLastError() == hipSuccess ? STGCN_OK : STGCN_EHIP;
+}
diff --git a/realtime-st-gcn_amd/layer_fn.py b/realtime-st-gcn_amd/layer_fn.py
--- a/realtime-st-gcn_amd/layer_fn.py
+++ b/realtime-st-gcn_amd/layer_fn.py
@@ -6,6 +6,7 @@
 import torch
 
 from . import native as K
+from . import tails
 from .routing import ROUTING
 from .syncbn import active_sync
 
@@ -24,6 +25,8 @@
     cache: dict = None
     packs: object = None
     sync: object = None
+    defer: bool = True
+    dM_out: object = None
 
 
 class RtLayerCfg(NamedTuple):
@@ -191,7 +194,7 @@
 class StgcnLayerFunction(torch.autograd.Function):
 
     @staticmethod
-    def forward(ctx, x, A, wg, bg, n1w, n1b, wt, bt, n2w, n2b, wr, br, nrw, nrb, cfg):
+    def forward(ctx, x, A, wg, bg, n1w, n1b, wt, bt, n2w, n2b, wr, br, nrw, nrb, cfg, M=None, A0=None):
         kt, stride, residual, norm, dtype, sup, packs = (cfg.kt, cfg.stride, cfg.residual, cfg.norm, cfg.dtype,
                                                          cfg.sup, cfg.packs)
         dev = x.device
@@ -219,7 +222,7 @@
             ctx.sup = sup
             ctx.dims = (N, Cin, Cout, T, T_out, V, P, pad, False)
             _save_named(ctx, x=x, A32=A32, XA=None, g=g, u=u, y=y, wg=wg, bg=bg, wt=wt, n1w=n1w, n1b=n1b, n2w=n2w,
-                        n2b=n2b, ls1=ls1, ls2=ls2, h=h)
+                        n2b=n2b, ls1=ls1, ls2=ls2, h=h, M=M, A0=A0)
             ctx.in_dtype = A.dtype
             return y
         st1 = st2 = str_ = None
@@ -290,7 +293,8 @@
         ctx.cfg = cfg
         ctx.sup = sup if gather else None
         ctx.dims = (N, Cin, Cout, T, T_out, V, P, pad, res_conv)
-        saved = dict(x=x, A32=A32, XA=XA, g=g, u=u, y=y, wg=wg, bg=bg, wt=wt, n1w=n1w, n1b=n1b, n2w=n2w, n2b=n2b)
+        saved = dict(x=x, A32=A32, XA=XA, g=g, u=u, y=y, wg=wg, bg=bg, wt=wt, n1w=n1w, n1b=n1b, n2w=n2w, n2b=n2b,
+                     M=M, A0=A0)
         if norm == BN:
             saved.update(mr1=mr1, sc1=sc1, sh1=sh1, mr2=mr2, ybits=ybits)
         else:
@@ -390,9 +394,14 @@
         if ctx.sup is not None:
             sup = ctx.sup
             wg2 = _f32(wg).reshape(P * Cout, Cin)
-            dA, grads["wg"], grads["bg"] = _gconv_wgrad_dweff(x, dg, A32, wg2, bg, sup,
-                                                              cfg.dense_dA and ctx.needs_input_grad[1], zero_targets,
-                                                              dtype)
+            want_dM = s.M is not None and s.M.requires_grad
+            dM_slot = None if getattr(ctx, "dM_slot_used", False) else cfg.dM_out
+            ctx.dM_slot_used = True
+            defer = tails.queue(dev) if not ctx.needs_input_grad[1] and \
+                tails.can_defer(cfg, (wg, bg) + ((s.M,) if want_dM else ())) else None
+            dA, grads["wg"], grads["bg"], dM = _gconv_wgrad_dweff(
+                x, dg, A32, wg2, bg, sup, cfg.dense_dA and ctx.needs_input_grad[1], zero_targets, dtype,
+                defer=defer, A0=s.A0 if want_dM else None, dM_out=dM_slot)
             wgT = packs.gwT if packs is not None and packs.gwT is not None else \
                 K.gconv_weights(A32, wg2, sup, Cout, Cin, True, dtype)
             K.gconv(dg, wgT, sup, Cout, Cin, trans=True, out=dx, accumulate=dx_written,
@@ -400,6 +409,9 @@
         else:
             dA, grads["wg"], grads["bg"] = gcn_backward(x, A32, s.XA, wg, bg, dg, dx, dx_written, dtype,
                                                         z_S=zero_targets()[2])
+            dM = dM_slot = None
+        if dM is None and s.M is not None and s.M.requires_grad:
+            dM = torch.mul(dA, s.A0, out=dM_slot).view(dA.shape) if dM_slot is not None else (dA * s.A0).to(s.M.dtype)
 
         def gr(name, like):
             v = grads.get(name)
@@ -408,9 +420,10 @@
             return v.to(like.dtype).view(like.shape)
 
         wr_, nrw_, nrb_ = (s.wr, s.nrw, s.nrb) if res_conv else (None, None, None)
-        return (dx, dA.to(ctx.in_dtype), gr("wg", wg), gr("bg", bg), gr("n1w", s.n1w), gr("n1b", s.n1b), gr("wt", wt),
+        return (dx, dA.to(ctx.in_dtype) if ctx.needs_input_grad[1] else None, gr("wg", wg), gr("bg", bg),
+                gr("n1w", s.n1w), gr("n1b", s.n1b), gr("wt", wt),
                 grads["bt"], gr("n2w", s.n2w), gr("n2b", s.n2b), gr("wr", wr_),
-                grads.get("br"), gr("nrw", nrw_), gr("nrb", nrb_), None)
+                grads.get("br"), gr("nrw", nrw_), gr("nrb", nrb_), None, dM, None)
 
 
 def _norm_backward(norm, dy, x, st, gamma, beta, out, sync=None, **mask):
@@ -428,21 +441,29 @@
     return dgb[0].view(gamma.shape), dgb[1].view(beta.shape)
 
 
-def _gconv_wgrad_dweff(x, dg, A32, wg2, bg, sup, dense_dA, zero_targets, dtype):
+def _gconv_wgrad_dweff(x, dg, A32, wg2, bg, sup, dense_dA, zero_targets, dtype, defer=None, A0=None, dM_out=None):
     N, Cin, T, V = x.shape
     P, Cout = A32.shape[-3], dg.shape[1]
     fuse_s = A32.dim() == 3 and K.gconv_wgrad_rowsum_ok(sup, Cin, Cout, dtype)
+    one_finish = fuse_s and not dense_dA and K.gconv_finish_bias_ok(A32, sup)
+    if not one_finish:
+        defer = None
+    tails.STATS["deferred" if defer is not None else "immediate"] += 1
     S_rows = torch.empty((V, Cout), dtype=torch.float32, device=x.device) if fuse_s else None
-    dweff = K.gconv_wgrad(x, dg, sup, Cin, Cout, rowsum=S_rows)
-    if fuse_s and not dense_dA and K.gconv_finish_bias_ok(A32, sup):
+    dweff = K.gconv_wgrad(x, dg, sup, Cin, Cout, rowsum=S_rows, defer=defer)
+    if one_finish:
+        if defer is not None:
+            dwg2, dA, dbg, dM = K.gconv_finish_bias(dweff, A32, wg2, sup, Cout, Cin, _f32(bg), S_rows, defer=defer,
+                                                    A0=A0, poison=ROUTING.poison_deferred, dM=dM_out)
+            return dA, dwg2, dbg, dM
         dwg2, dA, dbg = K.gconv_finish_bias(dweff, A32, wg2, sup, Cout, Cin, _f32(bg), S_rows)
-        return dA, dwg2, dbg
+        return dA, dwg2, dbg, None
     z_dwg, z_dA, z_S = zero_targets()
     dwg2, dA = K.gconv_finish(dweff, A32, wg2, sup, Cout, Cin, dW=z_dwg, dA=z_dA)
     if dense_dA:
         dA = K.amix_dA(x, _gcn_dgrad_rows(dg, wg2, P, Cin, Cout, T, dtype), A32)
     dA, dbg = _bias_through_A(dA, A32, bg, dg, S=S_rows, z_S=z_S)
-    return dA, dwg2, dbg
+    return dA, dwg2, dbg, None
 
 
 @K.on_tensor_device
diff --git a/realtime-st-gcn_amd/modules.py b/realtime-st-gcn_amd/modules.py
--- a/realtime-st-gcn_amd/modules.py
+++ b/realtime-st-gcn_amd/modules.py
@@ -119,7 +119,7 @@
         self.bind_graph(A, masked=False)
         return self._gsup
 
-    def forward(self, x, A, packs=None):
+    def forward(self, x, A, packs=None, M=None, A0=None, defer=True, dM_out=None):
         if self.dropout and self.training:
             raise NotImplementedError("stgcn_amd: dropout > 0 in training is not implemented (every reference "
                                       "config uses dropout 0)")
@@ -132,13 +132,14 @@
         else:
             wr = br = nrw = nrb = None
         infer = not torch.is_grad_enabled() or not (
-            x.requires_grad or A.requires_grad or any(p.requires_grad for p in self.parameters()))
+            x.requires_grad or A.requires_grad or (M is not None and M.requires_grad)
+            or any(p.requires_grad for p in self.parameters()))
         cfg = F_.LayerCfg(kt=self.kernel_size[0], stride=self.stride, residual=self.is_residual,
                           norm=self.normalization, dtype=self.compute_dtype, sup=self.graph_support(A),
                           dense_dA=not self._graph_bound, infer=infer, cache=self._fused_cache,
-                          packs=None if infer else packs, sync=active_sync(self))
+                          packs=None if infer else packs, sync=active_sync(self), defer=defer, dM_out=dM_out)
         return F_.StgcnLayerFunction.apply(x, A, self.gcn.conv.weight, self.gcn.conv.bias, n1.weight, n1.bias,
-                                           conv.weight, conv.bias, n2.weight, n2.bias, wr, br, nrw, nrb, cfg)
+                                           conv.weight, conv.bias, n2.weight, n2.bias, wr, br, nrw, nrb, cfg, M, A0)
 
 
 def set_compute_dtype(module: nn.Module, dtype):
diff --git a/realtime-st-gcn_amd/native.py b/realtime-st-gcn_amd/native.py
--- a/realtime-st-gcn_amd/native.py
+++ b/realtime-st-gcn_amd/native.py
@@ -530,7 +530,7 @@
     return dtype == torch.bfloat16 and Cin % 64 == 0 and Cout % 64 == 0 and sup.J <= 5
 
 
-def gconv_wgrad(x, dy, sup, Cin, Cout, rowsum=None):
+def gconv_wgrad(x, dy, sup, Cin, Cout, rowsum=None, defer=None):
     N, _, T, V = x.shape
     dweff = torch.empty((V, sup.J, Cout, Cin), dtype=torch.float32, device=x.device)
     d = L.GconvWgradDesc()
@@ -544,10 +544,21 @@
         work = torch.empty(nbytes // 4, dtype=torch.float32, device=x.device)
         d.work, d.work_bytes = work.data_ptr(), nbytes
     fn = L.lib().stgcn_gconv_wgrad
+    if defer is not None:
+        R, so, ro = ctypes.c_int(), ctypes.c_long(), ctypes.c_long()
+        if L.lib().stgcn_gconv_wgrad_tail(d, code, ctypes.byref(R), ctypes.byref(so), ctypes.byref(ro)):
+            E = V * sup.J * Cout * Cin
+            j = L.TailJob(kind=0, R=R.value, J=sup.J, E=E, EC=Cout * Cin, src=work.data_ptr() + so.value,
+                          deg=sup.deg.data_ptr(), dst=dweff.data_ptr())
+            defer.add(0, j, work, sup.deg, dweff)
+            if ro.value >= 0:
+                defer.add(0, L.TailJob(kind=1, R=R.value, E=V * Cout, src=work.data_ptr() + ro.value,
+                                       dst=rowsum.data_ptr()), rowsum)
+        d.phase = 1
 
     def launches():
         hook = EVENT_HOOK
-        if hook and gconv_wgrad3_shape(sup, Cin, Cout, x.dtype):
+        if defer is None and hook and gconv_wgrad3_shape(sup, Cin, Cout, x.dtype):
             d.phase = 1
             hook("gconv_wgrad3", "start", {"flop": 2.0 * N * T * sup.nnz * Cin * Cout,
                                            "bytes": x.element_size() * N * T * V * (Cin + Cout),
@@ -581,15 +592,39 @@
     return dW, dA
 
 
-def gconv_finish_bias(dweff, A, W, sup, Cout, Cin, bconv, S):
+def gconv_finish_bias(dweff, A, W, sup, Cout, Cin, bconv, S, defer=None, A0=None, poison=False, dM=None):
     A = _dense(A)
     P, V = A.shape[0], A.shape[-1]
     dev = A.device
-    out = torch.empty(P * Cout * Cin + P * V * V + P * Cout, dtype=torch.float32, device=dev)
-    dW = out[:P * Cout * Cin].view(P * Cout, Cin)
-    dA = out[P * Cout * Cin:P * Cout * Cin + P * V * V].view(P, V, V)
-    db = out[P * Cout * Cin + P * V * V:]
+    nW, nA = P * Cout * Cin, P * V * V
+    out = torch.empty(nW + nA + P * Cout + (nA if defer is not None and A0 is not None and dM is None else 0),
+                      dtype=torch.float32, device=dev)
+    dW = out[:nW].view(P * Cout, Cin)
+    dA = out[nW:nW + nA].view(P, V, V)
+    db = out[nW + nA:nW + nA + P * Cout]
     work = _workspace(L.lib().stgcn_gconv_wgrad_finish_workspace(P, V, sup.J, Cout, Cin), dev)
+    if defer is not None:
+        if A0 is None:
+            dM = None
+        elif dM is None:
+            dM = out[nW + nA + P * Cout:].view(P, V, V)
+        elif not (dM.is_contiguous() and dM.dtype == torch.float32 and dM.shape == (P, V, V)):
+            raise RuntimeError("stgcn_amd: the edge-importance gradient buffer must be contiguous fp32 [P][V][V]")
+        if poison:
+            out.fill_(float("nan"))
+            if dM is not None:
+                dM.fill_(float("nan"))
+        E = Cout * Cin
+        geo = dict(P=P, V=V, J=sup.J, E=E, nbr=sup.nbr.data_ptr(), deg=sup.deg.data_ptr())
+        nch = -(-E // 2048)
+        defer.add(1, L.TailJob(kind=2, src=dweff.data_ptr(), A=A.data_ptr(), dst=dW.data_ptr(), **geo),
+                  dweff, A, sup.nbr, sup.deg, out)
+        defer.add(1, L.TailJob(kind=3, src=dweff.data_ptr(), W=W.data_ptr(), nch=nch, dst=work.data_ptr(), **geo),
+                  W, work)
+        defer.add(2, L.TailJob(kind=4, src=work.data_ptr(), A=A.data_ptr(), b=bconv.data_ptr(), S=S.data_ptr(), C=Cout,
+                               nch=nch, dst=dA.data_ptr(), dst2=db.data_ptr(), A0=L.ptr(A0), dst3=L.ptr(dM), **geo),
+                  bconv, S, A0, dM)
+        return dW, dA, db, None if dM is None else dM.view(P, V, V)
     _launch("gconv_finish_bias", L.lib().stgcn_gconv_wgrad_finish_bias, dweff.data_ptr(), A.data_ptr(), W.data_ptr(),
             sup.nbr.data_ptr(), sup.deg.data_ptr(), P, V, sup.J, Cout, Cin, bconv.data_ptr(), S.data_ptr(),
             dW.data_ptr(), dA.data_ptr(), db.data_ptr(), work.data_ptr(), L.stream(),
diff --git a/realtime-st-gcn_amd/parallel.py b/realtime-st-gcn_amd/parallel.py
--- a/realtime-st-gcn_amd/parallel.py
+++ b/realtime-st-gcn_amd/parallel.py
@@ -78,6 +78,9 @@
 
 def ddp(model: torch.nn.Module, device: torch.device, bucket_cap_mb: int = 4):
     from torch.nn.parallel import DistributedDataParallel as DDP
+    for m in model.modules():
+        if hasattr(m, "deferred_tails"):
+            m.deferred_tails = False
     ids = [device.index] if device.type == "cuda" else None
     return DDP(model, device_ids=ids, bucket_cap_mb=bucket_cap_mb, gradient_as_bucket_view=True)
 
diff --git a/realtime-st-gcn_amd/routing.py b/realtime-st-gcn_amd/routing.py
--- a/realtime-st-gcn_amd/routing.py
+++ b/realtime-st-gcn_amd/routing.py
@@ -9,6 +9,8 @@
         self.bn_mask_bits = e("STGCN_BN_BITS", "1") != "0"
         self.prep_plan = e("STGCN_PREP_PLAN", "1") != "0"
         self.rt_one_launch = e("STGCN_RT_ONE_LAUNCH", "1") != "0"
+        self.deferred_tails = e("STGCN_DEFERRED_TAILS", "1") != "0"
+        self.poison_deferred = False
 
 
 ROUTING = _Routing()
diff --git a/realtime-st-gcn_amd/stgcn.py b/realtime-st-gcn_amd/stgcn.py
--- a/realtime-st-gcn_amd/stgcn.py
+++ b/realtime-st-gcn_amd/stgcn.py
@@ -6,6 +6,7 @@
 
 from . import layer_fn as LF
 from . import native as K
+from . import tails
 from .graph import Graph
 from .modules import BatchNorm1d, LayerNorm, StgcnLayer, resolve_dtype
 from .routing import ROUTING
@@ -40,6 +41,7 @@
         self.fcn_out = nn.Conv2d(conf["out_ch"][-1], out_channels=kwargs["num_classes"], kernel_size=1)
         self.compute_dtype = torch.float32
         self._plan = None
+        self.deferred_tails = True
 
     def set_compute_dtype(self, dtype):
         dt = resolve_dtype(dtype)
@@ -88,13 +90,24 @@
                 x = F.pad(x.permute(0, 2, 3, 1), (0, IN_PAD - C % IN_PAD)).permute(0, 3, 1, 2)
             x = LF.Conv1x1Function.apply(x, self.fcn_in.weight, self.fcn_in.bias, self.compute_dtype,
                                          plan.head[0] if plan is not None else None)
-        if isinstance(self.edge_importance, nn.ParameterList) and len(self.edge_importance):
-            A_eff = (self.A * torch.stack(list(self.edge_importance))).unbind(0)
+        if self.A.is_cuda:
+            tails.discard_stale(self.A.device)
+        imp = isinstance(self.edge_importance, nn.ParameterList) and len(self.edge_importance)
+        defer = ROUTING.deferred_tails and self.deferred_tails
+        own = imp and defer and torch.is_grad_enabled() and self.A.is_cuda and \
+            all(m.grad is None for m in self.edge_importance)
+        if imp:
+            with torch.set_grad_enabled(not own):
+                A_eff = (self.A * torch.stack(list(self.edge_importance))).unbind(0)
         else:
             A_eff = [self.A * m for m in self.edge_importance]
+        dM_all = torch.empty((len(A_eff),) + tuple(self.A.shape), dtype=torch.float32, device=self.A.device) \
+            if own else None
         for i, (gcn, A_i) in enumerate(zip(self.gcn_networks, A_eff)):
             gcn.bind_graph(self.A)
-            x = gcn(x, A_i, packs=plan.layers[i] if plan is not None else None)
+            x = gcn(x, A_i, packs=plan.layers[i] if plan is not None else None, defer=defer,
+                    M=self.edge_importance[i] if own else None, A0=self.A if own else None,
+                    dM_out=dM_all[i] if own else None)
         x = LF.PoolFunction.apply(x, self.compute_dtype)
         x = LF.Conv1x1Function.apply(x, self.fcn_out.weight, self.fcn_out.bias, self.compute_dtype,
                                      plan.head[1] if plan is not None else None)
diff --git a/realtime-st-gcn_amd/tails.py b/realtime-st-gcn_amd/tails.py
--- /dev/null
+++ b/realtime-st-gcn_amd/tails.py
@@ -0,0 +1,141 @@
+from __future__ import annotations
+
+import ctypes
+
+import torch
+
+from . import _lib as L
+from .routing import ROUTING
+
+LEVELS = 3
+JOB_BYTES = ctypes.sizeof(L.TailJob)
+STATS = {"deferred": 0, "immediate": 0, "flushes": 0, "uploads": 0, "discarded": 0}
+
+_queues = {}
+_tables = {}
+_captured = []
+_spares = []
+SPARE_BYTES = 1 << 16
+
+
+class _Table:
+
+    def __init__(self, device, nbytes, host=None):
+        cap = max(SPARE_BYTES, 1 << (nbytes - 1).bit_length())
+        if host is not None and host.numel() < nbytes:
+            raise RuntimeError(f"stgcn_amd: a captured tail table of {nbytes} bytes exceeds {host.numel()}")
+        self.host = host if host is not None else torch.empty(cap, dtype=torch.uint8).pin_memory()
+        self.dev = torch.empty(self.host.numel(), dtype=torch.uint8, device=device)
+        self.raw = None
+        self.done = None
+
+    def upload(self, raw):
+        if self.done is not None:
+            self.done.synchronize()
+        n = len(raw)
+        self.host[:n].copy_(torch.frombuffer(raw, dtype=torch.uint8))
+        self.dev[:n].copy_(self.host[:n], non_blocking=True)
+        self.raw = raw
+        STATS["uploads"] += 1
+
+
+class TailQueue:
+    def __init__(self, device, engine=True):
+        self.device = device
+        self.engine = engine
+        self.task = torch._C._current_graph_task_id()
+        self.levels = [[] for _ in range(LEVELS)]
+        self.keep = []
+        self.stream = None
+        self.armed = False
+
+    def add(self, level, job, *keep):
+        if self.stream is None:
+            self.stream = torch.cuda.current_stream(self.device)
+        self.levels[level].append(job)
+        self.keep += [t for t in keep if t is not None]
+        if self.engine and not self.armed:
+            torch.autograd.Variable._execution_engine.queue_callback(self.flush)
+            self.armed = True
+
+    def flush(self):
+        if _queues.get(self.device.index) is self:
+            del _queues[self.device.index]
+        jobs = [j for lv in self.levels for j in lv]
+        if not jobs:
+            return
+        n = len(jobs)
+        arr = (L.TailJob * n)(*jobs)
+        L.check(L.lib().stgcn_tails_check(arr, n), "tails_check")
+        starts, runs, k = [], [], 0
+        for lv in self.levels:
+            if not lv:
+                continue
+            first, b = len(starts), 0
+            for j in arr[k:k + len(lv)]:
+                starts.append(b)
+                b += j.blocks
+            starts.append(b)
+            runs.append((k, first, len(lv), b))
+            k += len(lv)
+        raw = bytearray(memoryview(arr).cast("B")) + bytearray(memoryview((ctypes.c_long * len(starts))(*starts)).cast("B"))
+        cur = torch.cuda.current_stream(self.device)
+        with torch.cuda.stream(self.stream):
+            if torch.cuda.is_current_stream_capturing():
+                tab = _Table(self.device, len(raw), host=_spares.pop())
+                _captured.append(tab)
+            else:
+                tab = _tables.get(self.device.index)
+                if tab is None or tab.host.numel() < len(raw):
+                    tab = _tables[self.device.index] = _Table(self.device, len(raw))
+            if tab.raw != raw:
+                tab.upload(raw)
+                if tab not in _captured:
+                    tab.done = torch.cuda.Event()
+                    tab.done.record(self.stream)
+            base = tab.dev.data_ptr()
+            s = self.stream.cuda_stream
+            for k0, first, nj, nb in runs:
+                L.check(L.lib().stgcn_tails_run(base + k0 * JOB_BYTES, base + n * JOB_BYTES + 8 * first, nj, nb, s),
+                        "tails_run")
+        if cur != self.stream:
+            cur.wait_stream(self.stream)
+        STATS["flushes"] += 1
+        self.keep = []
+        self.levels = [[] for _ in range(LEVELS)]
+
+
+def queue(device) -> TailQueue:
+    q = _queues.get(device.index)
+    if q is not None and q.task != torch._C._current_graph_task_id():
+        STATS["discarded"] += 1
+        q = None
+    if q is None:
+        q = _queues[device.index] = TailQueue(device)
+    return q
+
+
+def discard_stale(device):
+    if not _spares and not torch.cuda.is_current_stream_capturing():
+        _spares.append(torch.empty(SPARE_BYTES, dtype=torch.uint8).pin_memory())
+    if _queues and device.index in _queues and torch._C._current_graph_task_id() == -1:
+        del _queues[device.index]
+        STATS["discarded"] += 1
+
+
+def _plain_leaf(p) -> bool:
+    return (p.is_leaf and p.grad is None and p.dtype == torch.float32 and p.is_contiguous()
+            and not p._backward_hooks and not getattr(p, "_post_accumulate_grad_hooks", None))
+
+
+def can_defer(cfg, params) -> bool:
+    if not (ROUTING.deferred_tails and cfg.defer) or cfg.sync is not None or torch.is_grad_enabled():
+        return False
+    if torch._C._current_graph_task_id() == -1:
+        return False
+    if not _spares and torch.cuda.is_current_stream_capturing():
+        return False
+    import torch.distributed as dist
+    if dist.is_available() and dist.is_initialized() and dist.get_world_size() > 1:
+        return False
+    return all(p is not None and p.requires_grad and _plain_leaf(p) for p in params)
```
